# matrixorigin/matrixone

Measured on AMD Instinct MI355X. Metric: ANN queries/sec @ recall@10>=0.95, 10Mx768 f32, higher is better.
Workload: dtype f32; 1 GPU; ivfflat-l2-10000000x768-nlist4096-nprobe32-batch1024-k10; rows_per_gpu=10000000, dim=768, nlist=4096, nprobe=32, global_batch=1024, k=10, scan=two-stage-refine-R64, parallelism=single

## Files before the change

include/moann.h:

```cpp

#ifndef MOANN_H
#define MOANN_H

#include <stdint.h>
#include <stddef.h>
#include <stdbool.h>

#ifdef __cplusplus
extern "C" {
#endif


typedef enum {
    DistanceType_L2Expanded = 0,
    DistanceType_L2SqrtExpanded = 1,
    DistanceType_CosineExpanded = 2,
    DistanceType_L1 = 3,
    DistanceType_InnerProduct = 6,
    DistanceType_Unknown = 255
} distance_type_t;

typedef enum {
    Quantization_F32 = 0,
    Quantization_F16 = 1,
    Quantization_INT8 = 2,
    Quantization_UINT8 = 3,
    Quantization_BF16 = 4
} quantization_t;

typedef enum {
    DistributionMode_SINGLE_GPU = 0,
    DistributionMode_SHARDED = 1,
    DistributionMode_REPLICATED = 2
} distribution_mode_t;

typedef struct {
    uint32_t n_lists;
    bool add_data_on_build;
    double kmeans_trainset_fraction;
} ivf_flat_build_params_t;

typedef struct {
    uint32_t n_probes;
} ivf_flat_search_params_t;

typedef void* gpu_ivf_flat_c;
typedef void* gpu_ivf_flat_result_c;

typedef struct {
    gpu_ivf_flat_result_c result_ptr;
} gpu_ivf_flat_search_res_t;


gpu_ivf_flat_c gpu_ivf_flat_new(const void* dataset_data,
                                uint64_t count_vectors, uint32_t dimension,
                                distance_type_t metric,
                                ivf_flat_build_params_t build_params,
                                const int* devices, int device_count,
                                uint32_t nthread,
                                distribution_mode_t dist_mode,
                                quantization_t btype, quantization_t qtype,
                                const int64_t* ids, void* errmsg);

gpu_ivf_flat_c gpu_ivf_flat_load_file(const char* filename,
                                      uint32_t dimension,
                                      distance_type_t metric,
                                      ivf_flat_build_params_t build_params,
                                      const int* devices, int device_count,
                                      uint32_t nthread,
                                      distribution_mode_t dist_mode,
                                      quantization_t btype,
                                      quantization_t qtype, void* errmsg);

gpu_ivf_flat_c gpu_ivf_flat_new_empty(uint64_t total_count, uint32_t dimension,
                                      distance_type_t metric,
                                      ivf_flat_build_params_t build_params,
                                      const int* devices, int device_count,
                                      uint32_t nthread,
                                      distribution_mode_t dist_mode,
                                      quantization_t btype, quantization_t qtype,
                                      const int64_t* ids, void* errmsg);

void gpu_ivf_flat_add_chunk(gpu_ivf_flat_c index_c, const void* chunk_data,
                            uint64_t chunk_count, const int64_t* ids,
                            void* errmsg);

void gpu_ivf_flat_add_chunk_float(gpu_ivf_flat_c index_c,
                                  const float* chunk_data,
                                  uint64_t chunk_count, const int64_t* ids,
                                  void* errmsg);

void gpu_ivf_flat_add_chunk_quantize(gpu_ivf_flat_c index_c,
                                     const void* base_data,
                                     uint64_t chunk_count, const int64_t* ids,
                                     void* errmsg);

void gpu_ivf_flat_extend(gpu_ivf_flat_c index_c, const void* new_data,
                         uint64_t n_rows, const int64_t* new_ids,
                         void* errmsg);
void gpu_ivf_flat_extend_float(gpu_ivf_flat_c index_c, const float* new_data,
                               uint64_t n_rows, const int64_t* new_ids,
                               void* errmsg);

void gpu_ivf_flat_train_quantizer(gpu_ivf_flat_c index_c,
                                  const float* train_data,
                                  uint64_t n_samples, void* errmsg);

void gpu_ivf_flat_delete_id(gpu_ivf_flat_c index_c, int64_t id, void* errmsg);

void moann_ivf_flat_set_centroids(gpu_ivf_flat_c index_c,
                                  const float* centroids, uint32_t n_lists,
                                  void* errmsg);
void moann_ivf_flat_set_assignments(gpu_ivf_flat_c index_c,
                                    const int32_t* assignments, uint64_t count,
                                    void* errmsg);

void gpu_ivf_flat_build(gpu_ivf_flat_c index_c, void* errmsg);

void moann_ivf_flat_set_kmeans_params(gpu_ivf_flat_c index_c, uint32_t n_iters,
                                      uint64_t max_train_rows, void* errmsg);

void moann_ivf_flat_get_assignments(gpu_ivf_flat_c index_c, int32_t* out,
                                    void* errmsg);

void moann_ivf_flat_kmeans_stats(gpu_ivf_flat_c index_c, double* train_ms,
                                 double* assign_ms, uint32_t* iters,
                                 uint64_t* n_train, void* errmsg);

void gpu_ivf_flat_start(gpu_ivf_flat_c index_c, void* errmsg);

void gpu_ivf_flat_save_dir(gpu_ivf_flat_c index_c, const char* dir,
                           void* errmsg);
void gpu_ivf_flat_load_dir(gpu_ivf_flat_c index_c, const char* dir,
                           distribution_mode_t target_mode, void* errmsg);

void gpu_ivf_flat_save(gpu_ivf_flat_c index_c, const char* filename,
                       void* errmsg);

char* gpu_ivf_flat_info(gpu_ivf_flat_c index_c, void* errmsg);

void gpu_ivf_flat_destroy(gpu_ivf_flat_c index_c, void* errmsg);

void gpu_ivf_flat_set_quantizer(gpu_ivf_flat_c index_c, float min, float max,
                                void* errmsg);
void gpu_ivf_flat_get_quantizer(gpu_ivf_flat_c index_c, float* min, float* max,
                                void* errmsg);


gpu_ivf_flat_search_res_t gpu_ivf_flat_search(gpu_ivf_flat_c index_c,
                                              const void* queries_data,
                                              uint64_t num_queries,
                                              uint32_t query_dimension,
                                              uint32_t limit,
                                              ivf_flat_search_params_t search_params,
                                              void* errmsg);

gpu_ivf_flat_search_res_t gpu_ivf_flat_search_quantize(
    gpu_ivf_flat_c index_c, const void* queries_data, uint64_t num_queries,
    uint32_t query_dimension, uint32_t limit,
    ivf_flat_search_params_t search_params, void* errmsg);

uint64_t gpu_ivf_flat_search_quantize_async(
    gpu_ivf_flat_c index_c, const void* queries_data, uint64_t num_queries,
    uint32_t query_dimension, uint32_t limit,
    ivf_flat_search_params_t search_params, void* errmsg);

void moann_ivf_flat_enable_refine(gpu_ivf_flat_c index_c, uint32_t depth,
                                  void* errmsg);

gpu_ivf_flat_search_res_t moann_ivf_flat_search_submit(
    gpu_ivf_flat_c index_c, const void* queries, int queries_on_device,
    uint64_t num_queries, uint32_t query_dimension, uint32_t limit,
    ivf_flat_search_params_t search_params, void* errmsg);
int moann_ivf_flat_result_wait(gpu_ivf_flat_result_c result_c, void* errmsg);

gpu_ivf_flat_search_res_t moann_ivf_flat_search_device(gpu_ivf_flat_c index_c,
                                                       const void* queries_dev,
                                                       uint64_t num_queries,
                                                       uint32_t query_dimension,
                                                       uint32_t limit,
                                                       ivf_flat_search_params_t search_params,
                                                       void* errmsg);

uint64_t gpu_ivf_flat_search_async(gpu_ivf_flat_c index_c,
                                   const void* queries_data,
                                   uint64_t num_queries,
                                   uint32_t query_dimension, uint32_t limit,
                                   ivf_flat_search_params_t search_params,
                                   void* errmsg);
gpu_ivf_flat_search_res_t gpu_ivf_flat_search_wait(gpu_ivf_flat_c index_c,
                                                   uint64_t job_id,
                                                   void* errmsg);

void gpu_ivf_flat_get_neighbors(gpu_ivf_flat_result_c result_c,
                                uint64_t total_elements, int64_t* neighbors);
void gpu_ivf_flat_get_distances(gpu_ivf_flat_result_c result_c,
                                uint64_t total_elements, float* distances);
void gpu_ivf_flat_free_result(gpu_ivf_flat_result_c result_c);


uint64_t gpu_ivf_flat_cap(gpu_ivf_flat_c index_c);
uint64_t gpu_ivf_flat_len(gpu_ivf_flat_c index_c);
uint32_t gpu_ivf_flat_get_n_list(gpu_ivf_flat_c index_c);
void gpu_ivf_flat_get_centers(gpu_ivf_flat_c index_c, void* centers,
                              void* errmsg);


void moann_brute_force_search(const float* dataset, uint64_t count,
                              uint32_t dimension, distance_type_t metric,
                              const int64_t* ids,
                              const float* queries, uint64_t num_queries,
                              uint32_t limit, int device,
                              int64_t* out_neighbors, float* out_distances,
                              void* errmsg);

void moann_pairwise_distance(distance_type_t metric, const float* query,
                             const float* rows, uint64_t n, uint32_t dim,
                             int device, float* out_dists, void* errmsg);

gpu_ivf_flat_search_res_t moann_ivf_flat_search_filtered(
    gpu_ivf_flat_c index_c, const void* queries_data, uint64_t num_queries,
    uint32_t query_dimension, uint32_t limit,
    ivf_flat_search_params_t search_params, const uint32_t* slot_bitset,
    uint64_t nbits, void* errmsg);

void moann_ivf_flat_slots_of_ids(gpu_ivf_flat_c index_c, const int64_t* ids,
                                 uint64_t n, int64_t* out_slots,
                                 void* errmsg);

void gpu_ivf_flat_set_batch_window(gpu_ivf_flat_c index_c, int64_t window_us,
                                   void* errmsg);

void gpu_ivf_flat_set_dynb_conservative_dispatch(gpu_ivf_flat_c index_c,
                                                 bool enable, void* errmsg);

void gpu_ivf_flat_set_filter_columns(gpu_ivf_flat_c index_c,
                                     const char* col_meta_json,
                                     uint64_t total_count, void* errmsg);
void gpu_ivf_flat_add_filter_chunk(gpu_ivf_flat_c index_c, uint32_t col_idx,
                                   const void* data,
                                   const uint32_t* null_bitmap,
                                   uint64_t nrows, void* errmsg);

gpu_ivf_flat_search_res_t gpu_ivf_flat_search_with_filter(
    gpu_ivf_flat_c index_c, const void* queries_data, uint64_t num_queries,
    uint32_t query_dimension, uint32_t limit,
    ivf_flat_search_params_t search_params, const char* preds_json,
    void* errmsg);
gpu_ivf_flat_search_res_t gpu_ivf_flat_search_quantize_with_filter(
    gpu_ivf_flat_c index_c, const void* queries_data, uint64_t num_queries,
    uint32_t query_dimension, uint32_t limit,
    ivf_flat_search_params_t search_params, const char* preds_json,
    void* errmsg);
uint64_t gpu_ivf_flat_search_quantize_with_filter_async(
    gpu_ivf_flat_c index_c, const void* queries_data, uint64_t num_queries,
    uint32_t query_dimension, uint32_t limit,
    ivf_flat_search_params_t search_params, const char* preds_json,
    void* errmsg);

#define MOANN_FILTER_BLOOM 0
#define MOANN_FILTER_CROARING 2
#define MOANN_FILTER_CBITMAP 3
#define MOANN_FILTER_SORTED64 4

int moann_docfilter_eval(int kind, const void* payload, uint64_t payload_len,
                         const int64_t* keys, uint64_t nkeys,
                         uint32_t* out_words, void* errmsg);

int moann_preds_eval(const char* cols_json, const char* preds_json,
                     const void* const* col_data,
                     const uint32_t* const* col_nulls,
                     const int64_t* host_ids, uint64_t nrows,
                     uint32_t* out_words, void* errmsg);

int moann_ivf_flat_filter_from_preds(gpu_ivf_flat_c index_c,
                                     const char* cols_json,
                                     const char* preds_json,
                                     const void* const* col_data,
                                     const uint32_t* const* col_nulls,
                                     uint32_t* out_words, void* errmsg);

int moann_ivf_flat_filter_from_docfilter(gpu_ivf_flat_c index_c, int kind,
                                         const void* payload,
                                         uint64_t payload_len,
                                         uint32_t* out_words, void* errmsg);


typedef struct {
    uint64_t scan_launches;
    double scan_ms;
    uint64_t scan_bytes;
    uint64_t scan_rows;
    uint64_t rank_launches;
    double rank_ms;
    uint64_t rank_flops;
    double select_ms;
    double other_ms;
} moann_perf_t;

void moann_ivf_flat_perf(gpu_ivf_flat_c index_c, moann_perf_t* out);
void moann_ivf_flat_perf_reset(gpu_ivf_flat_c index_c);


typedef void* moann_bf_c;

moann_bf_c moann_bf_new(uint32_t dimension, distance_type_t metric,
                        uint64_t capacity_hint, const int* devices,
                        int device_count, void* errmsg);
moann_bf_c moann_bf_new_typed(uint32_t dimension, distance_type_t metric,
                              quantization_t storage, uint64_t capacity_hint,
                              const int* devices, int device_count,
                              void* errmsg);
void moann_bf_add(moann_bf_c h, const float* rows, uint64_t n,
                  const int64_t* ids, void* errmsg);
void moann_bf_add_half(moann_bf_c h, const uint16_t* rows, uint64_t n,
                       const int64_t* ids, void* errmsg);
void moann_bf_delete_id(moann_bf_c h, int64_t id, void* errmsg);
void moann_bf_set_params(moann_bf_c h, uint32_t mode, uint32_t slice_rows,
                         void* errmsg);
void moann_bf_search(moann_bf_c h, const float* queries, uint64_t nq,
                     uint32_t dim, uint32_t k, int64_t* out_ids,
// ... 111 lines not shown
```

matrixone_amd/csrc/moann_internal.h:

```cpp

#ifndef MOANN_INTERNAL_H
#define MOANN_INTERNAL_H

#include <hip/hip_runtime.h>
#include <cstdint>

#include "moann_scan_plan.h"

namespace moann {

struct ScanJobs {
    const int64_t* databaseg;
    const int32_t* gstart;
    const int32_t* gcount;
    const int32_t* rows;
    const int32_t* nq;
    const int32_t* qbase;
    const int32_t* qslot_query;
    const int64_t* qslot_outbase;
    const int64_t* slot_base;
    int njobs;
};

void launch_scan(int metric, ScanVariant variant, const float* packed,
                 const float* queries, const float* qnorms, int dpad,
                 const ScanJobs& jobs, float* dists_out, hipStream_t stream,
                 const uint32_t* filter_bitset = nullptr);

void launch_scan_asm768(const float* packed, const float* queries,
                        int dpad, const ScanJobs& jobs, float* dists_out,
                        hipStream_t stream,
                        const uint32_t* filter_bitset = nullptr);

void launch_topk(const float* dists, const int64_t* qoffs, int64_t uniform_n,
                 int nq, int k, int32_t* out_slots, float* out_dists,
                 hipStream_t stream);

void launch_gather(const int32_t* sel_slots, const float* sel_dists,
                   const int32_t* probe_lists, const int64_t* probe_offs,
                   const int64_t* list_slot_base, const int64_t* id_by_slot,
                   int nprobe, int nq, int k, int do_sqrt, double inv_mul2,
                   int64_t* out_ids, float* out_dists, hipStream_t stream);

void launch_gather_uniform(const int32_t* sel_slots, const float* sel_dists,
                           const int64_t* id_by_slot, int nq, int k,
                           int do_sqrt, double inv_mul2,
                           int64_t* out_ids, float* out_dists,
                           hipStream_t stream);

void launch_pack(const float* vecs, int dim, int dpad,
                 const int64_t* group_rowbase, const int32_t* group_valid,
                 const int64_t* slot_rows, int64_t ngroups, float* packed,
                 hipStream_t stream);

void launch_unpack(const float* packed, int dim, int dpad,
                   const int64_t* group_slotbase, const int32_t* group_valid,
                   int64_t ngroups, int64_t slot_lo, int64_t slot_hi,
                   float* out, hipStream_t stream);

bool launch_rank_gemm(int metric, const float* queries, const float* cents,
                      const float* qnorms, const float* cnorms, int nq,
                      int nlist, int dpad, float* out, hipStream_t stream);

struct KmRowMap {
    int64_t num, den;
};

void launch_km_assign(int metric, const float* rows, int64_t row_stride,
                      KmRowMap map, int64_t n, const float* cents,
                      const float* cnorms, int k, int dim, int dpad,
                      int32_t* assign, float* best, hipStream_t stream);
void launch_km_row_sumsq(bool inverse_norm, const float* rows,
                         int64_t row_stride, KmRowMap map, int64_t n, int dim,
                         float* out, hipStream_t stream);
void launch_km_update(const float* rows, int64_t row_stride, KmRowMap map,
                      const int64_t* offs, const int32_t* members,
                      const float* inv_norm, int k, int dim, int dpad,
                      float* cents, hipStream_t stream);
void launch_km_set_centroids(const float* rows, int64_t row_stride,
                             KmRowMap map, const int32_t* cidx,
                             const int64_t* trow, int count, int dim, int dpad,
                             float* cents, hipStream_t stream);
void launch_km_gather_pad(const float* rows, int64_t row_stride, KmRowMap map,
                          int64_t i0, int64_t count, int dim, int dpad,
                          float* out, hipStream_t stream);

struct BfPlan;

void launch_bf_fused_topk(int metric, const float* rows, const float* xnorms,
                          const uint32_t* mask, int64_t n,
                          const float* queries, const float* qnorms, int nq,
                          int dpad, int k, const BfPlan& plan, float* cand_d,
                          int32_t* cand_r, hipStream_t stream);
void launch_bf_fused_topk_h(int metric, const uint16_t* rows,
                            const float* xnorms, const uint32_t* mask,
                            int64_t n, const uint16_t* queries,
                            const float* qnorms, int nq, int dpad, int k,
                            const BfPlan& plan, float* cand_d, int32_t* cand_r,
                            hipStream_t stream);
void launch_bf_widen_half(const uint16_t* in, int64_t nrows, int dpad_h,
                          int dpad_w, float* out, hipStream_t stream);
void launch_bf_mask(float* dmat, int nq, int64_t len, int64_t row0,
                    const uint32_t* mask, hipStream_t stream);
void launch_bf_stash(const int32_t* sel_slots, const float* sel_dists, int nq,
                     int k, int64_t row0, int64_t slice, int64_t nslices,
                     float* cand_d, int32_t* cand_r, hipStream_t stream);
void launch_bf_gather(const int32_t* sel_slots, const float* sel_dists,
                      const int32_t* cand_r, int64_t cand_per_q,
                      const int64_t* ids, int nq, int k, int do_sqrt,
                      int64_t* out_ids, float* out_dists, hipStream_t stream);

void launch_scan_i8(int metric, ScanVariant variant, bool uns,
                    ByteImageLayout layout, const uint8_t* packed,
                    const uint8_t* queries_q, const int32_t* qnorms,
                    const int32_t* rownorms, int dpad, const ScanJobs& jb,
                    float* dists_out, hipStream_t stream,
                    const uint32_t* filter_bitset = nullptr);
void launch_bytes_pack_mfma(const uint8_t* rows_q, int dpad,
                            const int64_t* group_rowbase,
                            const int32_t* group_valid,
                            const int64_t* slot_rows, int64_t ngroups,
                            uint8_t* packed, hipStream_t stream);
void launch_bytes_pack16(const uint8_t* rows_q, int dpad,
                         const int64_t* group_rowbase,
                         const int32_t* group_valid,
                         const int64_t* slot_rows, int64_t ngroups,
                         uint8_t* packed, hipStream_t stream);
void launch_rownorms_i8(bool uns, ByteImageLayout layout,
                        const uint8_t* packed, int64_t ngroups, int dpad,
                        int32_t* out, hipStream_t stream);
void launch_unpack_bytes(const uint8_t* packed, int dim, int dpad,
                         const int64_t* group_slotbase,
                         const int32_t* group_valid, int64_t ngroups,
                         int64_t slot_lo, int64_t slot_hi, uint8_t* out,
                         hipStream_t stream);
void launch_refine(int metric, const float* rows_f32, const float* queries,
                   const float* qnorms, int dim, int dpad, int R, int nq,
                   const int32_t* rsel_slots, const float* rsel_dists,
                   const int32_t* probe_lists, const int64_t* probe_offs,
                   const int64_t* list_slot_base, int nprobe, float* refined,
                   hipStream_t stream);
void launch_compose_select(const int32_t* sel2, const int32_t* rsel_slots,
                           int R, int k, int nq, int32_t* out,
                           hipStream_t stream);
void launch_quantize_rows(bool uns, const float* in, int64_t nrows,
                          int in_stride, int dim, int dpad, float fmul,
                          float fadd, uint8_t* out, hipStream_t stream);
void launch_pq_pack(const uint8_t* codes_rowmajor, int nsub,
                    const int64_t* group_rowbase, const int32_t* group_valid,
                    const int64_t* slot_rows, int64_t ngroups, uint8_t* packed,
                    hipStream_t stream);
void launch_quantize_half_rows(bool bf, const float* in, int64_t nrows,
                               int in_stride, int dim, int dpad,
                               uint16_t* out, hipStream_t stream);
void launch_qnorms_h(bool bf, const uint16_t* q, int nq, int dpad,
                     float* out, hipStream_t stream);
void launch_scan_h(int metric, ScanVariant variant, bool bf,
                   const uint16_t* packed, const uint16_t* queries_h,
                   const float* qnorms, int dpad, const ScanJobs& jb,
                   float* dists_out, hipStream_t stream,
                   const uint32_t* filter_bitset = nullptr);
void launch_qnorms_i8(bool uns, const uint8_t* q, int nq, int dpad,
                      int32_t* out, hipStream_t stream);

void launch_pairwise(int metric, const float* rows, const float* query,
                     float qnorm, int64_t n, int dim, float* out,
                     hipStream_t stream);

void launch_qnorms(const float* queries, int nq, int dpad, float* qnorms,
                   hipStream_t stream);

}

#endif
```

matrixone_amd/csrc/moann_kernels.hip:

```cpp

#include <hip/hip_runtime.h>
#include <hip/hip_fp16.h>
#include <algorithm>
#include <cfloat>
#include <cstdint>
#include <cstdlib>
#include <cstring>
#include <stdexcept>
#include <string>
#include <type_traits>

#include "moann_internal.h"
#include "moann_scan_device.h"

namespace moann {

#define WAVE 64

template <typename F>
static void with_metric(int metric, F&& f) {
    switch (metric) {
    case KM_L2SQ: f(std::integral_constant<int, KM_L2SQ>{}); break;
    case KM_IP:   f(std::integral_constant<int, KM_IP>{}); break;
    case KM_COS:  f(std::integral_constant<int, KM_COS>{}); break;
    default:      f(std::integral_constant<int, KM_L1>{}); break;
    }
}

__device__ __forceinline__ uint32_t f2u(float f) {
    uint32_t u = __float_as_uint(f);
    return u ^ (((int32_t)u >> 31) | 0x80000000u);
}
__device__ __forceinline__ float u2f(uint32_t u) {
    u ^= (((int32_t)(u ^ 0x80000000u)) >> 31) | 0x80000000u;
    return __uint_as_float(u);
}

template <int METRIC, int QT>
__global__ __launch_bounds__(256) void scan_kernel(
    const float* __restrict__ packed, const float* __restrict__ queries,
    const float* __restrict__ qnorms, int dpad, const ScanJobs jobs,
    const uint32_t* __restrict__ filter_bitset,
    float* __restrict__ dists_out) {
    extern __shared__ float lds[];
    float* ldsq = lds;
    float* ldsn = lds + QT * dpad;

    const JobView jv = load_job(jobs);
    stage_query_tile<QT, METRIC == KM_COS>(jv, jobs.qslot_query, queries,
                                           qnorms, dpad, ldsq, ldsn);

    const int wave = threadIdx.x >> 6, lane = threadIdx.x & 63;
    const int gend = jv.gstart + jv.gcount;
    const int d4 = dpad >> 2;

    for (int g0 = jv.gstart + 2 * wave; g0 < gend; g0 += 8) {
        const bool has1 = (g0 + 1) < gend;
        const int g1 = has1 ? g0 + 1 : g0;
        const float4* __restrict__ d0 =
            (const float4*)(packed + (jv.baseg + g0) * (int64_t)64 * dpad) + lane;
        const float4* __restrict__ d1 =
            (const float4*)(packed + (jv.baseg + g1) * (int64_t)64 * dpad) + lane;

        float acc0[QT], acc1[QT];
#pragma unroll
        for (int t = 0; t < QT; ++t) acc0[t] = acc1[t] = 0.f;
        float rn0 = 0.f, rn1 = 0.f;

#pragma unroll 2
        for (int q4 = 0; q4 < d4; ++q4) {
            const float4 x0 = d0[q4 * 64];
            const float4 x1 = d1[q4 * 64];
            if (METRIC == KM_COS) {
                rn0 += x0.x * x0.x + x0.y * x0.y + x0.z * x0.z + x0.w * x0.w;
                rn1 += x1.x * x1.x + x1.y * x1.y + x1.z * x1.z + x1.w * x1.w;
            }
#pragma unroll
            for (int t = 0; t < QT; ++t) {
                const float4 qv = ((const float4*)(ldsq + t * dpad))[q4];
                if (METRIC == KM_L2SQ) {
                    float e;
                    e = x0.x - qv.x; acc0[t] = fmaf(e, e, acc0[t]);
                    e = x0.y - qv.y; acc0[t] = fmaf(e, e, acc0[t]);
                    e = x0.z - qv.z; acc0[t] = fmaf(e, e, acc0[t]);
                    e = x0.w - qv.w; acc0[t] = fmaf(e, e, acc0[t]);
                    e = x1.x - qv.x; acc1[t] = fmaf(e, e, acc1[t]);
                    e = x1.y - qv.y; acc1[t] = fmaf(e, e, acc1[t]);
                    e = x1.z - qv.z; acc1[t] = fmaf(e, e, acc1[t]);
                    e = x1.w - qv.w; acc1[t] = fmaf(e, e, acc1[t]);
                } else if (METRIC == KM_IP || METRIC == KM_COS) {
                    acc0[t] = fmaf(x0.x, qv.x, acc0[t]);
                    acc0[t] = fmaf(x0.y, qv.y, acc0[t]);
                    acc0[t] = fmaf(x0.z, qv.z, acc0[t]);
                    acc0[t] = fmaf(x0.w, qv.w, acc0[t]);
                    acc1[t] = fmaf(x1.x, qv.x, acc1[t]);
                    acc1[t] = fmaf(x1.y, qv.y, acc1[t]);
                    acc1[t] = fmaf(x1.z, qv.z, acc1[t]);
                    acc1[t] = fmaf(x1.w, qv.w, acc1[t]);
                } else {
                    acc0[t] += fabsf(x0.x - qv.x) + fabsf(x0.y - qv.y) +
                               fabsf(x0.z - qv.z) + fabsf(x0.w - qv.w);
                    acc1[t] += fabsf(x1.x - qv.x) + fabsf(x1.y - qv.y) +
                               fabsf(x1.z - qv.z) + fabsf(x1.w - qv.w);
                }
            }
        }

        store_group_pair<QT, METRIC == KM_COS>(
            jobs, jv, lane, g0, g1, has1, acc0, acc1, rn0, rn1, ldsn,
            filter_bitset, dists_out, [](float acc, float rn, float qn) {
                return finish_f32<METRIC>(acc, rn, qn);
            });
    }
}

[[noreturn]] static void bad_variant(const char* launcher, ScanVariant v) {
    throw std::logic_error(std::string(launcher) + ": no kernel for scan " +
                           scan_kind_name(v.kind) + " qt=" +
                           std::to_string(v.qt));
}

void launch_scan(int metric, ScanVariant v, const float* packed,
                 const float* queries, const float* qnorms, int dpad,
                 const ScanJobs& jb, float* dists_out, hipStream_t stream,
                 const uint32_t* filter_bitset) {
    const int qt = v.qt;
    const bool asm768 = v.kind == ScanKind::F32_ASM768 && qt == 16 &&
                        metric == KM_L2SQ && dpad == 768;
    const bool generic = v.kind == ScanKind::F32 &&
                         (qt == 8 || qt == 4 || qt == 2 || qt == 1);
    if (!asm768 && !generic) bad_variant("launch_scan", v);
    if (jb.njobs == 0) return;
    if (asm768) {
        launch_scan_asm768(packed, queries, dpad, jb, dists_out, stream,
                           filter_bitset);
        return;
    }
    with_metric(metric, [&](auto m) {
        constexpr int M = decltype(m)::value;
        const dim3 grid(jb.njobs), block(256);
        const size_t shmem = (size_t)(qt * dpad + qt) * sizeof(float);
        const auto launch = [&](auto kernel) {
            hipLaunchKernelGGL(kernel, grid, block, shmem, stream, packed,
                               queries, qnorms, dpad, jb, filter_bitset,
                               dists_out);
        };
        switch (qt) {
        case 8:  launch(scan_kernel<M, 8>); break;
        case 4:  launch(scan_kernel<M, 4>); break;
        case 2:  launch(scan_kernel<M, 2>); break;
        default: launch(scan_kernel<M, 1>); break;
        }
    });
}

__global__ __launch_bounds__(256) void topk_kernel(
    const float* __restrict__ dists, const int64_t* __restrict__ qoffs,
    int64_t uniform_n, int k, int sortP,
    int32_t* __restrict__ out_slots, float* __restrict__ out_dists) {
    extern __shared__ unsigned char smem[];
    uint32_t* hist = (uint32_t*)smem;
    uint32_t* ctr = hist + 256;
    uint32_t* st = ctr + 8;
    uint64_t* keys = (uint64_t*)(smem + 2048);

    const int q = blockIdx.x;
    const int64_t off = qoffs ? qoffs[q] : (int64_t)q * uniform_n;
    const int64_t count = (qoffs ? qoffs[q + 1] : (int64_t)(q + 1) * uniform_n) - off;
    const int tid = threadIdx.x;
    const int m = (int)(count < (int64_t)k ? count : k);
    int nkeys;

    if (count > (int64_t)k) {
        if (tid == 0) { st[0] = 0; st[1] = 0; st[3] = 0; st[4] = 0; st[5] = 0; }
        __syncthreads();
        for (int level = 0; level < 4 && !st[4]; ++level) {
            const int shift = 24 - 8 * level;
            for (int b = tid; b < 256; b += blockDim.x) hist[b] = 0;
            __syncthreads();
            const uint32_t pref = st[0];
            const int64_t step = blockDim.x;
            int64_t i = tid;
#define MOANN_HISTO(u)                                                                  if (level == 0 || ((u) >> (shift + 8)) == (pref >> (shift + 8)))                atomicAdd(&hist[((u) >> shift) & 255], 1u);
            for (; i + 3 * step < count; i += 4 * step) {
                const uint32_t u0 = f2u(dists[off + i]);
                const uint32_t u1 = f2u(dists[off + i + step]);
                const uint32_t u2 = f2u(dists[off + i + 2 * step]);
                const uint32_t u3 = f2u(dists[off + i + 3 * step]);
                MOANN_HISTO(u0) MOANN_HISTO(u1) MOANN_HISTO(u2) MOANN_HISTO(u3)
            }
            for (; i < count; i += step) {
                const uint32_t u = f2u(dists[off + i]);
                MOANN_HISTO(u)
            }
#undef MOANN_HISTO
            __syncthreads();
            if (tid == 0) {
                const uint32_t need = (uint32_t)k - st[1];
                uint32_t cum = 0; int b = 0;
                for (; b < 256; ++b) {
                    if (cum + hist[b] >= need) break;
                    cum += hist[b];
                }
                st[0] = pref | ((uint32_t)b << shift);
                st[1] += cum;
                if (cum + hist[b] == need) {
                    st[1] += hist[b];
                    st[0] |= (shift ? ((1u << shift) - 1u) : 0u);
                    st[3] = 0; st[4] = 1;
                } else if (st[1] + hist[b] <= (uint32_t)sortP) {
                    st[2] = st[0];
                    st[3] = hist[b];
                    st[5] = (uint32_t)shift;
                    st[4] = 1;
                } else if (level == 3) {
                    st[2] = st[0];
                    st[3] = need - cum;
                    st[5] = 0;
                }
            }
            __syncthreads();
        }
        const uint32_t c_sure = st[1];
        const uint32_t tieval = st[2];
        const uint32_t need_ties = st[3];
        const uint32_t tie_shift = st[5];
        const int exact = st[4] && !need_ties;
        const uint64_t below = (uint64_t)st[0] + (exact ? 1u : 0u);
        if (tid == 0) { ctr[0] = 0; ctr[1] = 0; }
        __syncthreads();
        {
            const int64_t step = blockDim.x;
            int64_t i = tid;
#define MOANN_COLLECT(u, idx)                                                           if ((uint64_t)(u) < below) {                                                    const uint32_t pos = atomicAdd(&ctr[0], 1u);                                keys[pos] = ((uint64_t)(u) << 32) | (uint32_t)(idx);                    } else if (need_ties &&                                                                ((u) >> tie_shift) == (tieval >> tie_shift)) {                       const uint32_t t = atomicAdd(&ctr[1], 1u);                                  if (t < need_ties)                                                              keys[c_sure + t] = ((uint64_t)(u) << 32) | (uint32_t)(idx);             }
            for (; i + 3 * step < count; i += 4 * step) {
                const uint32_t u0 = f2u(dists[off + i]);
                const uint32_t u1 = f2u(dists[off + i + step]);
                const uint32_t u2 = f2u(dists[off + i + 2 * step]);
                const uint32_t u3 = f2u(dists[off + i + 3 * step]);
                MOANN_COLLECT(u0, i) MOANN_COLLECT(u1, i + step)
                MOANN_COLLECT(u2, i + 2 * step) MOANN_COLLECT(u3, i + 3 * step)
            }
            for (; i < count; i += step) {
                const uint32_t u = f2u(dists[off + i]);
                MOANN_COLLECT(u, i)
            }
#undef MOANN_COLLECT
        }
        __syncthreads();
        nkeys = (int)(c_sure + need_ties);
    } else {
        for (int64_t i = tid; i < count; i += blockDim.x)
            keys[i] = ((uint64_t)f2u(dists[off + i]) << 32) | (uint32_t)i;
        __syncthreads();
        nkeys = m;
    }

    for (int i = nkeys + tid; i < sortP; i += blockDim.x) keys[i] = ~0ULL;
    __syncthreads();

    for (int ks = 2; ks <= sortP; ks <<= 1) {
        for (int jj = ks >> 1; jj > 0; jj >>= 1) {
            for (int i = tid; i < sortP; i += blockDim.x) {
                const int l = i ^ jj;
                if (l > i) {
                    const uint64_t a = keys[i], b = keys[l];
                    const bool up = (i & ks) == 0;
                    if ((a > b) == up) { keys[i] = b; keys[l] = a; }
                }
            }
            __syncthreads();
        }
    }

    for (int i = tid; i < k; i += blockDim.x) {
        if (i < m) {
            const uint64_t kv = keys[i];
            out_slots[(int64_t)q * k + i] = (int32_t)(kv & 0xFFFFFFFFu);
            out_dists[(int64_t)q * k + i] = u2f((uint32_t)(kv >> 32));
        } else {
            out_slots[(int64_t)q * k + i] = -1;
            out_dists[(int64_t)q * k + i] = FLT_MAX;
        }
    }
}

void launch_topk(const float* dists, const int64_t* qoffs, int64_t uniform_n,
                 int nq, int k, int32_t* out_slots, float* out_dists,
                 hipStream_t stream) {
    if (nq == 0) return;
    int sortP = 1;
    while (sortP < k) sortP <<= 1;
    if (sortP < 1024) sortP = 1024;
    const size_t shmem = 2048 + (size_t)sortP * 8;
    hipLaunchKernelGGL(topk_kernel, dim3(nq), dim3(256), shmem, stream,
                       dists, qoffs, uniform_n, k, sortP, out_slots, out_dists);
}


__device__ __forceinline__ float transform_score_dev(float raw, int do_sqrt,
                                                     double inv_mul2) {
    double r = (double)raw * inv_mul2;
    if (do_sqrt) r = sqrt(r);
    return (float)r;
}

__global__ void gather_kernel(
    const int32_t* __restrict__ sel_slots, const float* __restrict__ sel_dists,
    const int32_t* __restrict__ probe_lists, const int64_t* __restrict__ probe_offs,
    const int64_t* __restrict__ list_slot_base, const int64_t* __restrict__ id_by_slot,
    int nprobe, int nq, int k, int do_sqrt, double inv_mul2,
    int64_t* __restrict__ out_ids, float* __restrict__ out_dists) {
    const int64_t idx = (int64_t)blockIdx.x * blockDim.x + threadIdx.x;
    if (idx >= (int64_t)nq * k) return;
    const int q = (int)(idx / k);
    const int32_t slot = sel_slots[idx];
    if (slot < 0 || sel_dists[idx] == FLT_MAX) {
        out_ids[idx] = -1; out_dists[idx] = FLT_MAX; return;
    }
    const int64_t* offs = probe_offs + (int64_t)q * (nprobe + 1);
    int lo = 0, hi = nprobe - 1;
    while (lo < hi) {
        const int mid = (lo + hi + 1) >> 1;
        if (offs[mid] <= slot) lo = mid; else hi = mid - 1;
    }
    const int32_t list = probe_lists[(int64_t)q * nprobe + lo];
    const int64_t local = slot - offs[lo];
    out_ids[idx] = id_by_slot[list_slot_base[list] + local];
    out_dists[idx] = transform_score_dev(sel_dists[idx], do_sqrt, inv_mul2);
}

void launch_gather(const int32_t* sel_slots, const float* sel_dists,
                   const int32_t* probe_lists, const int64_t* probe_offs,
                   const int64_t* list_slot_base, const int64_t* id_by_slot,
                   int nprobe, int nq, int k, int do_sqrt, double inv_mul2,
                   int64_t* out_ids, float* out_dists, hipStream_t stream) {
    const int64_t total = (int64_t)nq * k;
    if (!total) return;
    const int block = 256;
    const int grid = (int)((total + block - 1) / block);
    hipLaunchKernelGGL(gather_kernel, dim3(grid), dim3(block), 0, stream,
                       sel_slots, sel_dists, probe_lists, probe_offs,
                       list_slot_base, id_by_slot, nprobe, nq, k, do_sqrt,
                       inv_mul2, out_ids, out_dists);
}

__global__ void gather_uniform_kernel(
    const int32_t* __restrict__ sel_slots, const float* __restrict__ sel_dists,
    const int64_t* __restrict__ id_by_slot, int nq, int k, int do_sqrt,
    double inv_mul2, int64_t* __restrict__ out_ids,
    float* __restrict__ out_dists) {
    const int64_t idx = (int64_t)blockIdx.x * blockDim.x + threadIdx.x;
    if (idx >= (int64_t)nq * k) return;
    const int32_t slot = sel_slots[idx];
    if (slot < 0) { out_ids[idx] = -1; out_dists[idx] = FLT_MAX; return; }
    out_ids[idx] = id_by_slot ? id_by_slot[slot] : (int64_t)slot;
    out_dists[idx] = transform_score_dev(sel_dists[idx], do_sqrt, inv_mul2);
}

void launch_gather_uniform(const int32_t* sel_slots, const float* sel_dists,
                           const int64_t* id_by_slot, int nq, int k,
                           int do_sqrt, double inv_mul2, int64_t* out_ids,
                           float* out_dists, hipStream_t stream) {
    const int64_t total = (int64_t)nq * k;
    if (!total) return;
    const int block = 256;
    const int grid = (int)((total + block - 1) / block);
    hipLaunchKernelGGL(gather_uniform_kernel, dim3(grid), dim3(block), 0,
                       stream, sel_slots, sel_dists, id_by_slot, nq, k,
                       do_sqrt, inv_mul2, out_ids, out_dists);
}

__global__ void pack_kernel(const float* __restrict__ vecs, int dim, int dpad,
                            const int64_t* __restrict__ group_rowbase,
                            const int32_t* __restrict__ group_valid,
                            const int64_t* __restrict__ slot_rows,
                            int64_t ngroups, float* __restrict__ packed) {
    const int64_t nquads = ngroups * (dpad >> 2) * 64;
    const int64_t stride = (int64_t)gridDim.x * blockDim.x;
    for (int64_t idx = (int64_t)blockIdx.x * blockDim.x + threadIdx.x;
         idx < nquads; idx += stride) {
        const int lane = (int)(idx & 63);
        const int64_t rest = idx >> 6;
        const int j4 = (int)(rest % (dpad >> 2));
        const int64_t g = rest / (dpad >> 2);
        float4 v = {0.f, 0.f, 0.f, 0.f};
        if (lane < group_valid[g]) {
            const int64_t row = slot_rows[group_rowbase[g] + lane];
            const float* src = vecs + row * (int64_t)dim;
            const int base = 4 * j4;
            v.x = base + 0 < dim ? src[base + 0] : 0.f;
            v.y = base + 1 < dim ? src[base + 1] : 0.f;
            v.z = base + 2 < dim ? src[base + 2] : 0.f;
            v.w = base + 3 < dim ? src[base + 3] : 0.f;
        }
        ((float4*)packed)[idx] = v;
    }
}

void launch_pack(const float* vecs, int dim, int dpad,
                 const int64_t* group_rowbase, const int32_t* group_valid,
                 const int64_t* slot_rows, int64_t ngroups, float* packed,
                 hipStream_t stream) {
    const int64_t nquads = ngroups * (int64_t)(dpad >> 2) * 64;
    if (!nquads) return;
    const int block = 256;
    const int64_t grid = std::min<int64_t>((nquads + block - 1) / block,
                                           1 << 22);
    hipLaunchKernelGGL(pack_kernel, dim3((uint32_t)grid), dim3(block), 0,
                       stream, vecs, dim, dpad, group_rowbase, group_valid,
                       slot_rows, ngroups, packed);
}

__global__ void unpack_kernel(const float* __restrict__ packed, int dim,
                              int dpad,
                              const int64_t* __restrict__ group_slotbase,
                              const int32_t* __restrict__ group_valid,
                              int64_t ngroups, int64_t slot_lo,
                              int64_t slot_hi, float* __restrict__ out) {
    const int64_t nquads = ngroups * (dpad >> 2) * 64;
    const int64_t stride = (int64_t)gridDim.x * blockDim.x;
    for (int64_t idx = (int64_t)blockIdx.x * blockDim.x + threadIdx.x;
         idx < nquads; idx += stride) {
        const int lane = (int)(idx & 63);
        const int64_t rest = idx >> 6;
        const int j4 = (int)(rest % (dpad >> 2));
        const int64_t g = rest / (dpad >> 2);
        if (lane >= group_valid[g]) continue;
        const int64_t slot = group_slotbase[g] + lane;
        if (slot < slot_lo || slot >= slot_hi) continue;
        const float4 v = ((const float4*)packed)[idx];
        float* dst = out + (slot - slot_lo) * (int64_t)dim;
        const int base = 4 * j4;
        if (base + 0 < dim) dst[base + 0] = v.x;
        if (base + 1 < dim) dst[base + 1] = v.y;
        if (base + 2 < dim) dst[base + 2] = v.z;
        if (base + 3 < dim) dst[base + 3] = v.w;
    }
}

void launch_unpack(const float* packed, int dim, int dpad,
                   const int64_t* group_slotbase, const int32_t* group_valid,
                   int64_t ngroups, int64_t slot_lo, int64_t slot_hi,
                   float* out, hipStream_t stream) {
    const int64_t nquads = ngroups * (int64_t)(dpad >> 2) * 64;
    if (!nquads) return;
    const int block = 256;
    const int64_t grid = std::min<int64_t>((nquads + block - 1) / block,
                                           1 << 22);
// ... 190 lines not shown
            }
#pragma unroll
            for (int t = 0; t < QT; ++t) {
                const uint4 qw =
                    *(const uint4*)(ldsq + t * dpad + j8 * 8);
                float qv[8];
                MOANN_H8(qw.x, qv[0], qv[1]) MOANN_H8(qw.y, qv[2], qv[3])
                MOANN_H8(qw.z, qv[4], qv[5]) MOANN_H8(qw.w, qv[6], qv[7])
#pragma unroll
                for (int u = 0; u < 8; ++u) {
                    if (METRIC == KM_L2SQ) {
                        const float e0 = x0[u] - qv[u];
                        acc0[t] = fmaf(e0, e0, acc0[t]);
                        const float e1 = x1[u] - qv[u];
                        acc1[t] = fmaf(e1, e1, acc1[t]);
                    } else if (METRIC == KM_IP || METRIC == KM_COS) {
                        acc0[t] = fmaf(x0[u], qv[u], acc0[t]);
                        acc1[t] = fmaf(x1[u], qv[u], acc1[t]);
                    } else {
                        acc0[t] += fabsf(x0[u] - qv[u]);
                        acc1[t] += fabsf(x1[u] - qv[u]);
                    }
                }
            }
        }
#undef MOANN_H8

        store_group_pair<QT, METRIC == KM_COS>(
            jobs, jv, lane, g0, g1, has1, acc0, acc1, rn0, rn1, ldsn,
            filter_bitset, dists_out, [](float acc, float rn, float qn) {
                return finish_f32<METRIC>(acc, rn, qn);
            });
    }
}

void launch_scan_h(int metric, ScanVariant v, bool bf,
                   const uint16_t* packed, const uint16_t* queries_h,
                   const float* qnorms, int dpad, const ScanJobs& jb,
                   float* dists_out, hipStream_t stream,
                   const uint32_t* filter_bitset) {
    if (v.kind != ScanKind::HALF || v.qt != 8) bad_variant("launch_scan_h", v);
    if (!jb.njobs) return;
    with_metric(metric, [&](auto m) {
        constexpr int M = decltype(m)::value;
        const dim3 grid(jb.njobs), block(256);
        const size_t shmem = 8 * dpad * 2 + 8 * 4 + 16;
        const auto launch = [&](auto kernel) {
            hipLaunchKernelGGL(kernel, grid, block, shmem, stream, packed,
                               queries_h, qnorms, dpad, jb, filter_bitset,
                               dists_out);
        };
        bf ? launch(scan_h_kernel<M, true>) : launch(scan_h_kernel<M, false>);
    });
}

template <int METRIC>
__global__ __launch_bounds__(256) void refine_kernel(
    const float* __restrict__ rows_f32,
    const float* __restrict__ queries,
    const float* __restrict__ qnorms,
    int dim, int dpad, int R,
    const int32_t* __restrict__ rsel_slots,
    const float* __restrict__ rsel_dists,
    const int32_t* __restrict__ probe_lists,
    const int64_t* __restrict__ probe_offs,
    const int64_t* __restrict__ list_slot_base, int nprobe,
    float* __restrict__ refined ) {
    extern __shared__ float ldsq[];
    const int q = blockIdx.x;
    const float* qv = queries + (int64_t)q * dpad;
    for (int e = threadIdx.x; e < dpad; e += blockDim.x) ldsq[e] = qv[e];
    __syncthreads();
    const int wave = threadIdx.x >> 6, lane = threadIdx.x & 63;
    const int64_t* offs = probe_offs + (int64_t)q * (nprobe + 1);

    for (int c = wave; c < R; c += 4) {
        const int64_t idx = (int64_t)q * R + c;
        const int32_t pos = rsel_slots[idx];
        if (pos < 0 || rsel_dists[idx] == FLT_MAX) {
            if (lane == 0) refined[idx] = FLT_MAX;
            continue;
        }
        int lo = 0, hi = nprobe - 1;
        while (lo < hi) {
            const int mid = (lo + hi + 1) >> 1;
            if (offs[mid] <= pos) lo = mid; else hi = mid - 1;
        }
        const int32_t list = probe_lists[(int64_t)q * nprobe + lo];
        const int64_t slot = list_slot_base[list] + (pos - offs[lo]);
        const float* row = rows_f32 + slot * (int64_t)dim;
        float acc = 0.f, rn = 0.f;
        for (int t = lane; t < dim; t += 64) {
            const float x = row[t], qq = ldsq[t];
            if (METRIC == KM_L2SQ) {
                const float e = x - qq;
                acc = fmaf(e, e, acc);
            } else if (METRIC == KM_IP || METRIC == KM_COS) {
                acc = fmaf(x, qq, acc);
                if (METRIC == KM_COS) rn = fmaf(x, x, rn);
            } else {
                acc += fabsf(x - qq);
            }
        }
        for (int off = 32; off; off >>= 1) {
            acc += __shfl_down(acc, off, 64);
            if (METRIC == KM_COS) rn += __shfl_down(rn, off, 64);
        }
        if (lane == 0) {
            float dist;
            if (METRIC == KM_IP) dist = -acc;
            else if (METRIC == KM_COS)
                dist = mo_cos_distance(acc, rn, qnorms[q]);
            else dist = acc;
            refined[idx] = dist;
        }
    }
}

void launch_refine(int metric, const float* rows_f32, const float* queries,
                   const float* qnorms, int dim, int dpad, int R, int nq,
                   const int32_t* rsel_slots, const float* rsel_dists,
                   const int32_t* probe_lists, const int64_t* probe_offs,
                   const int64_t* list_slot_base, int nprobe, float* refined,
                   hipStream_t stream) {
    if (!nq) return;
    const size_t shmem = (size_t)dpad * 4;
    with_metric(metric, [&](auto m) {
        hipLaunchKernelGGL(refine_kernel<decltype(m)::value>, dim3(nq),
                           dim3(256), shmem, stream, rows_f32, queries, qnorms,
                           dim, dpad, R, rsel_slots, rsel_dists, probe_lists,
                           probe_offs, list_slot_base, nprobe, refined);
    });
}

__global__ void compose_select_kernel(const int32_t* __restrict__ sel2,
                                      const int32_t* __restrict__ rsel_slots,
                                      int R, int k, int64_t total,
                                      int32_t* __restrict__ out) {
    const int64_t i = (int64_t)blockIdx.x * blockDim.x + threadIdx.x;
    if (i >= total) return;
    const int32_t s2 = sel2[i];
    const int64_t q = i / k;
    out[i] = s2 < 0 ? -1 : rsel_slots[q * R + s2];
}

void launch_compose_select(const int32_t* sel2, const int32_t* rsel_slots,
                           int R, int k, int nq, int32_t* out,
                           hipStream_t stream) {
    const int64_t total = (int64_t)nq * k;
    if (!total) return;
    hipLaunchKernelGGL(compose_select_kernel,
                       dim3((uint32_t)((total + 255) / 256)), dim3(256), 0,
                       stream, sel2, rsel_slots, R, k, total, out);
}

template <int METRIC, bool UNSIGNED>
__global__ __launch_bounds__(256) void scan_i8_kernel(
    const uint8_t* __restrict__ packed, const uint8_t* __restrict__ queries_q,
    const int32_t* __restrict__ qnorms_i ,
    int dpad, const ScanJobs jobs,
    const uint32_t* __restrict__ filter_bitset,
    float* __restrict__ dists_out) {
    constexpr int QT = 8;
    extern __shared__ float ldsf[];
    uint8_t* ldsq = (uint8_t*)ldsf;
    int32_t* ldsn = (int32_t*)(ldsq + QT * dpad);

    const JobView jv = load_job(jobs);
    stage_query_tile<QT, METRIC == KM_COS>(jv, jobs.qslot_query, queries_q,
                                           qnorms_i, dpad, ldsq, ldsn);

    const int wave = threadIdx.x >> 6, lane = threadIdx.x & 63;
    const int gend = jv.gstart + jv.gcount;
    const int d4 = dpad >> 2;

    const auto sx = [](uint8_t b) -> int {
        return UNSIGNED ? (int)b : (int)(int8_t)b;
    };

    for (int g0 = jv.gstart + 2 * wave; g0 < gend; g0 += 8) {
        const bool has1 = (g0 + 1) < gend;
        const int g1 = has1 ? g0 + 1 : g0;
        const uchar4* __restrict__ d0 =
            (const uchar4*)(packed + (jv.baseg + g0) * (int64_t)64 * dpad) + lane;
        const uchar4* __restrict__ d1 =
            (const uchar4*)(packed + (jv.baseg + g1) * (int64_t)64 * dpad) + lane;
        int32_t acc0[QT], acc1[QT];
#pragma unroll
        for (int t = 0; t < QT; ++t) acc0[t] = acc1[t] = 0;
        int32_t rn0 = 0, rn1 = 0;
#pragma unroll 2
        for (int q4 = 0; q4 < d4; ++q4) {
            const uchar4 x0 = d0[q4 * 64];
            const uchar4 x1 = d1[q4 * 64];
            if (METRIC == KM_COS) {
                rn0 += sx(x0.x) * sx(x0.x) + sx(x0.y) * sx(x0.y) +
                       sx(x0.z) * sx(x0.z) + sx(x0.w) * sx(x0.w);
                rn1 += sx(x1.x) * sx(x1.x) + sx(x1.y) * sx(x1.y) +
                       sx(x1.z) * sx(x1.z) + sx(x1.w) * sx(x1.w);
            }
#pragma unroll
            for (int t = 0; t < QT; ++t) {
                const uchar4 qv = ((const uchar4*)(ldsq + t * dpad))[q4];
                if (METRIC == KM_L2SQ) {
                    int e;
                    e = sx(x0.x) - sx(qv.x); acc0[t] += e * e;
                    e = sx(x0.y) - sx(qv.y); acc0[t] += e * e;
                    e = sx(x0.z) - sx(qv.z); acc0[t] += e * e;
                    e = sx(x0.w) - sx(qv.w); acc0[t] += e * e;
                    e = sx(x1.x) - sx(qv.x); acc1[t] += e * e;
                    e = sx(x1.y) - sx(qv.y); acc1[t] += e * e;
                    e = sx(x1.z) - sx(qv.z); acc1[t] += e * e;
                    e = sx(x1.w) - sx(qv.w); acc1[t] += e * e;
                } else if (METRIC == KM_IP || METRIC == KM_COS) {
                    acc0[t] += sx(x0.x) * sx(qv.x) + sx(x0.y) * sx(qv.y) +
                               sx(x0.z) * sx(qv.z) + sx(x0.w) * sx(qv.w);
                    acc1[t] += sx(x1.x) * sx(qv.x) + sx(x1.y) * sx(qv.y) +
                               sx(x1.z) * sx(qv.z) + sx(x1.w) * sx(qv.w);
                } else {
                    acc0[t] += abs(sx(x0.x) - sx(qv.x)) +
                               abs(sx(x0.y) - sx(qv.y)) +
                               abs(sx(x0.z) - sx(qv.z)) +
                               abs(sx(x0.w) - sx(qv.w));
                    acc1[t] += abs(sx(x1.x) - sx(qv.x)) +
                               abs(sx(x1.y) - sx(qv.y)) +
                               abs(sx(x1.z) - sx(qv.z)) +
                               abs(sx(x1.w) - sx(qv.w));
                }
            }
        }
        store_group_pair<QT, METRIC == KM_COS>(
            jobs, jv, lane, g0, g1, has1, acc0, acc1, rn0, rn1, ldsn,
            filter_bitset, dists_out, [](int32_t acc, int32_t rn, int32_t qn) {
                return finish_i32<METRIC, false>(acc, rn, qn);
            });
    }
}

template <int METRIC, bool UNSIGNED, int QT = 8>
__global__ __launch_bounds__(256) void scan_i8_dot_kernel(
    const uint8_t* __restrict__ packed, const uint8_t* __restrict__ queries_q,
    const int32_t* __restrict__ qnorms_i,
    const int32_t* __restrict__ rownorms,
    int dpad, const ScanJobs jobs,
    const uint32_t* __restrict__ filter_bitset,
    float* __restrict__ dists_out) {
    constexpr bool NEED_N = METRIC == KM_L2SQ || METRIC == KM_COS;
    extern __shared__ float ldsf[];
    uint8_t* ldsq = (uint8_t*)ldsf;
    int32_t* ldsn = (int32_t*)(ldsq + QT * dpad);

    const JobView jv = load_job(jobs);
    stage_query_tile<QT, NEED_N>(jv, jobs.qslot_query, queries_q, qnorms_i,
                                 dpad, ldsq, ldsn);

    const int wave = threadIdx.x >> 6, lane = threadIdx.x & 63;
    const int gend = jv.gstart + jv.gcount;
    const int d16 = dpad >> 4;

    for (int g0 = jv.gstart + 2 * wave; g0 < gend; g0 += 8) {
        const bool has1 = (g0 + 1) < gend;
        const int g1 = has1 ? g0 + 1 : g0;
        const uint4* __restrict__ d0 =
            (const uint4*)(packed + (jv.baseg + g0) * (int64_t)64 * dpad) + lane;
        const uint4* __restrict__ d1 =
            (const uint4*)(packed + (jv.baseg + g1) * (int64_t)64 * dpad) + lane;

        int32_t acc0[QT], acc1[QT];
#pragma unroll
        for (int t = 0; t < QT; ++t) acc0[t] = acc1[t] = 0;

#pragma unroll 2
        for (int j16 = 0; j16 < d16; ++j16) {
            uint4 x0 = d0[j16 * 64];
            uint4 x1 = d1[j16 * 64];
            if (METRIC == KM_L1 && !UNSIGNED) {
                x0.x ^= 0x80808080u; x0.y ^= 0x80808080u;
                x0.z ^= 0x80808080u; x0.w ^= 0x80808080u;
                x1.x ^= 0x80808080u; x1.y ^= 0x80808080u;
                x1.z ^= 0x80808080u; x1.w ^= 0x80808080u;
            }
#pragma unroll
            for (int t = 0; t < QT; ++t) {
                uint4 qv = *(const uint4*)(ldsq + t * dpad + j16 * 16);
                if (METRIC == KM_L1) {
                    if (!UNSIGNED) {
                        qv.x ^= 0x80808080u; qv.y ^= 0x80808080u;
                        qv.z ^= 0x80808080u; qv.w ^= 0x80808080u;
                    }
                    acc0[t] = (int32_t)__builtin_amdgcn_sad_u8(x0.x, qv.x, (uint32_t)acc0[t]);
                    acc0[t] = (int32_t)__builtin_amdgcn_sad_u8(x0.y, qv.y, (uint32_t)acc0[t]);
                    acc0[t] = (int32_t)__builtin_amdgcn_sad_u8(x0.z, qv.z, (uint32_t)acc0[t]);
                    acc0[t] = (int32_t)__builtin_amdgcn_sad_u8(x0.w, qv.w, (uint32_t)acc0[t]);
                    acc1[t] = (int32_t)__builtin_amdgcn_sad_u8(x1.x, qv.x, (uint32_t)acc1[t]);
                    acc1[t] = (int32_t)__builtin_amdgcn_sad_u8(x1.y, qv.y, (uint32_t)acc1[t]);
                    acc1[t] = (int32_t)__builtin_amdgcn_sad_u8(x1.z, qv.z, (uint32_t)acc1[t]);
                    acc1[t] = (int32_t)__builtin_amdgcn_sad_u8(x1.w, qv.w, (uint32_t)acc1[t]);
                } else if (UNSIGNED) {
                    acc0[t] = (int32_t)__builtin_amdgcn_udot4(x0.x, qv.x, (uint32_t)acc0[t], false);
                    acc0[t] = (int32_t)__builtin_amdgcn_udot4(x0.y, qv.y, (uint32_t)acc0[t], false);
                    acc0[t] = (int32_t)__builtin_amdgcn_udot4(x0.z, qv.z, (uint32_t)acc0[t], false);
                    acc0[t] = (int32_t)__builtin_amdgcn_udot4(x0.w, qv.w, (uint32_t)acc0[t], false);
                    acc1[t] = (int32_t)__builtin_amdgcn_udot4(x1.x, qv.x, (uint32_t)acc1[t], false);
                    acc1[t] = (int32_t)__builtin_amdgcn_udot4(x1.y, qv.y, (uint32_t)acc1[t], false);
                    acc1[t] = (int32_t)__builtin_amdgcn_udot4(x1.z, qv.z, (uint32_t)acc1[t], false);
                    acc1[t] = (int32_t)__builtin_amdgcn_udot4(x1.w, qv.w, (uint32_t)acc1[t], false);
// ... 513 lines not shown
```

matrixone_amd/csrc/moann_lib.cpp:

```cpp

#include <hip/hip_runtime.h>

#include <algorithm>
#include <cfloat>
#include <cmath>
#include <cstdio>
#include <cstdlib>
#include <cstring>
#include <map>
#include <unordered_map>
#include <memory>
#include <atomic>
#include <condition_variable>
#include <mutex>
#include <thread>
#include <chrono>
#include <numeric>
#include <stdexcept>
#include <string>
#include <vector>

#include "../../include/moann.h"
#include "moann_host_common.h"
#include "moann_kmeans_plan.h"

namespace {

using namespace moann;

#define HIP_CHECK MOANN_HIP_CHECK
#define KCHECK MOANN_KCHECK
using DevBuf = MoannDevBuf;
constexpr auto set_errmsg = moann_set_errmsg;

using Result = MoannResult;

struct PerfState {
    moann_perf_t c {};
    hipEvent_t ev[8] {};
    bool made = false;
    void ensure() {
        if (made) return;
        for (auto& e : ev) HIP_CHECK(hipEventCreate(&e));
        made = true;
    }
    ~PerfState() {
        if (made)
            for (auto& e : ev) (void)hipEventDestroy(e);
    }
};

struct SearchCtx {
    hipStream_t stream = nullptr;
    hipEvent_t ev[6] {};
    bool made = false;
    DevBuf w_queries, w_qnorms, w_cdists, w_csel_slots, w_csel_dists;
    DevBuf w_jobs, w_qslots, w_cand, w_sel_slots, w_sel_dists;
    DevBuf w_probe_lists, w_probe_offs, w_qoffs, w_out_ids, w_out_dists;
    DevBuf w_filter, w_queries_q, w_qnorms_i;
    DevBuf w_rsel_slots, w_rsel_dists, w_refined, w_sel2;
    void* h_out = nullptr;
    size_t h_out_bytes = 0;
    std::vector<uint32_t> h_filter;
    std::vector<int32_t> h_probe;
    HostScanJobs rank_jobs;
    ProbeOffsets offs;
    ListScanPlan lists;
    struct Call {
        uint64_t nq = 0;
        uint32_t limit = 0, probe = 0;
        ScanChoice scan {};
        bool refine = false;
        const float* d_q = nullptr;
        const float* d_qn = nullptr;
    } call;
    MoannResult* pending = nullptr;
    void* parent = nullptr;
    void ensure(void* ix) {
        parent = ix;
        if (made) return;
        HIP_CHECK(hipStreamCreate(&stream));
        for (auto& e : ev) HIP_CHECK(hipEventCreate(&e));
        made = true;
    }
    void ensure_hout(size_t need) {
        if (need <= h_out_bytes) return;
        if (h_out) (void)hipHostFree(h_out);
        h_out = nullptr;
        h_out_bytes = 0;
        HIP_CHECK(hipHostMalloc(&h_out, need));
        h_out_bytes = need;
    }
    ~SearchCtx() {
        if (made) {
            (void)hipStreamDestroy(stream);
            for (auto& e : ev) (void)hipEventDestroy(e);
        }
        if (h_out) (void)hipHostFree(h_out);
    }
};

struct IvfIndex {
    int device = 0;
    uint32_t dim = 0, dpad = 0, nlist = 0;
    distance_type_t metric = DistanceType_L2Expanded;
    int kmetric = KM_L2SQ;
    uint64_t cap = 0, count = 0;
    quantization_t btype = Quantization_F32;
    quantization_t qtype = Quantization_F32;
    double quant_mul = 1.0, quant_add = 0.0;
    double quant_min = 0.0, quant_max = 0.0;
    uint8_t* d_packed_q = nullptr;
    int32_t* d_rownorm_q = nullptr;
    int refine_depth = 0;
    float* d_rows_f32 = nullptr;
    uint8_t* d_packed_rq = nullptr;
    ByteImageLayout rq_layout = ByteImageLayout::ROWS16;
    int32_t* d_rownorm_rq = nullptr;
    double rq_mul = 1.0, rq_add = 0.0;
    bool built = false, started = false;

    hipStream_t stream = nullptr;

    std::vector<int64_t> h_ids;
    std::vector<int32_t> h_assign;
    std::vector<float> h_centroids;
    float* d_staging = nullptr;
    double km_fraction = KMEANS_DEFAULT_FRACTION;
    uint32_t km_iters = 0;
    uint64_t km_max_train = 0;
    double km_train_ms = 0.0, km_assign_ms = 0.0;
    uint32_t km_iters_run = 0;
    uint64_t km_n_train = 0;

    float* d_packed = nullptr;
    float* d_cent_packed = nullptr;
    float* d_cent_rows = nullptr;
    float* d_cnorms = nullptr;
    bool rank_mfma = false;
    int64_t* d_id_by_slot = nullptr;
    int64_t* d_list_slot_base = nullptr;
    std::vector<int64_t> list_gbase;
    std::vector<int64_t> group_slotbase;
    std::vector<int32_t> group_valid;
    std::vector<int32_t> list_rows;
    std::vector<int64_t> list_slot_base;
    int64_t total_groups = 0;
    int64_t cent_groups = 0;

    SearchCtx sctx[2];
    uint64_t sparity = 0;
    std::vector<int64_t> h_id_by_slot;
    std::vector<int64_t> h_slot_rows;
    std::unordered_map<int64_t, int64_t> id_to_slot;

    std::mutex mu;
    PerfState perf;

    std::map<uint64_t, std::unique_ptr<Result>> jobs;
    uint64_t next_job = 1;

    std::atomic<int64_t> batch_window_us {0};
    struct PendingReq {
        std::vector<float> queries;
        uint64_t nq;
        uint32_t limit, nprobe;
        uint64_t job_id;
    };
    std::mutex bmu;
    std::condition_variable bcv;
    std::condition_variable bdone_cv;
    std::vector<PendingReq> pending;
    std::map<uint64_t, std::unique_ptr<Result>> done_jobs;
    std::thread batcher;
    bool batcher_stop = false;
    bool batcher_started = false;
    bool dynb_conservative = false;

    std::shared_ptr<IvfIndex> tail;
    std::vector<float> tail_staging;
    std::vector<int64_t> tail_ids;
    std::vector<int32_t> tail_assign;
    std::vector<int64_t> tail_deleted;

    std::vector<uint32_t> alive;
    uint64_t deleted_count = 0;

    std::string filter_cols_json;
    std::vector<int> filter_col_types;
    std::vector<std::vector<uint8_t>> filter_col_data;
    std::vector<std::vector<uint32_t>> filter_col_nulls;
    std::vector<uint64_t> filter_col_rows;
    std::vector<bool> filter_col_has_nulls;

    ~IvfIndex() {
        if (batcher_started) {
            {
                std::lock_guard<std::mutex> lk(bmu);
                batcher_stop = true;
            }
            bcv.notify_all();
            batcher.join();
        }
        (void)hipSetDevice(device);
        for (auto p : {(void*)d_staging, (void*)d_packed, (void*)d_cent_packed,
                       (void*)d_cent_rows, (void*)d_cnorms, (void*)d_packed_q,
                       (void*)d_rownorm_q, (void*)d_rows_f32,
                       (void*)d_packed_rq, (void*)d_rownorm_rq,
                       (void*)d_id_by_slot, (void*)d_list_slot_base})
            if (p) (void)hipFree(p);
        if (stream) (void)hipStreamDestroy(stream);
    }
};

void pack_lists(IvfIndex* ix, const float* d_rows, int64_t nrows,
                const std::vector<int64_t>& slot_rows,
                const std::vector<int64_t>& loffsets,
                float** d_packed_out, std::vector<int64_t>* gbase_out,
                int64_t* ngroups_out) {
    (void)nrows;
    const int64_t nlists = (int64_t)loffsets.size() - 1;
    std::vector<int64_t> gbase(nlists + 1, 0);
    for (int64_t l = 0; l < nlists; ++l) {
        const int64_t rows = loffsets[l + 1] - loffsets[l];
        gbase[l + 1] = gbase[l] + (rows + 63) / 64;
    }
    const int64_t ngroups = gbase[nlists];
    std::vector<int64_t> group_rowbase(ngroups);
    std::vector<int32_t> group_valid(ngroups);
    for (int64_t l = 0; l < nlists; ++l) {
        const int64_t rows = loffsets[l + 1] - loffsets[l];
        for (int64_t g = gbase[l]; g < gbase[l + 1]; ++g) {
            const int64_t gi = g - gbase[l];
            group_rowbase[g] = loffsets[l] + gi * 64;
            const int64_t rem = rows - gi * 64;
            group_valid[g] = (int32_t)std::min<int64_t>(64, rem);
        }
    }
    float* d_packed = nullptr;
    HIP_CHECK(hipMalloc(&d_packed,
                        (size_t)ngroups * 64 * ix->dpad * sizeof(float)));
    DevBuf tmp_rb, tmp_gv, tmp_sr;
    tmp_rb.ensure(ngroups * sizeof(int64_t));
    tmp_gv.ensure(ngroups * sizeof(int32_t));
    tmp_sr.ensure(std::max<size_t>(1, slot_rows.size() * sizeof(int64_t)));
    HIP_CHECK(hipMemcpyAsync(tmp_rb.ptr, group_rowbase.data(),
                             ngroups * sizeof(int64_t), hipMemcpyHostToDevice,
                             ix->stream));
    HIP_CHECK(hipMemcpyAsync(tmp_gv.ptr, group_valid.data(),
                             ngroups * sizeof(int32_t), hipMemcpyHostToDevice,
                             ix->stream));
    if (!slot_rows.empty())
        HIP_CHECK(hipMemcpyAsync(tmp_sr.ptr, slot_rows.data(),
                                 slot_rows.size() * sizeof(int64_t),
                                 hipMemcpyHostToDevice, ix->stream));
    launch_pack(d_rows, (int)ix->dim, (int)ix->dpad, tmp_rb.as<int64_t>(),
                tmp_gv.as<int32_t>(), tmp_sr.as<int64_t>(), ngroups, d_packed,
                ix->stream);
    KCHECK("pack");
    HIP_CHECK(hipStreamSynchronize(ix->stream));
    HIP_CHECK(hipGetLastError());
    *d_packed_out = d_packed;
    if (gbase_out) *gbase_out = std::move(gbase);
    *ngroups_out = ngroups;
}


float half_to_f32(uint16_t b) {
    const uint32_t s = (uint32_t)(b >> 15) << 31;
    uint32_t e = (b >> 10) & 0x1f, m = b & 0x3ff;
    uint32_t out;
    if (e == 0) {
        if (m == 0) out = s;
        else {
            e = 127 - 14;
            while (!(m & 0x400)) { m <<= 1; --e; }
            m &= 0x3ff;
            out = s | (e << 23) | (m << 13);
        }
    } else if (e == 31) {
        out = s | 0x7f800000u | (m << 13);
    } else {
        out = s | ((e + 112) << 23) | (m << 13);
    }
    float f;
    memcpy(&f, &out, 4);
    return f;
}

float bf16_to_f32(uint16_t b) {
    const uint32_t out = (uint32_t)b << 16;
    float f;
    memcpy(&f, &out, 4);
    return f;
}

void storage_to_f32(quantization_t st, const void* src, size_t n,
                    double mul, double add, float* dst) {
    switch (st) {
    case Quantization_F32:
        memcpy(dst, src, n * 4);
        break;
    case Quantization_INT8: {
        const int8_t* p = (const int8_t*)src;
        const double m = mul == 0.0 ? 1.0 : mul;
        for (size_t i = 0; i < n; ++i)
            dst[i] = (float)(((double)p[i] - add) / m);
        break;
    }
    case Quantization_UINT8: {
        const uint8_t* p = (const uint8_t*)src;
        const double m = mul == 0.0 ? 1.0 : mul;
        for (size_t i = 0; i < n; ++i)
            dst[i] = (float)(((double)p[i] - add) / m);
        break;
    }
    case Quantization_F16: {
        const uint16_t* p = (const uint16_t*)src;
        for (size_t i = 0; i < n; ++i) dst[i] = half_to_f32(p[i]);
        break;
    }
    case Quantization_BF16: {
        const uint16_t* p = (const uint16_t*)src;
        for (size_t i = 0; i < n; ++i) dst[i] = bf16_to_f32(p[i]);
        break;
    }
    default:
        throw std::runtime_error("unsupported storage type");
    }
}

size_t storage_elem_bytes(quantization_t st) {
    return st == Quantization_F32 ? 4
           : (st == Quantization_F16 || st == Quantization_BF16) ? 2 : 1;
}

std::vector<float> base_to_f32(quantization_t btype, const void* src,
                               size_t n) {
    std::vector<float> out(n);
    if (btype == Quantization_F32) memcpy(out.data(), src, n * 4);
    else if (btype == Quantization_F16) {
        const uint16_t* p = (const uint16_t*)src;
        for (size_t i = 0; i < n; ++i) out[i] = half_to_f32(p[i]);
    } else throw std::runtime_error("base type must be F32 or F16");
    return out;
}


double collect_result(MoannResult* res);

const ScanOverrides& scan_overrides() {
    static const ScanOverrides ov = [] {
        const char *sc = getenv("MOANN_SCAN"), *bq = getenv("MOANN_BYTE_QT"),
                   *cg = getenv("MOANN_CHUNKG"),
                   *bm = getenv("MOANN_BYTE_MFMA");
        ScanOverrides o;
        o.generic_f32 = sc && strcmp(sc, "generic") == 0;
        o.byte_qt8 = bq && atoi(bq) == 8;
        o.chunk_g = cg ? atoi(cg) : 0;
        o.byte_mfma_off = bm && strcmp(bm, "0") == 0;
        return o;
    }();
    return ov;
}

void stage_queries(IvfIndex* ix, SearchCtx* cx, const float* queries,
                   bool queries_on_device) {
    SearchCtx::Call& c = cx->call;
    const int dpad = (int)ix->dpad;
    const hipStream_t s = cx->stream;
    c.d_q = stage_padded_queries(cx->w_queries, queries, queries_on_device,
                                 c.nq, ix->dim, ix->dpad, s);
    c.d_qn = nullptr;
    const bool use_mfma_rank = ix->rank_mfma && ix->kmetric != KM_L1;
    if (ix->kmetric == KM_COS || use_mfma_rank) {
        cx->w_qnorms.ensure(c.nq * 4);
        launch_qnorms(c.d_q, (int)c.nq, dpad, cx->w_qnorms.as<float>(), s);
        KCHECK("qnorms");
        c.d_qn = cx->w_qnorms.as<float>();
    }
}

void rank_centroids(IvfIndex* ix, SearchCtx* cx) {
    const SearchCtx::Call& c = cx->call;
    const int dpad = (int)ix->dpad, nq = (int)c.nq;
    const hipStream_t s = cx->stream;
    cx->w_cdists.ensure((size_t)c.nq * ix->nlist * 4);
    if (ix->rank_mfma && ix->kmetric != KM_L1) {
        HIP_CHECK(hipEventRecord(cx->ev[0], s));
        launch_rank_gemm(ix->kmetric, c.d_q, ix->d_cent_rows, c.d_qn,
                         ix->d_cnorms, nq, (int)ix->nlist, dpad,
                         cx->w_cdists.as<float>(), s);
        KCHECK("rank-gemm");
    } else {
        plan_rank_scan(c.nq, c.scan.rank.qt, ix->nlist, ix->cent_groups,
                       cx->rank_jobs);
        const ScanJobs jb = upload_scan_jobs(cx->rank_jobs, cx->w_jobs, s);
        HIP_CHECK(hipEventRecord(cx->ev[0], s));
        launch_scan(ix->kmetric, c.scan.rank, ix->d_cent_packed, c.d_q,
                    c.d_qn, dpad, jb, cx->w_cdists.as<float>(), s);
        KCHECK("rank-scan");
    }
    HIP_CHECK(hipEventRecord(cx->ev[1], s));
    cx->w_csel_slots.ensure((size_t)c.nq * c.probe * 4);
    cx->w_csel_dists.ensure((size_t)c.nq * c.probe * 4);
    launch_topk(cx->w_cdists.as<float>(), nullptr, ix->nlist, nq,
                (int)c.probe, cx->w_csel_slots.as<int32_t>(),
                cx->w_csel_dists.as<float>(), s);
    KCHECK("rank-topk");
}

void fetch_probe_and_plan(IvfIndex* ix, SearchCtx* cx) {
    const SearchCtx::Call& c = cx->call;
    const hipStream_t s = cx->stream;
    cx->h_probe.resize((size_t)c.nq * c.probe);
    HIP_CHECK(hipMemcpyAsync(cx->h_probe.data(), cx->w_csel_slots.ptr,
                             cx->h_probe.size() * 4, hipMemcpyDeviceToHost, s));
    HIP_CHECK(hipStreamSynchronize(s));
    HIP_CHECK(hipGetLastError());
    plan_probe_offsets(cx->h_probe.data(), c.nq, c.probe, ix->list_rows,
                       cx->offs);
    plan_list_scan(cx->h_probe.data(), c.nq, c.probe, c.scan.list.qt,
                   list_chunk_groups(ix->qtype, scan_overrides()),
                   ix->list_rows, ix->list_gbase, ix->list_slot_base,
                   cx->offs, cx->lists);
}

void scan_lists(IvfIndex* ix, SearchCtx* cx, const uint32_t* filter_words) {
    const SearchCtx::Call& c = cx->call;
    const int dpad = (int)ix->dpad, nq = (int)c.nq;
    const hipStream_t s = cx->stream;
    const ScanVariant v = c.scan.list;
    const uint32_t* d_filter = nullptr;
    if (filter_words) {
        const size_t fw = (size_t)((ix->count + 31) / 32);
        cx->h_filter.assign(filter_words, filter_words + fw);
        cx->w_filter.ensure(fw * 4);
        HIP_CHECK(hipMemcpyAsync(cx->w_filter.ptr, cx->h_filter.data(),
                                 fw * 4, hipMemcpyHostToDevice, s));
        d_filter = cx->w_filter.as<uint32_t>();
    }
    cx->w_cand.ensure(std::max<int64_t>(1, cx->offs.total_cand) * 4);
    float* d_cand = cx->w_cand.as<float>();
    const ScanJobs jb = upload_scan_jobs(cx->lists.jobs, cx->w_qslots, s);
    HIP_CHECK(hipEventRecord(cx->ev[2], s));
    switch (v.kind) {
    case ScanKind::BYTE_DOT:
    case ScanKind::BYTE_U4: {
        const bool uns = !c.refine && ix->qtype == Quantization_UINT8;
        const uint8_t* image = c.refine ? ix->d_packed_rq : ix->d_packed_q;
        const ByteImageLayout layout =
            c.refine ? ix->rq_layout : ByteImageLayout::ROWS16;
        const int32_t* rownorms =
            c.refine ? ix->d_rownorm_rq : ix->d_rownorm_q;
        const double mul = c.refine ? ix->rq_mul : ix->quant_mul;
        const double add = c.refine ? ix->rq_add : ix->quant_add;
        cx->w_queries_q.ensure((size_t)c.nq * dpad);
        uint8_t* d_qq = cx->w_queries_q.as<uint8_t>();
        launch_quantize_rows(uns, c.d_q, (int64_t)c.nq, dpad, (int)ix->dim,
                             dpad, (float)mul, (float)add, d_qq, s);
        KCHECK("query-quantize");
        const int32_t* d_qni = nullptr;
        if (ix->kmetric == KM_COS || ix->kmetric == KM_L2SQ) {
            cx->w_qnorms_i.ensure(c.nq * 4);
            launch_qnorms_i8(uns, d_qq, nq, dpad,
                             cx->w_qnorms_i.as<int32_t>(), s);
            d_qni = cx->w_qnorms_i.as<int32_t>();
        }
        launch_scan_i8(ix->kmetric, v, uns, layout, image, d_qq, d_qni,
                       rownorms, dpad, jb, d_cand, s, d_filter);
        break;
    }
    case ScanKind::HALF: {
        const bool bf = ix->qtype == Quantization_BF16;
        cx->w_queries_q.ensure((size_t)c.nq * dpad * 2);
        uint16_t* d_qh = cx->w_queries_q.as<uint16_t>();
        launch_quantize_half_rows(bf, c.d_q, (int64_t)c.nq, dpad,
                                  (int)ix->dim, dpad, d_qh, s);
        KCHECK("query-half-cast");
        const float* d_qnh = nullptr;
        if (ix->kmetric == KM_COS) {
            cx->w_qnorms_i.ensure(c.nq * 4);
            launch_qnorms_h(bf, d_qh, nq, dpad, cx->w_qnorms_i.as<float>(),
                            s);
            d_qnh = cx->w_qnorms_i.as<float>();
        }
        launch_scan_h(ix->kmetric, v, bf, (const uint16_t*)ix->d_packed_q,
                      d_qh, d_qnh, dpad, jb, d_cand, s, d_filter);
        break;
    }
    case ScanKind::F32:
    case ScanKind::F32_ASM768:
        launch_scan(ix->kmetric, v, ix->d_packed, c.d_q, c.d_qn, dpad, jb,
                    d_cand, s, d_filter);
        break;
    }
    KCHECK("list-scan");
    HIP_CHECK(hipEventRecord(cx->ev[3], s));
}

void select_candidates(IvfIndex* ix, SearchCtx* cx) {
    const SearchCtx::Call& c = cx->call;
    const int dpad = (int)ix->dpad, nq = (int)c.nq, limit = (int)c.limit;
    const hipStream_t s = cx->stream;
    upload_vector(cx->w_qoffs, cx->offs.qoffs, s);
    upload_vector(cx->w_probe_lists, cx->h_probe, s);
    upload_vector(cx->w_probe_offs, cx->offs.probe_offs, s);
    cx->w_sel_slots.ensure((size_t)c.nq * limit * 4);
    cx->w_sel_dists.ensure((size_t)c.nq * limit * 4);
    HIP_CHECK(hipEventRecord(cx->ev[4], s));
    if (c.refine) {
        const int R = std::max<int>(limit, ix->refine_depth);
        cx->w_rsel_slots.ensure((size_t)c.nq * R * 4);
        cx->w_rsel_dists.ensure((size_t)c.nq * R * 4);
        launch_topk(cx->w_cand.as<float>(), cx->w_qoffs.as<int64_t>(), 0, nq,
                    R, cx->w_rsel_slots.as<int32_t>(),
                    cx->w_rsel_dists.as<float>(), s);
        KCHECK("refine-topR");
        cx->w_refined.ensure((size_t)c.nq * R * 4);
        launch_refine(ix->kmetric, ix->d_rows_f32, c.d_q, c.d_qn,
                      (int)ix->dim, dpad, R, nq,
                      cx->w_rsel_slots.as<int32_t>(),
                      cx->w_rsel_dists.as<float>(),
                      cx->w_probe_lists.as<int32_t>(),
                      cx->w_probe_offs.as<int64_t>(), ix->d_list_slot_base,
                      (int)c.probe, cx->w_refined.as<float>(), s);
        KCHECK("refine");
        cx->w_sel2.ensure((size_t)c.nq * limit * 4);
        launch_topk(cx->w_refined.as<float>(), nullptr, R, nq, limit,
                    cx->w_sel2.as<int32_t>(), cx->w_sel_dists.as<float>(), s);
        KCHECK("refine-topk");
        launch_compose_select(cx->w_sel2.as<int32_t>(),
                              cx->w_rsel_slots.as<int32_t>(), R, limit, nq,
                              cx->w_sel_slots.as<int32_t>(), s);
        KCHECK("refine-compose");
    } else {
        launch_topk(cx->w_cand.as<float>(), cx->w_qoffs.as<int64_t>(), 0, nq,
                    limit, cx->w_sel_slots.as<int32_t>(),
                    cx->w_sel_dists.as<float>(), s);
        KCHECK("cand-topk");
    }
    HIP_CHECK(hipEventRecord(cx->ev[5], s));
}

void gather_results(IvfIndex* ix, SearchCtx* cx) {
    const SearchCtx::Call& c = cx->call;
    const size_t n = (size_t)c.nq * c.limit;
    const hipStream_t s = cx->stream;
    const int do_sqrt = ix->metric == DistanceType_L2SqrtExpanded;
    const double inv_mul2 =
        (ix->quant_mul != 0.0 && ix->quant_mul != 1.0)
            ? 1.0 / (ix->quant_mul * ix->quant_mul) : 1.0;
    cx->w_out_ids.ensure(n * 8);
    cx->w_out_dists.ensure(n * 4);
    launch_gather(cx->w_sel_slots.as<int32_t>(), cx->w_sel_dists.as<float>(),
                  cx->w_probe_lists.as<int32_t>(),
                  cx->w_probe_offs.as<int64_t>(), ix->d_list_slot_base,
                  ix->d_id_by_slot, (int)c.probe, (int)c.nq, (int)c.limit,
                  do_sqrt, inv_mul2, cx->w_out_ids.as<int64_t>(),
                  cx->w_out_dists.as<float>(), s);
    KCHECK("gather");
    cx->ensure_hout(n * 12);
    int64_t* ho_ids = (int64_t*)cx->h_out;
    float* ho_dists = (float*)(ho_ids + n);
    HIP_CHECK(hipMemcpyAsync(ho_ids, cx->w_out_ids.ptr, n * 8,
                             hipMemcpyDeviceToHost, s));
    HIP_CHECK(hipMemcpyAsync(ho_dists, cx->w_out_dists.ptr, n * 4,
                             hipMemcpyDeviceToHost, s));
}

std::unique_ptr<Result> run_search(IvfIndex* ix, const float* queries,
                                   bool queries_on_device, uint64_t nq,
                                   uint32_t limit, uint32_t n_probes,
                                   const uint32_t* filter_words = nullptr,
                                   bool sync_end = true) {
    std::lock_guard<std::mutex> lk(ix->mu);
    HIP_CHECK(hipSetDevice(ix->device));
    SearchCtx* cx = &ix->sctx[ix->sparity++ & 1];
    cx->ensure(ix);
    if (cx->pending) collect_result(cx->pending);
    auto res = std::make_unique<Result>();
    res->neighbors.assign((size_t)nq * limit, -1);
    res->distances.assign((size_t)nq * limit, FLT_MAX);
    if (nq == 0) return res;
    if (!ix->built) throw std::runtime_error("index not built");
    if (ix->count == 0) return res;
    if (limit > 4096) throw std::runtime_error("limit > 4096 unsupported");
    const uint32_t probe =
        std::min<uint32_t>(n_probes ? n_probes : 1, ix->nlist);
    if (probe > 4096) throw std::runtime_error("n_probes > 4096 unsupported");
    ix->perf.ensure();

    SearchCtx::Call& c = cx->call;
    c.nq = nq;
    c.limit = limit;
    c.probe = probe;
    c.refine = ix->qtype == Quantization_F32 && ix->refine_depth > 0 &&
               ix->d_packed_rq != nullptr;
    c.scan = pick_scan(ix->kmetric, (int)ix->dpad, ix->qtype, c.refine,
                       (c.refine ? ix->d_rownorm_rq : ix->d_rownorm_q) !=
                           nullptr,
                       scan_overrides());

    const auto t_all0 = std::chrono::steady_clock::now();
    stage_queries(ix, cx, queries, queries_on_device);
    rank_centroids(ix, cx);
    fetch_probe_and_plan(ix, cx);
    scan_lists(ix, cx, filter_words);
    select_candidates(ix, cx);
    gather_results(ix, cx);

    ix->perf.c.rank_launches++;
    ix->perf.c.rank_flops += 2ull * nq * ix->nlist * ix->dim;
    uint64_t unique_rows = 0;
    for (uint32_t l = 0; l < ix->nlist; ++l)
        if (cx->lists.lcount[l]) unique_rows += (uint64_t)ix->list_rows[l];
    ix->perf.c.scan_launches++;
    ix->perf.c.scan_bytes += unique_rows * ix->dim * 4;
    ix->perf.c.scan_rows += (uint64_t)cx->offs.total_cand;

    res->owner = cx;
    res->collected = false;
    HIP_CHECK(hipEventCreate(&res->done_ev));
    HIP_CHECK(hipEventRecord(res->done_ev, cx->stream));
    cx->pending = res.get();
    const double kms = sync_end ? collect_result(res.get()) : 0.0;
    const double wall = std::chrono::duration<double, std::milli>(
        std::chrono::steady_clock::now() - t_all0).count();
    ix->perf.c.other_ms += wall - kms;
    return res;
}

void merge_tail_into(MoannResult* res) {
    if (!res->tail_res || res->tail_merged) return;
    MoannResult* t = res->tail_res.get();
    const size_t total = res->neighbors.size();
    if (t->neighbors.size() != total || total == 0) { res->tail_merged = true; return; }
    const uint32_t limit = res->merge_limit;
    const size_t nq = limit ? total / limit : 0;
    const bool ip = res->merge_kmetric == KM_IP;
    auto closer = [&](float a, float b) { return ip ? a > b : a < b; };
    std::vector<int64_t> mi(limit);
    std::vector<float> md(limit);
    for (size_t q = 0; q < nq; ++q) {
        const int64_t* an = res->neighbors.data() + q * limit;
        const float* ad = res->distances.data() + q * limit;
        const int64_t* bn = t->neighbors.data() + q * limit;
        const float* bd = t->distances.data() + q * limit;
        uint32_t i = 0, j = 0, o = 0;
        while (o < limit) {
            const bool av = i < limit && an[i] != -1;
            const bool bv = j < limit && bn[j] != -1;
            if (!av && !bv) break;
            if (av && (!bv || closer(ad[i], bd[j]) ||
                       (ad[i] == bd[j] && true ))) {
                mi[o] = an[i]; md[o] = ad[i]; ++i;
            } else {
                mi[o] = bn[j]; md[o] = bd[j]; ++j;
            }
            ++o;
        }
        for (; o < limit; ++o) { mi[o] = -1; md[o] = FLT_MAX; }
        memcpy(res->neighbors.data() + q * limit, mi.data(), limit * 8);
        memcpy(res->distances.data() + q * limit, md.data(), limit * 4);
    }
    res->tail_merged = true;
    res->tail_res.reset();
}

double collect_result(MoannResult* res) {
    if (res->collected) return 0.0;
    auto cx = (SearchCtx*)res->owner;
    auto ix = (IvfIndex*)cx->parent;
    HIP_CHECK(hipEventSynchronize(res->done_ev));
    HIP_CHECK(hipGetLastError());
    const size_t n = res->neighbors.size();
    const int64_t* ho_ids = (const int64_t*)cx->h_out;
    const float* ho_dists = (const float*)(ho_ids + n);
    memcpy(res->neighbors.data(), ho_ids, n * 8);
    memcpy(res->distances.data(), ho_dists, n * 4);
    if (ix->kmetric == KM_IP) {
        float* d = res->distances.data();
        for (size_t i = 0; i < n; ++i)
            if (d[i] != FLT_MAX && d[i] != -FLT_MAX) d[i] = -d[i];
    }
    float r_ms = 0, sc_ms = 0, sel_ms = 0;
    (void)hipEventElapsedTime(&r_ms, cx->ev[0], cx->ev[1]);
    (void)hipEventElapsedTime(&sc_ms, cx->ev[2], cx->ev[3]);
    (void)hipEventElapsedTime(&sel_ms, cx->ev[4], cx->ev[5]);
    ix->perf.c.rank_ms += r_ms;
    ix->perf.c.scan_ms += sc_ms;
    ix->perf.c.select_ms += sel_ms;
    res->collected = true;
    if (cx->pending == res) cx->pending = nullptr;
    merge_tail_into(res);
    return (double)r_ms + sc_ms + sel_ms;
}

uint64_t total_len(IvfIndex* ix) {
    return ix->count + (ix->tail ? ix->tail->count : 0);
}

std::vector<uint32_t> combined_filter(IvfIndex* ix, uint64_t slot0,
                                      const uint32_t* user, uint64_t nbits) {
    const uint64_t n = ix->count;
    std::vector<uint32_t> out((size_t)((n + 31) / 32), ~0u);
    if (user) {
        if (slot0 % 32 == 0 && slot0 + n <= nbits) {
            memcpy(out.data(), user + slot0 / 32, out.size() * 4);
            if (n % 32)
                out.back() |= ~((1u << (n % 32)) - 1u);
        } else {
            for (uint64_t i = 0; i < n; ++i) {
                const uint64_t g = slot0 + i;
// ... 879 lines not shown
        ix->done_jobs.erase(it);
        if (res->neighbors.empty() && res->distances.empty())
            throw std::runtime_error("batched search failed");
        out.result_ptr = res.release();
    } catch (const std::exception& e) {
        set_errmsg(errmsg, "gpu_ivf_flat_search_wait", e.what());
    }
    return out;
}

void gpu_ivf_flat_get_neighbors(gpu_ivf_flat_result_c r, uint64_t n,
                                int64_t* neighbors) {
    auto res = (Result*)r;
    if (!res->collected) collect_result(res);
    const uint64_t m = std::min<uint64_t>(n, res->neighbors.size());
    memcpy(neighbors, res->neighbors.data(), m * 8);
}

void gpu_ivf_flat_get_distances(gpu_ivf_flat_result_c r, uint64_t n,
                                float* distances) {
    auto res = (Result*)r;
    if (!res->collected) collect_result(res);
    const uint64_t m = std::min<uint64_t>(n, res->distances.size());
    memcpy(distances, res->distances.data(), m * 4);
}

void gpu_ivf_flat_free_result(gpu_ivf_flat_result_c r) {
    auto res = (Result*)r;
    if (res && res->done_ev) {
        if (!res->collected) {
            (void)hipEventSynchronize(res->done_ev);
            auto cx = (SearchCtx*)res->owner;
            if (cx && cx->pending == res) cx->pending = nullptr;
        }
        (void)hipEventDestroy(res->done_ev);
    }
    delete res;
}

int moann_ivf_flat_filter_from_preds(gpu_ivf_flat_c h, const char* cols_json,
                                     const char* preds_json,
                                     const void* const* col_data,
                                     const uint32_t* const* col_nulls,
                                     uint32_t* out_words, void* errmsg) {
    try {
        auto ix = IX(h);
        if (!ix->built) throw std::runtime_error("index not built");
        const uint64_t n = ix->count;
        std::vector<uint32_t> row_bits((n + 31) / 32, 0);
        std::vector<int64_t> ids_by_row(n);
        for (uint64_t s2 = 0; s2 < n; ++s2)
            ids_by_row[ix->h_slot_rows[s2]] = ix->h_id_by_slot[s2];
        const int rc = moann_preds_eval(cols_json, preds_json, col_data,
                                        col_nulls, ids_by_row.data(), n,
                                        row_bits.data(), errmsg);
        if (rc != 0) return rc;
        std::memset(out_words, 0, ((n + 31) / 32) * 4);
        for (uint64_t s2 = 0; s2 < n; ++s2) {
            const uint64_t row = (uint64_t)ix->h_slot_rows[s2];
            if ((row_bits[row >> 5] >> (row & 31)) & 1u)
                out_words[s2 >> 5] |= 1u << (s2 & 31);
        }
        return 0;
    } catch (const std::exception& e) {
        set_errmsg(errmsg, "moann_ivf_flat_filter_from_preds", e.what());
        return -1;
    }
}

int moann_ivf_flat_filter_from_docfilter(gpu_ivf_flat_c h, int kind,
                                         const void* payload,
                                         uint64_t payload_len,
                                         uint32_t* out_words, void* errmsg) {
    try {
        auto ix = IX(h);
        if (!ix->built) throw std::runtime_error("index not built");
        return moann_docfilter_eval(kind, payload, payload_len,
                                    ix->h_id_by_slot.data(), ix->count,
                                    out_words, errmsg);
    } catch (const std::exception& e) {
        set_errmsg(errmsg, "moann_ivf_flat_filter_from_docfilter", e.what());
        return -1;
    }
}

uint64_t gpu_ivf_flat_cap(gpu_ivf_flat_c h) { return IX(h)->cap; }
uint64_t gpu_ivf_flat_len(gpu_ivf_flat_c h) { return total_len(IX(h)); }
uint32_t gpu_ivf_flat_get_n_list(gpu_ivf_flat_c h) { return IX(h)->nlist; }

void gpu_ivf_flat_get_centers(gpu_ivf_flat_c h, void* centers, void* errmsg) {
    try {
        auto ix = IX(h);
        if (ix->h_centroids.empty())
            throw std::runtime_error("no centroids set");
        memcpy(centers, ix->h_centroids.data(),
               ix->h_centroids.size() * sizeof(float));
    } catch (const std::exception& e) {
        set_errmsg(errmsg, "gpu_ivf_flat_get_centers", e.what());
    }
}

void moann_ivf_flat_set_kmeans_params(gpu_ivf_flat_c h, uint32_t n_iters,
                                      uint64_t max_train_rows, void* errmsg) {
    try {
        auto ix = IX(h);
        std::lock_guard<std::mutex> lk(ix->mu);
        if (ix->built)
            throw std::runtime_error("index already built");
        ix->km_iters = n_iters;
        ix->km_max_train = max_train_rows;
    } catch (const std::exception& e) {
        set_errmsg(errmsg, "moann_ivf_flat_set_kmeans_params", e.what());
    }
}

void moann_ivf_flat_get_assignments(gpu_ivf_flat_c h, int32_t* out,
                                    void* errmsg) {
    try {
        auto ix = IX(h);
        std::lock_guard<std::mutex> lk(ix->mu);
        if (!ix->built) throw std::runtime_error("index not built");
        if (ix->h_slot_rows.size() != ix->count)
            throw std::runtime_error(
                "add-order rows are not kept for a loaded index");
        for (uint32_t l = 0; l < ix->nlist; ++l) {
            const int64_t b = ix->list_slot_base[l];
            for (int64_t sl = b; sl < b + ix->list_rows[l]; ++sl)
                out[ix->h_slot_rows[sl]] = (int32_t)l;
        }
        for (size_t i = 0; i < ix->tail_assign.size(); ++i)
            out[ix->count + i] = ix->tail_assign[i];
    } catch (const std::exception& e) {
        set_errmsg(errmsg, "moann_ivf_flat_get_assignments", e.what());
    }
}

void moann_ivf_flat_kmeans_stats(gpu_ivf_flat_c h, double* train_ms,
                                 double* assign_ms, uint32_t* iters,
                                 uint64_t* n_train, void* errmsg) {
    try {
        auto ix = IX(h);
        if (!ix) throw std::runtime_error("null index");
        std::lock_guard<std::mutex> lk(ix->mu);
        if (!ix->built) throw std::runtime_error("index not built");
        if (train_ms) *train_ms = ix->km_train_ms;
        if (assign_ms) *assign_ms = ix->km_assign_ms;
        if (iters) *iters = ix->km_iters_run;
        if (n_train) *n_train = ix->km_n_train;
    } catch (const std::exception& e) {
        set_errmsg(errmsg, "moann_ivf_flat_kmeans_stats", e.what());
    }
}

void moann_brute_force_search(const float* dataset, uint64_t count,
                              uint32_t dimension, distance_type_t metric,
                              const int64_t* ids, const float* queries,
                              uint64_t num_queries, uint32_t limit, int device,
                              int64_t* out_neighbors, float* out_distances,
                              void* errmsg) {
    char* inner = nullptr;
    try {
        ivf_flat_build_params_t bp {1, true, 0.5};
        gpu_ivf_flat_c h = gpu_ivf_flat_new_empty(
            count, dimension, metric, bp, &device, 1, 0,
            DistributionMode_SINGLE_GPU, Quantization_F32, Quantization_F32,
            nullptr, &inner);
        if (!h) throw std::runtime_error(inner ? inner : "new failed");
        gpu_ivf_flat_add_chunk(h, dataset, count, ids, &inner);
        std::vector<float> cent(dimension, 0.f);
        moann_ivf_flat_set_centroids(h, cent.data(), 1, &inner);
        std::vector<int32_t> assign(count, 0);
        moann_ivf_flat_set_assignments(h, assign.data(), count, &inner);
        gpu_ivf_flat_build(h, &inner);
        if (inner) throw std::runtime_error(inner);
        ivf_flat_search_params_t sp {1};
        auto r = gpu_ivf_flat_search(h, queries, num_queries, dimension, limit,
                                     sp, &inner);
        if (!r.result_ptr) throw std::runtime_error(inner ? inner : "search failed");
        gpu_ivf_flat_get_neighbors(r.result_ptr, num_queries * limit,
                                   out_neighbors);
        gpu_ivf_flat_get_distances(r.result_ptr, num_queries * limit,
                                   out_distances);
        if (metric == DistanceType_InnerProduct)
            for (uint64_t i = 0; i < num_queries * (uint64_t)limit; ++i)
                if (out_distances[i] != FLT_MAX && out_distances[i] != -FLT_MAX)
                    out_distances[i] = -out_distances[i];
        gpu_ivf_flat_free_result(r.result_ptr);
        gpu_ivf_flat_destroy(h, nullptr);
    } catch (const std::exception& e) {
        set_errmsg(errmsg, "moann_brute_force_search", e.what());
    }
    if (inner) free(inner);
}

gpu_ivf_flat_search_res_t moann_ivf_flat_search_filtered(
    gpu_ivf_flat_c h, const void* queries_data, uint64_t num_queries,
    uint32_t query_dimension, uint32_t limit, ivf_flat_search_params_t sp,
    const uint32_t* slot_bitset, uint64_t nbits, void* errmsg) {
    gpu_ivf_flat_search_res_t out {nullptr};
    try {
        auto ix = IX(h);
        if (query_dimension != ix->dim)
            throw std::runtime_error("query dimension mismatch");
        if (nbits < total_len(ix))
            throw std::runtime_error("filter bitset smaller than index");
        out.result_ptr = run_search_full(ix, (const float*)queries_data,
                                         false, num_queries, limit,
                                         sp.n_probes, slot_bitset, nbits)
                             .release();
    } catch (const std::exception& e) {
        set_errmsg(errmsg, "moann_ivf_flat_search_filtered", e.what());
    }
    return out;
}

void moann_ivf_flat_slots_of_ids(gpu_ivf_flat_c h, const int64_t* ids,
                                 uint64_t n, int64_t* out_slots,
                                 void* errmsg) {
    try {
        auto ix = IX(h);
        std::lock_guard<std::mutex> lk(ix->mu);
        if (!ix->built) throw std::runtime_error("index not built");
        if (ix->id_to_slot.empty() && ix->count) {
            ix->id_to_slot.reserve(ix->count * 2);
            for (uint64_t sidx = 0; sidx < ix->count; ++sidx)
                ix->id_to_slot.emplace(ix->h_id_by_slot[sidx], (int64_t)sidx);
        }
        IvfIndex* t = ix->tail.get();
        if (t && t->count && t->id_to_slot.empty()) {
            t->id_to_slot.reserve(t->count * 2);
            for (uint64_t sidx = 0; sidx < t->count; ++sidx)
                t->id_to_slot.emplace(t->h_id_by_slot[sidx], (int64_t)sidx);
        }
        for (uint64_t i = 0; i < n; ++i) {
            auto it = ix->id_to_slot.find(ids[i]);
            if (it != ix->id_to_slot.end()) {
                out_slots[i] = it->second;
                continue;
            }
            out_slots[i] = -1;
            if (t && t->count) {
                auto jt = t->id_to_slot.find(ids[i]);
                if (jt != t->id_to_slot.end())
                    out_slots[i] = (int64_t)ix->count + jt->second;
            }
        }
    } catch (const std::exception& e) {
        set_errmsg(errmsg, "moann_ivf_flat_slots_of_ids", e.what());
    }
}


gpu_ivf_flat_c gpu_ivf_flat_new(const void* dataset_data,
                                uint64_t count_vectors, uint32_t dimension,
                                distance_type_t metric,
                                ivf_flat_build_params_t build_params,
                                const int* devices, int device_count,
                                uint32_t nthread,
                                distribution_mode_t dist_mode,
                                quantization_t btype, quantization_t qtype,
                                const int64_t* ids, void* errmsg) {
    char* inner = nullptr;
    gpu_ivf_flat_c h = gpu_ivf_flat_new_empty(
        count_vectors, dimension, metric, build_params, devices,
        device_count, nthread, dist_mode, btype, qtype, ids, &inner);
    if (!h) {
        set_errmsg(errmsg, "gpu_ivf_flat_new", inner ? inner : "new failed");
        if (inner) free(inner);
        return nullptr;
    }
    if (count_vectors)
        gpu_ivf_flat_add_chunk(h, dataset_data, count_vectors, ids, &inner);
    if (inner) {
        set_errmsg(errmsg, "gpu_ivf_flat_new", inner);
        free(inner);
        gpu_ivf_flat_destroy(h, nullptr);
        return nullptr;
    }
    return h;
}


static void rebuild_tail(IvfIndex* ix) {
    char* inner = nullptr;
    auto chk = [&](const char* what) {
        if (inner) {
            std::string m = std::string(what) + ": " + inner;
            free(inner);
            inner = nullptr;
            throw std::runtime_error(m);
        }
    };
    const uint64_t n = ix->tail_ids.size();
    ivf_flat_build_params_t bp {ix->nlist, true, 1.0};
    int dev = ix->device;
    gpu_ivf_flat_c th = gpu_ivf_flat_new_empty(
        n, ix->dim, ix->metric, bp, &dev, 1, 0,
        DistributionMode_SINGLE_GPU, ix->btype, ix->qtype, nullptr, &inner);
    chk("tail new_empty");
    if (!th) throw std::runtime_error("tail new_empty failed");
    std::unique_ptr<IvfIndex> tix((IvfIndex*)th);
    if (ix->qtype == Quantization_INT8 || ix->qtype == Quantization_UINT8) {
        gpu_ivf_flat_set_quantizer(th, (float)ix->quant_min,
                                   (float)ix->quant_max, &inner);
        chk("tail set_quantizer");
    }
    gpu_ivf_flat_add_chunk_float(th, ix->tail_staging.data(), n,
                                 ix->tail_ids.data(), &inner);
    chk("tail add_chunk");
    moann_ivf_flat_set_centroids(th, ix->h_centroids.data(), ix->nlist,
                                 &inner);
    chk("tail set_centroids");
    moann_ivf_flat_set_assignments(th, ix->tail_assign.data(), n, &inner);
    chk("tail set_assignments");
    gpu_ivf_flat_build(th, &inner);
    chk("tail build");
    ix->tail = std::move(tix);
    for (int64_t id : ix->tail_deleted) {
        IvfIndex* t = ix->tail.get();
        if (t->id_to_slot.empty() && t->count) {
            t->id_to_slot.reserve(t->count * 2);
            for (uint64_t s2 = 0; s2 < t->count; ++s2)
                t->id_to_slot.emplace(t->h_id_by_slot[s2], (int64_t)s2);
        }
        auto it = t->id_to_slot.find(id);
        if (it == t->id_to_slot.end()) continue;
        const uint64_t pos = (uint64_t)it->second;
        const uint64_t nw = (t->count + 31) / 32;
        if (t->alive.size() < nw) t->alive.resize(nw, ~0u);
        if ((t->alive[pos / 32] >> (pos % 32)) & 1u) {
            t->alive[pos / 32] &= ~(1u << (pos % 32));
            ++t->deleted_count;
        }
    }
}

void gpu_ivf_flat_extend_float(gpu_ivf_flat_c h, const float* new_data,
                               uint64_t n_rows, const int64_t* new_ids,
                               void* errmsg) {
    try {
        auto ix = IX(h);
        std::lock_guard<std::mutex> lk(ix->mu);
        if (!ix->built)
            throw std::runtime_error("extend: index not built");
        if (n_rows == 0) return;
        std::vector<int64_t> nearest(n_rows);
        std::vector<float> ndist(n_rows);
        char* inner = nullptr;
        moann_brute_force_search(ix->h_centroids.data(), ix->nlist, ix->dim,
                                 ix->metric, nullptr, new_data, n_rows, 1,
                                 ix->device, nearest.data(), ndist.data(),
                                 &inner);
        if (inner) {
            std::string m = std::string("extend assign: ") + inner;
            free(inner);
            throw std::runtime_error(m);
        }
        const uint64_t base = total_len(ix);
        ix->tail_staging.insert(ix->tail_staging.end(), new_data,
                                new_data + n_rows * ix->dim);
        for (uint64_t i = 0; i < n_rows; ++i) {
            ix->tail_ids.push_back(new_ids ? new_ids[i]
                                           : (int64_t)(base + i));
            ix->tail_assign.push_back((int32_t)nearest[i]);
        }
        rebuild_tail(ix);
    } catch (const std::exception& e) {
        set_errmsg(errmsg, "gpu_ivf_flat_extend_float", e.what());
    }
}

void gpu_ivf_flat_extend(gpu_ivf_flat_c h, const void* new_data,
                         uint64_t n_rows, const int64_t* new_ids,
                         void* errmsg) {
    try {
        auto ix = IX(h);
        if (ix->qtype == Quantization_F32) {
            gpu_ivf_flat_extend_float(h, (const float*)new_data, n_rows,
                                      new_ids, errmsg);
            return;
        }
        std::vector<float> conv((size_t)n_rows * ix->dim);
        storage_to_f32(ix->qtype, new_data, conv.size(), ix->quant_mul,
                       ix->quant_add, conv.data());
        gpu_ivf_flat_extend_float(h, conv.data(), n_rows, new_ids, errmsg);
    } catch (const std::exception& e) {
        set_errmsg(errmsg, "gpu_ivf_flat_extend", e.what());
    }
}


void gpu_ivf_flat_delete_id(gpu_ivf_flat_c h, int64_t id, void* errmsg) {
    try {
        auto ix = IX(h);
        std::lock_guard<std::mutex> lk(ix->mu);
        if (!ix->built) throw std::runtime_error("delete_id: index not built");
        if (ix->id_to_slot.empty() && ix->count) {
            ix->id_to_slot.reserve(ix->count * 2);
            for (uint64_t sidx = 0; sidx < ix->count; ++sidx)
                ix->id_to_slot.emplace(ix->h_id_by_slot[sidx],
                                       (int64_t)sidx);
        }
        auto it = ix->id_to_slot.find(id);
        if (it != ix->id_to_slot.end()) {
            const uint64_t pos = (uint64_t)it->second;
            const uint64_t nw = (ix->count + 31) / 32;
            if (ix->alive.size() < nw) ix->alive.resize(nw, ~0u);
            if ((ix->alive[pos / 32] >> (pos % 32)) & 1u) {
                ix->alive[pos / 32] &= ~(1u << (pos % 32));
                ++ix->deleted_count;
            }
            return;
        }
        IvfIndex* t = ix->tail.get();
        if (t && t->count) {
            if (t->id_to_slot.empty()) {
                t->id_to_slot.reserve(t->count * 2);
                for (uint64_t s2 = 0; s2 < t->count; ++s2)
                    t->id_to_slot.emplace(t->h_id_by_slot[s2], (int64_t)s2);
            }
            auto jt = t->id_to_slot.find(id);
            if (jt != t->id_to_slot.end()) {
                const uint64_t pos = (uint64_t)jt->second;
                const uint64_t nw = (t->count + 31) / 32;
                if (t->alive.size() < nw) t->alive.resize(nw, ~0u);
                if ((t->alive[pos / 32] >> (pos % 32)) & 1u) {
                    t->alive[pos / 32] &= ~(1u << (pos % 32));
                    ++t->deleted_count;
                    ix->tail_deleted.push_back(id);
                }
                return;
            }
        }
    } catch (const std::exception& e) {
        set_errmsg(errmsg, "gpu_ivf_flat_delete_id", e.what());
    }
}


void gpu_ivf_flat_train_quantizer(gpu_ivf_flat_c h, const float* train_data,
                                  uint64_t n_samples, void* errmsg) {
    try {
        auto ix = IX(h);
        if (ix->qtype != Quantization_INT8 &&
            ix->qtype != Quantization_UINT8)
            throw std::runtime_error(
                "storage has no affine quantizer (int8/uint8 only)");
        if (n_samples == 0) throw std::runtime_error("empty training set");
        size_t n = (size_t)n_samples * ix->dim;
        size_t stride = 1;
        const size_t cap = 1u << 26;
        if (n > cap) stride = (n + cap - 1) / cap;
        if (stride > 1) {
            stride |= 1;
            if (stride % 3 == 0) stride += 2;
        }
        std::vector<float> samp;
        samp.reserve(n / stride + 1);
        for (size_t i = 0; i < n; i += stride) samp.push_back(train_data[i]);
        const size_t k = samp.size() / 200;
        std::nth_element(samp.begin(), samp.begin() + k, samp.end());
        const float lo = samp[k];
        std::nth_element(samp.begin(), samp.end() - 1 - k, samp.end());
        const float hi = samp[samp.size() - 1 - k];
        gpu_ivf_flat_set_quantizer(h, lo, hi, errmsg);
    } catch (const std::exception& e) {
        set_errmsg(errmsg, "gpu_ivf_flat_train_quantizer", e.what());
    }
}
// ... 913 lines not shown
```

matrixone_amd/csrc/moann_scan_plan.h:

```cpp

#ifndef MOANN_SCAN_PLAN_H
#define MOANN_SCAN_PLAN_H

#include <algorithm>
#include <cstddef>
#include <cstdint>
#include <stdexcept>
#include <vector>

#include "../../include/moann.h"

namespace moann {

enum MetricKind : int {
    KM_L2SQ = 0,
    KM_IP = 1,
    KM_COS = 2,
    KM_L1 = 3,
};

inline int metric_kind(distance_type_t m) {
    switch (m) {
    case DistanceType_L2Expanded:
    case DistanceType_L2SqrtExpanded: return KM_L2SQ;
    case DistanceType_CosineExpanded: return KM_COS;
    case DistanceType_InnerProduct: return KM_IP;
    case DistanceType_L1: return KM_L1;
    default: throw std::runtime_error("unsupported metric");
    }
}


enum class ScanKind {
    F32,
    F32_ASM768,
    HALF,
    BYTE_DOT,
    BYTE_U4,
};

struct ScanVariant {
    ScanKind kind;
    int qt;
};

inline const char* scan_kind_name(ScanKind k) {
    static const char* const names[] = {"F32", "F32_ASM768", "HALF",
                                        "BYTE_DOT", "BYTE_U4"};
    return names[(int)k];
}

struct ScanOverrides {
    bool generic_f32 = false;
    bool byte_qt8 = false;
    int chunk_g = 0;
    bool byte_mfma_off = false;
};

struct ScanChoice {
    ScanVariant list, rank;
};

inline ScanVariant pick_f32_variant(int kmetric, int dpad, bool allow_asm) {
    if (allow_asm && kmetric == KM_L2SQ && dpad == 768)
        return {ScanKind::F32_ASM768, 16};
    for (int qt : {8, 4, 2})
        if ((size_t)qt * dpad * 4 + qt * 4 <= 52 * 1024)
            return {ScanKind::F32, qt};
    return {ScanKind::F32, 1};
}

inline ScanChoice pick_scan(int kmetric, int dpad, quantization_t storage,
                            bool refine, bool rownorms,
                            const ScanOverrides& ov) {
    const bool f32_st = storage == Quantization_F32;
    const bool half_st = storage == Quantization_F16 ||
                         storage == Quantization_BF16;
    const bool byte_scan = f32_st ? refine : !half_st;
    ScanChoice c;
    c.rank = pick_f32_variant(kmetric, dpad,
                              f32_st && !refine && !ov.generic_f32);
    if (byte_scan) {
        if (dpad % 16 == 0 && rownorms) {
            const bool wide = (size_t)16 * dpad + 80 <= 48 * 1024 &&
                              !ov.byte_qt8;
            c.list = {ScanKind::BYTE_DOT, wide ? 16 : 8};
        } else {
            c.list = {ScanKind::BYTE_U4, 8};
        }
    } else if (half_st) {
        c.list = {ScanKind::HALF, 8};
    } else {
        c.list = c.rank;
    }
    return c;
}

enum class ByteImageLayout {
    ROWS16,
    MFMA64,
};

inline bool byte_mfma_applies(int kmetric, ScanVariant list, int dpad) {
    return list.kind == ScanKind::BYTE_DOT && list.qt == 16 &&
           kmetric != KM_L1 && dpad % 64 == 0;
}

inline ByteImageLayout pick_refine_layout(int kmetric, ScanVariant list,
                                          int dpad, const ScanOverrides& ov) {
    return byte_mfma_applies(kmetric, list, dpad) && !ov.byte_mfma_off
               ? ByteImageLayout::MFMA64
               : ByteImageLayout::ROWS16;
}


struct HostScanJobs {
    std::vector<int64_t> databaseg, qslot_outbase, slot_base;
    std::vector<int32_t> gstart, gcount, rows, nq, qbase, qslot_query;
    int njobs = 0, nqslots = 0;
    void clear() {
        for (auto* v : {&databaseg, &qslot_outbase, &slot_base}) v->clear();
        for (auto* v : {&gstart, &gcount, &rows, &nq, &qbase, &qslot_query})
            v->clear();
        njobs = nqslots = 0;
    }
};

inline void plan_rank_scan(uint64_t nq, int qt, uint32_t nlist,
                           int64_t cent_groups, HostScanJobs& out) {
    out.clear();
    const int ntiles = (int)((nq + qt - 1) / qt);
    const int64_t want_chunks = std::min<int64_t>(
        cent_groups, std::max<int64_t>(1, (1024 + ntiles - 1) / ntiles));
    const int chunk = (int)((cent_groups + want_chunks - 1) / want_chunks);
    const int nchunk = (int)((cent_groups + chunk - 1) / chunk);
    out.njobs = ntiles * nchunk;
    out.nqslots = ntiles * qt;
    for (int t = 0; t < ntiles; ++t) {
        const int q0 = t * qt;
        const int tn = (int)std::min<int64_t>(qt, (int64_t)nq - q0);
        for (int u = 0; u < qt; ++u) {
            const int qi = std::min<int>(q0 + u, (int)nq - 1);
            out.qslot_query.push_back(qi);
            out.qslot_outbase.push_back((int64_t)qi * nlist);
        }
        for (int c = 0; c < nchunk; ++c) {
            out.databaseg.push_back(0);
            out.gstart.push_back((int32_t)(c * chunk));
            out.gcount.push_back(
                (int32_t)std::min<int64_t>(chunk, cent_groups - c * chunk));
            out.rows.push_back((int32_t)nlist);
            out.nq.push_back(tn);
            out.qbase.push_back(q0);
        }
    }
}

struct ProbeOffsets {
    std::vector<int64_t> probe_offs;
    std::vector<int64_t> qoffs;
    int64_t total_cand = 0;
};

inline void plan_probe_offsets(const int32_t* h_probe, uint64_t nq,
                               uint32_t probe,
                               const std::vector<int32_t>& list_rows,
                               ProbeOffsets& out) {
    out.probe_offs.resize((size_t)nq * (probe + 1));
    out.qoffs.assign(nq + 1, 0);
    for (uint64_t q = 0; q < nq; ++q) {
        int64_t acc = 0;
        out.probe_offs[q * (probe + 1)] = 0;
        for (uint32_t r = 0; r < probe; ++r) {
            const int32_t l = h_probe[q * probe + r];
            if (l >= 0) acc += list_rows[l];
            out.probe_offs[q * (probe + 1) + r + 1] = acc;
        }
        out.qoffs[q + 1] = out.qoffs[q] + acc;
    }
    out.total_cand = out.qoffs[nq];
}

struct ListScanPlan {
    HostScanJobs jobs;
    std::vector<int32_t> lcount, pair_q;
    std::vector<int64_t> lbase, cursor, pair_ob;
};

inline void plan_list_scan(const int32_t* h_probe, uint64_t nq,
                           uint32_t probe, int qt, int64_t chunk_g,
                           const std::vector<int32_t>& list_rows,
                           const std::vector<int64_t>& list_gbase,
                           const std::vector<int64_t>& list_slot_base,
                           const ProbeOffsets& offs, ListScanPlan& out) {
    const uint32_t nlist = (uint32_t)list_rows.size();
    out.lcount.assign(nlist, 0);
    for (uint64_t q = 0; q < nq; ++q)
        for (uint32_t r = 0; r < probe; ++r) {
            const int32_t l = h_probe[q * probe + r];
            if (l >= 0 && list_rows[l] > 0) out.lcount[l]++;
        }
    out.lbase.assign(nlist + 1, 0);
    for (uint32_t l = 0; l < nlist; ++l)
        out.lbase[l + 1] = out.lbase[l] + out.lcount[l];
    const int64_t npairs = out.lbase[nlist];
    out.pair_q.resize(npairs);
    out.pair_ob.resize(npairs);
    out.cursor.assign(out.lbase.begin(), out.lbase.end() - 1);
    for (uint64_t q = 0; q < nq; ++q)
// ... 50 lines not shown
```

matrixone_amd/engine.py:

```python

from __future__ import annotations

import ctypes as ct
import os

import numpy as np

_PKG = os.path.dirname(os.path.abspath(__file__))
_LIB_PATH = os.path.join(_PKG, "libmoann_hip.so")

METRICS = {
    "l2sq": 0,
    "l2": 1,
    "cos": 2,
    "l1": 3,
    "ip": 6,
}


class BuildParams(ct.Structure):
    _fields_ = [("n_lists", ct.c_uint32), ("add_data_on_build", ct.c_bool),
                ("kmeans_trainset_fraction", ct.c_double)]


class SearchParams(ct.Structure):
    _fields_ = [("n_probes", ct.c_uint32)]


class SearchRes(ct.Structure):
    _fields_ = [("result_ptr", ct.c_void_p)]


class PerfT(ct.Structure):
    _fields_ = [
        ("scan_launches", ct.c_uint64), ("scan_ms", ct.c_double),
        ("scan_bytes", ct.c_uint64), ("scan_rows", ct.c_uint64),
        ("rank_launches", ct.c_uint64), ("rank_ms", ct.c_double),
        ("rank_flops", ct.c_uint64),
        ("select_ms", ct.c_double), ("other_ms", ct.c_double),
    ]


_lib = None


def lib() -> ct.CDLL:
    global _lib
    if _lib is not None:
        return _lib
    if not os.path.exists(_LIB_PATH):
        raise RuntimeError(
            f"moann HIP extension missing at {_LIB_PATH} — build it with "
            "`make -C matrixone_amd/csrc` or __graft_entry__.build(). "
            "There is no CPU fallback.")
    L = ct.CDLL(_LIB_PATH)
    L.gpu_ivf_flat_new_empty.restype = ct.c_void_p
    L.gpu_ivf_flat_new_empty.argtypes = [
        ct.c_uint64, ct.c_uint32, ct.c_int, BuildParams,
        ct.POINTER(ct.c_int), ct.c_int, ct.c_uint32, ct.c_int, ct.c_int,
        ct.c_int, ct.c_void_p, ct.c_void_p]
    L.gpu_ivf_flat_new.restype = ct.c_void_p
    L.gpu_ivf_flat_new.argtypes = [
        ct.c_void_p, ct.c_uint64, ct.c_uint32, ct.c_int, BuildParams,
        ct.POINTER(ct.c_int), ct.c_int, ct.c_uint32, ct.c_int, ct.c_int,
        ct.c_int, ct.c_void_p, ct.c_void_p]
    L.gpu_ivf_flat_load_file.restype = ct.c_void_p
    L.gpu_ivf_flat_load_file.argtypes = [
        ct.c_char_p, ct.c_uint32, ct.c_int, BuildParams,
        ct.POINTER(ct.c_int), ct.c_int, ct.c_uint32, ct.c_int, ct.c_int,
        ct.c_int, ct.c_void_p]
    for f in (L.gpu_ivf_flat_add_chunk, L.gpu_ivf_flat_add_chunk_float,
              L.gpu_ivf_flat_add_chunk_quantize, L.gpu_ivf_flat_extend,
              L.gpu_ivf_flat_extend_float):
        f.argtypes = [
            ct.c_void_p, ct.c_void_p, ct.c_uint64, ct.c_void_p, ct.c_void_p]
    L.gpu_ivf_flat_delete_id.argtypes = [ct.c_void_p, ct.c_int64, ct.c_void_p]
    L.gpu_ivf_flat_train_quantizer.argtypes = [
        ct.c_void_p, ct.c_void_p, ct.c_uint64, ct.c_void_p]
    L.gpu_ivf_flat_info.restype = ct.c_void_p
    L.gpu_ivf_flat_info.argtypes = [ct.c_void_p, ct.c_void_p]
    L.gpu_ivf_flat_save.argtypes = [ct.c_void_p, ct.c_char_p, ct.c_void_p]
    L.gpu_ivf_flat_set_dynb_conservative_dispatch.argtypes = [
        ct.c_void_p, ct.c_bool, ct.c_void_p]
    L.gpu_ivf_flat_set_filter_columns.argtypes = [
        ct.c_void_p, ct.c_char_p, ct.c_uint64, ct.c_void_p]
    L.gpu_ivf_flat_add_filter_chunk.argtypes = [
        ct.c_void_p, ct.c_uint32, ct.c_void_p, ct.c_void_p, ct.c_uint64,
        ct.c_void_p]
    for f in (L.gpu_ivf_flat_search_with_filter,
              L.gpu_ivf_flat_search_quantize_with_filter):
        f.restype = SearchRes
        f.argtypes = [ct.c_void_p, ct.c_void_p, ct.c_uint64, ct.c_uint32,
                      ct.c_uint32, SearchParams, ct.c_char_p, ct.c_void_p]
    L.gpu_ivf_flat_search_quantize_with_filter_async.restype = ct.c_uint64
    L.gpu_ivf_flat_search_quantize_with_filter_async.argtypes = [
        ct.c_void_p, ct.c_void_p, ct.c_uint64, ct.c_uint32, ct.c_uint32,
        SearchParams, ct.c_char_p, ct.c_void_p]
    L.moann_docfilter_parse.restype = ct.c_void_p
    L.moann_docfilter_parse.argtypes = [ct.c_int, ct.c_void_p, ct.c_uint64,
                                        ct.c_void_p]
    L.moann_docfilter_test.restype = ct.c_int
    L.moann_docfilter_test.argtypes = [ct.c_void_p, ct.c_void_p,
                                       ct.c_uint64, ct.c_void_p, ct.c_void_p]
    L.moann_docfilter_free.argtypes = [ct.c_void_p]
    L.moann_hnsw_set_ef.argtypes = [ct.c_void_p, ct.c_uint32, ct.c_void_p]
    L.usearchex_filtered_search_with_membership.restype = ct.c_size_t
    L.usearchex_filtered_search_with_membership.argtypes = [
        ct.c_void_p, ct.c_void_p, ct.c_int, ct.c_size_t, ct.c_void_p,
        ct.c_int, ct.c_void_p, ct.c_void_p, ct.POINTER(ct.c_char_p)]
    L.moann_ivf_flat_set_centroids.argtypes = [
        ct.c_void_p, ct.c_void_p, ct.c_uint32, ct.c_void_p]
    L.moann_ivf_flat_set_assignments.argtypes = [
        ct.c_void_p, ct.c_void_p, ct.c_uint64, ct.c_void_p]
    L.moann_ivf_flat_set_kmeans_params.argtypes = [
        ct.c_void_p, ct.c_uint32, ct.c_uint64, ct.c_void_p]
    L.moann_ivf_flat_get_assignments.argtypes = [
        ct.c_void_p, ct.c_void_p, ct.c_void_p]
    L.gpu_ivf_flat_get_centers.argtypes = [
        ct.c_void_p, ct.c_void_p, ct.c_void_p]
    L.moann_ivf_flat_kmeans_stats.argtypes = [
        ct.c_void_p, ct.POINTER(ct.c_double), ct.POINTER(ct.c_double),
        ct.POINTER(ct.c_uint32), ct.POINTER(ct.c_uint64), ct.c_void_p]
    for f in (L.gpu_ivf_flat_build, L.gpu_ivf_flat_start):
        f.argtypes = [ct.c_void_p, ct.c_void_p]
    L.gpu_ivf_flat_destroy.argtypes = [ct.c_void_p, ct.c_void_p]
    for f in (L.gpu_ivf_flat_search, L.gpu_ivf_flat_search_quantize,
              L.moann_ivf_flat_search_device):
        f.restype = SearchRes
        f.argtypes = [ct.c_void_p, ct.c_void_p, ct.c_uint64, ct.c_uint32,
                      ct.c_uint32, SearchParams, ct.c_void_p]
    for f in (L.gpu_ivf_flat_search_async,
              L.gpu_ivf_flat_search_quantize_async):
        f.restype = ct.c_uint64
        f.argtypes = [
            ct.c_void_p, ct.c_void_p, ct.c_uint64, ct.c_uint32, ct.c_uint32,
            SearchParams, ct.c_void_p]
    L.gpu_ivf_flat_search_wait.restype = SearchRes
    L.gpu_ivf_flat_search_wait.argtypes = [ct.c_void_p, ct.c_uint64, ct.c_void_p]
    L.gpu_ivf_flat_get_neighbors.argtypes = [ct.c_void_p, ct.c_uint64, ct.c_void_p]
    L.gpu_ivf_flat_get_distances.argtypes = [ct.c_void_p, ct.c_uint64, ct.c_void_p]
    L.gpu_ivf_flat_free_result.argtypes = [ct.c_void_p]
    for f in (L.gpu_ivf_flat_cap, L.gpu_ivf_flat_len):
        f.restype = ct.c_uint64
        f.argtypes = [ct.c_void_p]
    L.gpu_ivf_flat_get_n_list.restype = ct.c_uint32
    L.gpu_ivf_flat_get_n_list.argtypes = [ct.c_void_p]
    L.gpu_ivf_flat_set_batch_window.argtypes = [ct.c_void_p, ct.c_int64,
                                                ct.c_void_p]
    L.gpu_ivf_flat_set_quantizer.argtypes = [ct.c_void_p, ct.c_float,
                                             ct.c_float, ct.c_void_p]
    L.gpu_ivf_flat_get_quantizer.argtypes = [ct.c_void_p, ct.c_void_p,
                                             ct.c_void_p, ct.c_void_p]
    L.gpu_ivf_flat_save_dir.argtypes = [ct.c_void_p, ct.c_char_p, ct.c_void_p]
    L.gpu_ivf_flat_load_dir.argtypes = [ct.c_void_p, ct.c_char_p, ct.c_int,
                                        ct.c_void_p]
    L.moann_ivf_flat_search_filtered.restype = SearchRes
    L.moann_ivf_flat_search_filtered.argtypes = [
        ct.c_void_p, ct.c_void_p, ct.c_uint64, ct.c_uint32, ct.c_uint32,
        SearchParams, ct.c_void_p, ct.c_uint64, ct.c_void_p]
    L.moann_ivf_flat_search_submit.restype = SearchRes
    L.moann_ivf_flat_search_submit.argtypes = [
        ct.c_void_p, ct.c_void_p, ct.c_int, ct.c_uint64, ct.c_uint32,
        ct.c_uint32, SearchParams, ct.c_void_p]
    L.moann_ivf_flat_result_wait.restype = ct.c_int
    L.moann_ivf_flat_result_wait.argtypes = [ct.c_void_p, ct.c_void_p]
    L.moann_ivf_flat_enable_refine.argtypes = [ct.c_void_p, ct.c_uint32,
                                               ct.c_void_p]
    L.moann_docfilter_eval.restype = ct.c_int
    L.moann_docfilter_eval.argtypes = [
        ct.c_int, ct.c_void_p, ct.c_uint64, ct.c_void_p, ct.c_uint64,
        ct.c_void_p, ct.c_void_p]
    L.moann_ivf_flat_filter_from_docfilter.restype = ct.c_int
    L.moann_ivf_flat_filter_from_docfilter.argtypes = [
        ct.c_void_p, ct.c_int, ct.c_void_p, ct.c_uint64, ct.c_void_p,
        ct.c_void_p]
    L.moann_preds_eval.restype = ct.c_int
    L.moann_preds_eval.argtypes = [
        ct.c_char_p, ct.c_char_p, ct.POINTER(ct.c_void_p),
        ct.POINTER(ct.c_void_p), ct.c_void_p, ct.c_uint64, ct.c_void_p,
        ct.c_void_p]
    L.moann_ivf_flat_filter_from_preds.restype = ct.c_int
    L.moann_ivf_flat_filter_from_preds.argtypes = [
        ct.c_void_p, ct.c_char_p, ct.c_char_p, ct.POINTER(ct.c_void_p),
        ct.POINTER(ct.c_void_p), ct.c_void_p, ct.c_void_p]
    L.moann_ivf_flat_slots_of_ids.argtypes = [
        ct.c_void_p, ct.c_void_p, ct.c_uint64, ct.c_void_p, ct.c_void_p]
    L.moann_brute_force_search.argtypes = [
        ct.c_void_p, ct.c_uint64, ct.c_uint32, ct.c_int, ct.c_void_p,
        ct.c_void_p, ct.c_uint64, ct.c_uint32, ct.c_int, ct.c_void_p,
        ct.c_void_p, ct.c_void_p]
    L.moann_ivf_pq_new.restype = ct.c_void_p
    L.moann_ivf_pq_new.argtypes = [ct.c_uint32, ct.c_uint32, ct.c_uint32,
                                   ct.c_uint64, ct.POINTER(ct.c_int),
                                   ct.c_int, ct.c_void_p]
    L.moann_ivf_pq_set_centroids.argtypes = [ct.c_void_p, ct.c_void_p,
                                             ct.c_uint32, ct.c_void_p]
    L.moann_ivf_pq_set_codebooks.argtypes = [ct.c_void_p, ct.c_void_p,
                                             ct.c_void_p]
    L.moann_ivf_pq_add_codes.argtypes = [ct.c_void_p, ct.c_void_p,
                                         ct.c_uint64, ct.c_void_p, ct.c_void_p]
    L.moann_ivf_pq_set_assignments.argtypes = [ct.c_void_p, ct.c_void_p,
                                               ct.c_uint64, ct.c_void_p]
    L.moann_ivf_pq_build.argtypes = [ct.c_void_p, ct.c_void_p]
    L.moann_ivf_pq_search.restype = SearchRes
    L.moann_ivf_pq_save_dir.argtypes = [ct.c_void_p, ct.c_char_p,
                                        ct.c_void_p]
    L.moann_ivf_pq_load_dir.argtypes = [ct.c_void_p, ct.c_char_p,
                                        ct.c_void_p]
    L.moann_ivf_pq_search_filtered.restype = SearchRes
    L.moann_ivf_pq_search_filtered.argtypes = [
        ct.c_void_p, ct.c_void_p, ct.c_uint64, ct.c_uint32, ct.c_uint32,
        SearchParams, ct.c_void_p, ct.c_uint64, ct.c_void_p]
    L.moann_ivf_pq_search.argtypes = [ct.c_void_p, ct.c_void_p, ct.c_uint64,
                                      ct.c_uint32, ct.c_uint32, SearchParams,
                                      ct.c_void_p]
    L.moann_ivf_pq_perf.argtypes = [ct.c_void_p, ct.POINTER(PerfT)]
    L.moann_ivf_pq_destroy.argtypes = [ct.c_void_p, ct.c_void_p]
    L.moann_ivf_flat_perf.argtypes = [ct.c_void_p, ct.POINTER(PerfT)]
    L.moann_ivf_flat_perf_reset.argtypes = [ct.c_void_p]
    L.moann_pairwise_distance.argtypes = [
        ct.c_int, ct.c_void_p, ct.c_void_p, ct.c_uint64, ct.c_uint32,
        ct.c_int, ct.c_void_p, ct.c_void_p]
    L.moann_bf_new.restype = ct.c_void_p
    L.moann_bf_new.argtypes = [ct.c_uint32, ct.c_int, ct.c_uint64,
                               ct.c_void_p, ct.c_int, ct.c_void_p]
    L.moann_bf_new_typed.restype = ct.c_void_p
    L.moann_bf_new_typed.argtypes = [ct.c_uint32, ct.c_int, ct.c_int,
                                     ct.c_uint64, ct.c_void_p, ct.c_int,
                                     ct.c_void_p]
    L.moann_bf_add_half.argtypes = [ct.c_void_p, ct.c_void_p, ct.c_uint64,
                                    ct.c_void_p, ct.c_void_p]
    L.moann_bf_storage.restype = ct.c_uint32
    L.moann_bf_storage.argtypes = [ct.c_void_p]
    L.moann_bf_add.argtypes = [ct.c_void_p, ct.c_void_p, ct.c_uint64,
                               ct.c_void_p, ct.c_void_p]
    L.moann_bf_delete_id.argtypes = [ct.c_void_p, ct.c_int64, ct.c_void_p]
    L.moann_bf_set_params.argtypes = [ct.c_void_p, ct.c_uint32, ct.c_uint32,
                                      ct.c_void_p]
    for f in (L.moann_bf_search, L.moann_bf_search_device):
        f.argtypes = [ct.c_void_p, ct.c_void_p, ct.c_uint64, ct.c_uint32,
                      ct.c_uint32, ct.c_void_p, ct.c_void_p, ct.c_void_p]
    L.moann_bf_search_filtered.argtypes = [
        ct.c_void_p, ct.c_void_p, ct.c_uint64, ct.c_uint32, ct.c_uint32,
        ct.c_void_p, ct.c_uint64, ct.c_void_p, ct.c_void_p, ct.c_void_p]
    L.moann_bf_len.restype = ct.c_uint64
    L.moann_bf_len.argtypes = [ct.c_void_p]
    L.moann_bf_fused_kmax.restype = ct.c_uint32
    L.moann_bf_perf.argtypes = [ct.c_void_p, ct.POINTER(PerfT)]
    L.moann_bf_destroy.argtypes = [ct.c_void_p, ct.c_void_p]
    L.moann_device_count.restype = ct.c_int
    L.moann_version.restype = ct.c_char_p
    _lib = L
    return L


class MoannError(RuntimeError):
    pass


class _Err:

    def __init__(self):
        self.p = ct.c_char_p(None)

    @property
    def ref(self):
        return ct.byref(self.p)

    def check(self, where: str):
        if self.p.value:
            msg = self.p.value.decode()
            raise MoannError(f"{where}: {msg}")


def device_count() -> int:
    return lib().moann_device_count()


def _as_f32(a) -> np.ndarray:
    arr = np.ascontiguousarray(a, dtype=np.float32)
    return arr


COL_I32, COL_I64, COL_F32, COL_F64, COL_U64 = 0, 1, 2, 3, 4
_COL_DTYPES = {0: np.int32, 1: np.int64, 2: np.float32, 3: np.float64,
               4: np.uint64}


def _col_arrays(cols_meta, columns, nulls):
    import json as _json
    cols_json = _json.dumps([{"name": n, "type": t}
                             for n, t in cols_meta]).encode()
    keep = []
    data_arr = (ct.c_void_p * max(1, len(columns)))()
    null_arr = (ct.c_void_p * max(1, len(columns)))()
    for i, ((name, t), col) in enumerate(zip(cols_meta, columns)):
        a = np.ascontiguousarray(col, dtype=_COL_DTYPES[t])
        keep.append(a)
        data_arr[i] = a.ctypes.data
        nl = None if nulls is None else nulls[i]
        if nl is not None:
            w = np.ascontiguousarray(nl, dtype=np.uint32)
            keep.append(w)
            null_arr[i] = w.ctypes.data
        else:
            null_arr[i] = None
    return cols_json, data_arr, null_arr, keep


def preds_eval(cols_meta, columns, preds_json: str, nrows: int, nulls=None,
               host_ids=None) -> np.ndarray:
    cols_json, data_arr, null_arr, keep = _col_arrays(cols_meta, columns,
                                                      nulls)
    out = np.zeros((nrows + 31) // 32, dtype=np.uint32)
    hid = None
    if host_ids is not None:
        hid = np.ascontiguousarray(host_ids, dtype=np.int64)
        keep.append(hid)
    err = _Err()
    rc = lib().moann_preds_eval(
# ... 144 lines not shown
        err = _Err()
        lib().moann_ivf_flat_set_assignments(self._h, assignments.ctypes.data,
                                             assignments.shape[0], err.ref)
        err.check("set_assignments")

    def set_kmeans_params(self, n_iters: int = 0, max_train_rows: int = 0):
        err = _Err()
        lib().moann_ivf_flat_set_kmeans_params(self._h, n_iters,
                                               max_train_rows, err.ref)
        err.check("set_kmeans_params")

    def centers(self) -> np.ndarray:
        out = np.empty((self.nlist, self.dim), dtype=np.float32)
        err = _Err()
        lib().gpu_ivf_flat_get_centers(self._h, out.ctypes.data, err.ref)
        err.check("get_centers")
        return out

    def assignments(self) -> np.ndarray:
        out = np.empty(len(self), dtype=np.int32)
        err = _Err()
        lib().moann_ivf_flat_get_assignments(self._h, out.ctypes.data,
                                             err.ref)
        err.check("get_assignments")
        return out

    def kmeans_stats(self) -> dict:
        t, a = ct.c_double(0), ct.c_double(0)
        it, nt = ct.c_uint32(0), ct.c_uint64(0)
        err = _Err()
        lib().moann_ivf_flat_kmeans_stats(self._h, ct.byref(t), ct.byref(a),
                                          ct.byref(it), ct.byref(nt), err.ref)
        err.check("kmeans_stats")
        return {"train_ms": t.value, "assign_ms": a.value,
                "iters": it.value, "n_train": nt.value}

    def build(self):
        err = _Err()
        lib().gpu_ivf_flat_build(self._h, err.ref)
        err.check("build")
        lib().gpu_ivf_flat_start(self._h, err.ref)
        err.check("start")

    def __len__(self):
        return lib().gpu_ivf_flat_len(self._h)

    def _read_result(self, res, nq, k, where):
        if not res.result_ptr:
            raise MoannError(f"{where} returned NULL result")
        ids = np.empty((nq, k), dtype=np.int64)
        dists = np.empty((nq, k), dtype=np.float32)
        L = lib()
        L.gpu_ivf_flat_get_neighbors(res.result_ptr, nq * k, ids.ctypes.data)
        L.gpu_ivf_flat_get_distances(res.result_ptr, nq * k, dists.ctypes.data)
        L.gpu_ivf_flat_free_result(res.result_ptr)
        if self.metric == "ip":
            sent = np.float32(np.finfo(np.float32).max)
            m = (dists != sent) & (dists != -sent)
            dists[m] = -dists[m]
        return ids, dists

    def search(self, queries, k: int, nprobe: int):
        queries = _as_f32(queries)
        nq = queries.shape[0]
        err = _Err()
        res = lib().gpu_ivf_flat_search_quantize(
            self._h, queries.ctypes.data, nq, queries.shape[1], k,
            SearchParams(nprobe), err.ref)
        err.check("search_quantize")
        return self._read_result(res, nq, k, "search")

    def set_quantizer(self, vmin: float, vmax: float):
        err = _Err()
        lib().gpu_ivf_flat_set_quantizer(self._h, vmin, vmax, err.ref)
        err.check("set_quantizer")

    def save_dir(self, path: str):
        err = _Err()
        lib().gpu_ivf_flat_save_dir(self._h, path.encode(), err.ref)
        err.check("save_dir")

    def load_dir(self, path: str):
        err = _Err()
        lib().gpu_ivf_flat_load_dir(self._h, path.encode(), 0, err.ref)
        err.check("load_dir")

    def slots_of_ids(self, ids):
        ids = np.ascontiguousarray(ids, dtype=np.int64)
        out = np.empty(ids.size, dtype=np.int64)
        err = _Err()
        lib().moann_ivf_flat_slots_of_ids(self._h, ids.ctypes.data, ids.size,
                                          out.ctypes.data, err.ref)
        err.check("slots_of_ids")
        return out

    def filter_bitset(self, allowed_ids):
        n = len(self)
        words = np.zeros((n + 31) // 32, dtype=np.uint32)
        slots = self.slots_of_ids(allowed_ids)
        slots = slots[slots >= 0]
        np.bitwise_or.at(words, slots // 32,
                         (np.uint32(1) << (slots % 32).astype(np.uint32)))
        return words

    def search_filtered(self, queries, k: int, nprobe: int, bitset_words):
        queries = _as_f32(queries)
        bitset_words = np.ascontiguousarray(bitset_words, dtype=np.uint32)
        nq = queries.shape[0]
        err = _Err()
        res = lib().moann_ivf_flat_search_filtered(
            self._h, queries.ctypes.data, nq, queries.shape[1], k,
            SearchParams(nprobe), bitset_words.ctypes.data,
            bitset_words.size * 32, err.ref)
        err.check("search_filtered")
        return self._read_result(res, nq, k, "search_filtered")

    def search_device(self, queries_tensor, k: int, nprobe: int):
        nq, qdim = queries_tensor.shape
        err = _Err()
        res = lib().moann_ivf_flat_search_device(
            self._h, ct.c_void_p(queries_tensor.data_ptr()), nq, qdim, k,
            SearchParams(nprobe), err.ref)
        err.check("search_device")
        return self._read_result(res, nq, k, "search_device")

    def search_submit(self, queries_tensor, k: int, nprobe: int):
        nq, qdim = queries_tensor.shape
        err = _Err()
        res = lib().moann_ivf_flat_search_submit(
            self._h, ct.c_void_p(queries_tensor.data_ptr()), 1, nq, qdim, k,
            SearchParams(nprobe), err.ref)
        err.check("search_submit")
        if not res.result_ptr:
            raise MoannError("search_submit returned NULL result")
        return (res.result_ptr, nq, k)

    def search_collect(self, ticket):
        ptr, nq, k = ticket
        err = _Err()
        rc = lib().moann_ivf_flat_result_wait(ptr, err.ref)
        err.check("result_wait")
        if rc != 0:
            raise MoannError("result_wait failed")

        class _R:
            result_ptr = ptr
        return self._read_result(_R, nq, k, "search_collect")

    def enable_refine(self, depth: int):
        err = _Err()
        lib().moann_ivf_flat_enable_refine(self._h, depth, err.ref)
        err.check("enable_refine")

    def preds_bitset(self, cols_meta, columns, preds_json: str,
                     nulls=None) -> np.ndarray:
        cols_json, data_arr, null_arr, keep = _col_arrays(cols_meta, columns,
                                                          nulls)
        n = len(self)
        out = np.zeros(max(1, (n + 31) // 32), dtype=np.uint32)
        err = _Err()
        rc = lib().moann_ivf_flat_filter_from_preds(
            self._h, cols_json, preds_json.encode(), data_arr, null_arr,
            out.ctypes.data, err.ref)
        err.check("preds_bitset")
        if rc != 0:
            raise MoannError("preds_bitset failed")
        return out

    def search_pred_filtered(self, queries, k: int, nprobe: int, cols_meta,
                             columns, preds_json: str, nulls=None):
        return self.search_filtered(
            queries, k, nprobe,
            self.preds_bitset(cols_meta, columns, preds_json, nulls))

    def docfilter_bitset(self, kind: int, payload: bytes) -> np.ndarray:
        n = len(self)
        nw = (n + 31) // 32
        out = np.zeros(max(1, nw), dtype=np.uint32)
        buf = ct.create_string_buffer(bytes(payload), len(payload))
        err = _Err()
        rc = lib().moann_ivf_flat_filter_from_docfilter(
            self._h, kind, ct.cast(buf, ct.c_void_p), len(payload),
            out.ctypes.data, err.ref)
        err.check("docfilter_bitset")
        if rc != 0:
            raise MoannError("docfilter_bitset failed")
        return out

    def search_docfiltered(self, queries, k: int, nprobe: int, kind: int,
                           payload: bytes):
        return self.search_filtered(queries, k, nprobe,
                                    self.docfilter_bitset(kind, payload))

    def set_batch_window(self, window_us: int):
        err = _Err()
        lib().gpu_ivf_flat_set_batch_window(self._h, window_us, err.ref)
        err.check("set_batch_window")

    def search_async(self, queries, k: int, nprobe: int):
        queries = _as_f32(queries)
        self._async_shape = (queries.shape[0], k)
        err = _Err()
        job = lib().gpu_ivf_flat_search_quantize_async(
            self._h, queries.ctypes.data, queries.shape[0], queries.shape[1],
            k, SearchParams(nprobe), err.ref)
        err.check("search_quantize_async")
        return job

    def search_wait(self, job: int):
        err = _Err()
        res = lib().gpu_ivf_flat_search_wait(self._h, job, err.ref)
        err.check("search_wait")
        nq, k = self._async_shape
        return self._read_result(res, nq, k, "search_wait")

    def perf(self) -> dict:
        p = PerfT()
        lib().moann_ivf_flat_perf(self._h, ct.byref(p))
        return {f[0]: getattr(p, f[0]) for f in PerfT._fields_}

    def perf_reset(self):
        lib().moann_ivf_flat_perf_reset(self._h)

    def close(self):
        if getattr(self, "_h", None):
            err = _Err()
            lib().gpu_ivf_flat_destroy(self._h, err.ref)
            self._h = None

    def __del__(self):
        try:
            self.close()
        except Exception:
            pass


def pairwise_distance(metric: str, query, rows, device: int = 0):
    query = _as_f32(query).reshape(-1)
    rows = _as_f32(rows)
    out = np.empty(rows.shape[0], dtype=np.float32)
    err = _Err()
    lib().moann_pairwise_distance(METRICS[metric], query.ctypes.data,
                                  rows.ctypes.data, rows.shape[0],
                                  rows.shape[1], device, out.ctypes.data,
                                  err.ref)
    err.check("pairwise_distance")
    return out


def search_with_tail(index, queries, k: int, nprobe: int,
                     tail_vecs, tail_ids, metric: str = None,
                     tail_index=None):
    metric = metric or getattr(index, "metric", "l2sq")
    main_ids, main_d = index.search(queries, k, nprobe)
    if tail_index is not None:
        if len(tail_index) == 0:
            return main_ids, main_d
        t_ids, t_d = tail_index.search(queries, min(k, len(tail_index)))
    elif tail_vecs is None or len(tail_vecs) == 0:
        return main_ids, main_d
    else:
        t_ids, t_d = brute_force_search(tail_vecs, queries,
                                        min(k, len(tail_vecs)),
                                        metric=metric, ids=tail_ids)
    nq = main_ids.shape[0]
    kk = t_ids.shape[1]
    if kk < k:
        pad_i = np.full((nq, k - kk), -1, dtype=np.int64)
        pad_d = np.full((nq, k - kk), np.finfo(np.float32).max,
                        dtype=np.float32)
        t_ids = np.concatenate([t_ids, pad_i], 1)
        t_d = np.concatenate([t_d, pad_d], 1)
    both_i = np.stack([main_ids, t_ids])
    both_d = np.stack([main_d.astype(np.float32), t_d.astype(np.float32)])
    dd = both_d.copy()
    dd[both_i < 0] = np.finfo(np.float32).max
    flat_i = both_i.transpose(1, 0, 2).reshape(nq, -1)
    flat_d = dd.transpose(1, 0, 2).reshape(nq, -1)
    order = np.argsort(flat_d, axis=1, kind="stable")[:, :k]
    out_d = np.take_along_axis(flat_d, order, 1)
    out_i = np.take_along_axis(flat_i, order, 1)
    out_i[out_d >= np.finfo(np.float32).max] = -1
    return out_i, out_d


def brute_force_search(dataset, queries, k: int, metric: str = "l2sq",
                       ids=None, device: int = 0):
    dataset = _as_f32(dataset)
    queries = _as_f32(queries)
    nq = queries.shape[0]
    out_ids = np.empty((nq, k), dtype=np.int64)
    out_dists = np.empty((nq, k), dtype=np.float32)
    idp = None
    if ids is not None:
        ids = np.ascontiguousarray(ids, dtype=np.int64)
        idp = ids.ctypes.data
    err = _Err()
    lib().moann_brute_force_search(
        dataset.ctypes.data, dataset.shape[0], dataset.shape[1],
        METRICS[metric], idp, queries.ctypes.data, nq, k, device,
        out_ids.ctypes.data, out_dists.ctypes.data, err.ref)
    err.check("brute_force_search")
    return out_ids, out_dists


BF_MODES = {"auto": 0, "fused": 1, "gemm": 2}
BF_STORAGES = {"f32": 0, "f16": 1}


def bf_fused_kmax() -> int:
    return int(lib().moann_bf_fused_kmax())


class BruteForceIndex:

    def __init__(self, dim: int, metric: str = "l2sq", capacity: int = 0,
                 storage: str = "f32", device: int = 0):
        self.dim, self.metric = int(dim), metric
        err = _Err()
        devs = (ct.c_int * 1)(device)
        if storage == "f32":
            self._h = lib().moann_bf_new(self.dim, METRICS[metric], capacity,
                                         devs, 1, err.ref)
        else:
            q = BF_STORAGES.get(storage, IvfFlatIndex.QTYPES.get(storage))
            if q is None:
                raise MoannError(f"BruteForceIndex: storage {storage!r} must "
                                 "be 'f32' or 'f16'")
            self._h = lib().moann_bf_new_typed(self.dim, METRICS[metric], q,
                                               capacity, devs, 1, err.ref)
        err.check("BruteForceIndex")
        if not self._h:
            raise MoannError("BruteForceIndex: moann_bf_new returned NULL")

    @property
    def storage(self) -> str:
        q = int(lib().moann_bf_storage(self._h))
        return next(name for name, v in BF_STORAGES.items() if v == q)

    def add(self, rows, ids=None):
        as_half = (self.storage == "f16" and
                   getattr(rows, "dtype", None) == np.float16)
        rows = np.ascontiguousarray(rows) if as_half else _as_f32(rows)
        if rows.ndim != 2 or rows.shape[1] != self.dim:
            raise MoannError(f"add: rows must be [n][{self.dim}]")
        idp = None
        if ids is not None:
            ids = np.ascontiguousarray(ids, dtype=np.int64)
            if ids.shape != (rows.shape[0],):
                raise MoannError("add: one id per row")
            idp = ids.ctypes.data
        err = _Err()
        entry = lib().moann_bf_add_half if as_half else lib().moann_bf_add
        entry(self._h, rows.ctypes.data, rows.shape[0], idp, err.ref)
        err.check("add")

    def add_half(self, rows, ids=None):
        rows = np.ascontiguousarray(rows, dtype=np.float16)
        if rows.ndim != 2 or rows.shape[1] != self.dim:
            raise MoannError(f"add_half: rows must be [n][{self.dim}]")
        idp = None
        if ids is not None:
            ids = np.ascontiguousarray(ids, dtype=np.int64)
            if ids.shape != (rows.shape[0],):
                raise MoannError("add_half: one id per row")
            idp = ids.ctypes.data
        err = _Err()
        lib().moann_bf_add_half(self._h, rows.ctypes.data, rows.shape[0], idp,
                                err.ref)
        err.check("add_half")

    def delete(self, id_: int):
        err = _Err()
        lib().moann_bf_delete_id(self._h, int(id_), err.ref)
        err.check("delete")

    def set_params(self, mode="auto", slice_rows: int = 0):
        err = _Err()
        lib().moann_bf_set_params(self._h, BF_MODES.get(mode, mode),
                                  slice_rows, err.ref)
        err.check("set_params")

    def search(self, queries, k: int, row_bitset=None):
        queries = _as_f32(queries)
        nq = queries.shape[0]
        out_ids = np.empty((nq, max(k, 0)), dtype=np.int64)
        out_dists = np.empty((nq, max(k, 0)), dtype=np.float32)
        err = _Err()
        if row_bitset is None:
            lib().moann_bf_search(self._h, queries.ctypes.data, nq,
                                  queries.shape[1], k, out_ids.ctypes.data,
                                  out_dists.ctypes.data, err.ref)
        else:
            row_bitset = np.ascontiguousarray(row_bitset, dtype=np.uint32)
            lib().moann_bf_search_filtered(
                self._h, queries.ctypes.data, nq, queries.shape[1], k,
                row_bitset.ctypes.data, row_bitset.size * 32,
                out_ids.ctypes.data, out_dists.ctypes.data, err.ref)
        err.check("search")
        return out_ids, out_dists

    def search_device(self, queries_tensor, k: int):
        nq, qdim = queries_tensor.shape
        out_ids = np.empty((nq, k), dtype=np.int64)
        out_dists = np.empty((nq, k), dtype=np.float32)
        err = _Err()
        lib().moann_bf_search_device(
            self._h, ct.c_void_p(queries_tensor.data_ptr()), nq, qdim, k,
            out_ids.ctypes.data, out_dists.ctypes.data, err.ref)
        err.check("search_device")
        return out_ids, out_dists

    def __len__(self):
        return int(lib().moann_bf_len(self._h))

    def perf(self) -> dict:
        p = PerfT()
        lib().moann_bf_perf(self._h, ct.byref(p))
        return {f[0]: getattr(p, f[0]) for f in PerfT._fields_}

    def close(self):
        if getattr(self, "_h", None):
            err = _Err()
            lib().moann_bf_destroy(self._h, err.ref)
            self._h = None

    def __del__(self):
        try:
            self.close()
        except Exception:
            pass


class IvfPqIndex:

    def __init__(self, dim: int, nsub: int, nlist: int, capacity: int = 0,
                 device: int = 0):
        err = _Err()
        dev = (ct.c_int * 1)(device)
        self.dim, self.nsub, self.nlist = dim, nsub, nlist
        self._h = lib().moann_ivf_pq_new(dim, nsub, nlist, capacity, dev, 1,
                                         err.ref)
        err.check("pq_new")
        if not self._h:
            raise MoannError("moann_ivf_pq_new returned NULL")

    def set_centroids(self, centroids):
        centroids = _as_f32(centroids)
        err = _Err()
        lib().moann_ivf_pq_set_centroids(self._h, centroids.ctypes.data,
                                         centroids.shape[0], err.ref)
        err.check("pq_set_centroids")

    def set_codebooks(self, cb):
        cb = _as_f32(cb)
        err = _Err()
        lib().moann_ivf_pq_set_codebooks(self._h, cb.ctypes.data, err.ref)
        err.check("pq_set_codebooks")
# ... 89 lines not shown
```

Measured before the change: 370,000 queries/s.

## Add sample-threshold filtered top-k select and fused refine-finish kernel

Adds a select kernel that samples 4096 distances per query, finds a rank threshold by bitwise binary search, and keeps only candidates under that threshold in LDS. It then bitonic-sorts the survivors, and falls back to the full radix top-k when the survivor count is out of range. It also adds a fused refine-finish kernel that recomputes exact distances for the R refine candidates, sorts them and writes final ids in one launch, replacing the separate refine, select, compose and gather steps. The aim is to cut full radix passes over each query's roughly 78k candidate distances and several small launches, at the cost of an extra sampling pass and atomics. Legacy paths remain selectable, and stats counters are added.

```diff
diff --git a/include/moann.h b/include/moann.h
--- a/include/moann.h
+++ b/include/moann.h
@@ -167,6 +167,22 @@
 
 void moann_ivf_flat_enable_refine(gpu_ivf_flat_c index_c, uint32_t depth,
                                   void* errmsg);
+
+void moann_ivf_flat_set_refine_tail(gpu_ivf_flat_c index_c, int legacy,
+                                    void* errmsg);
+
+void moann_ivf_flat_select_stats(gpu_ivf_flat_c index_c, uint64_t* filtered,
+                                 uint64_t* fallback, void* errmsg);
+
+void moann_select_topk(const float* dists, const int64_t* qoffs, int64_t nq,
+                       int32_t k, int32_t mode, int32_t* out_slots,
+                       float* out_dists, uint64_t* fallbacks,
+                       double* kernel_ms, void* errmsg);
+
+void moann_select_plan(int64_t count, int32_t k, int32_t* filter,
+                       int32_t* sample, int32_t* rank, int32_t* capacity,
+                       int64_t* min_count, int32_t* kmax);
+void moann_select_sample_positions(int64_t count, int32_t k, int64_t* out);
 
 gpu_ivf_flat_search_res_t moann_ivf_flat_search_submit(
     gpu_ivf_flat_c index_c, const void* queries, int queries_on_device,
diff --git a/matrixone_amd/csrc/moann_internal.h b/matrixone_amd/csrc/moann_internal.h
--- a/matrixone_amd/csrc/moann_internal.h
+++ b/matrixone_amd/csrc/moann_internal.h
@@ -35,6 +35,10 @@
 void launch_topk(const float* dists, const int64_t* qoffs, int64_t uniform_n,
                  int nq, int k, int32_t* out_slots, float* out_dists,
                  hipStream_t stream);
+
+void launch_select(const float* dists, const int64_t* qoffs, int nq, int k,
+                   int32_t* out_slots, float* out_dists,
+                   unsigned long long* stats, hipStream_t stream);
 
 void launch_gather(const int32_t* sel_slots, const float* sel_dists,
                    const int32_t* probe_lists, const int64_t* probe_offs,
@@ -143,6 +147,16 @@
 void launch_compose_select(const int32_t* sel2, const int32_t* rsel_slots,
                            int R, int k, int nq, int32_t* out,
                            hipStream_t stream);
+bool refine_finish_applies(int R, int dpad);
+void launch_refine_finish(int metric, const float* rows_f32,
+                          const float* queries, const float* qnorms, int dim,
+                          int dpad, int R, int nq, const int32_t* rsel_slots,
+                          const float* rsel_dists, const int32_t* probe_lists,
+                          const int64_t* probe_offs,
+                          const int64_t* list_slot_base,
+                          const int64_t* id_by_slot, int nprobe, int k,
+                          int do_sqrt, double inv_mul2, int64_t* out_ids,
+                          float* out_dists, hipStream_t stream);
 void launch_quantize_rows(bool uns, const float* in, int64_t nrows,
                           int in_stride, int dim, int dpad, float fmul,
                           float fadd, uint8_t* out, hipStream_t stream);
diff --git a/matrixone_amd/csrc/moann_kernels.hip b/matrixone_amd/csrc/moann_kernels.hip
--- a/matrixone_amd/csrc/moann_kernels.hip
+++ b/matrixone_amd/csrc/moann_kernels.hip
@@ -12,6 +12,7 @@
 
 #include "moann_internal.h"
 #include "moann_scan_device.h"
+#include "moann_select_plan.h"
 
 namespace moann {
 
@@ -154,19 +155,52 @@
     });
 }
 
-__global__ __launch_bounds__(256) void topk_kernel(
-    const float* __restrict__ dists, const int64_t* __restrict__ qoffs,
-    int64_t uniform_n, int k, int sortP,
+__host__ __device__ constexpr size_t topk_radix_lds(int sortP) {
+    return 2048 + (size_t)sortP * 8;
+}
+
+__device__ __forceinline__ void topk_sort_write(
+    uint64_t* keys, int nkeys, int P, int m, int q, int k,
     int32_t* __restrict__ out_slots, float* __restrict__ out_dists) {
-    extern __shared__ unsigned char smem[];
+    const int tid = threadIdx.x;
+    for (int i = nkeys + tid; i < P; i += blockDim.x) keys[i] = ~0ULL;
+    __syncthreads();
+
+    for (int ks = 2; ks <= P; ks <<= 1) {
+        for (int jj = ks >> 1; jj > 0; jj >>= 1) {
+            for (int i = tid; i < P; i += blockDim.x) {
+                const int l = i ^ jj;
+                if (l > i) {
+                    const uint64_t a = keys[i], b = keys[l];
+                    const bool up = (i & ks) == 0;
+                    if ((a > b) == up) { keys[i] = b; keys[l] = a; }
+                }
+            }
+            __syncthreads();
+        }
+    }
+
+    for (int i = tid; i < k; i += blockDim.x) {
+        if (i < m) {
+            const uint64_t kv = keys[i];
+            out_slots[(int64_t)q * k + i] = (int32_t)(kv & 0xFFFFFFFFu);
+            out_dists[(int64_t)q * k + i] = u2f((uint32_t)(kv >> 32));
+        } else {
+            out_slots[(int64_t)q * k + i] = -1;
+            out_dists[(int64_t)q * k + i] = FLT_MAX;
+        }
+    }
+}
+
+__device__ __forceinline__ void topk_radix_block(
+    const float* __restrict__ dists, int64_t off, int64_t count, int q, int k,
+    int sortP, unsigned char* smem, int32_t* __restrict__ out_slots,
+    float* __restrict__ out_dists) {
     uint32_t* hist = (uint32_t*)smem;
     uint32_t* ctr = hist + 256;
     uint32_t* st = ctr + 8;
     uint64_t* keys = (uint64_t*)(smem + 2048);
 
-    const int q = blockIdx.x;
-    const int64_t off = qoffs ? qoffs[q] : (int64_t)q * uniform_n;
-    const int64_t count = (qoffs ? qoffs[q + 1] : (int64_t)(q + 1) * uniform_n) - off;
     const int tid = threadIdx.x;
     const int m = (int)(count < (int64_t)k ? count : k);
     int nkeys;
@@ -256,45 +290,144 @@
         nkeys = m;
     }
 
-    for (int i = nkeys + tid; i < sortP; i += blockDim.x) keys[i] = ~0ULL;
-    __syncthreads();
-
-    for (int ks = 2; ks <= sortP; ks <<= 1) {
-        for (int jj = ks >> 1; jj > 0; jj >>= 1) {
-            for (int i = tid; i < sortP; i += blockDim.x) {
-                const int l = i ^ jj;
-                if (l > i) {
-                    const uint64_t a = keys[i], b = keys[l];
-                    const bool up = (i & ks) == 0;
-                    if ((a > b) == up) { keys[i] = b; keys[l] = a; }
-                }
-            }
+    topk_sort_write(keys, nkeys, sortP, m, q, k, out_slots, out_dists);
+}
+
+__global__ __launch_bounds__(256) void topk_kernel(
+    const float* __restrict__ dists, const int64_t* __restrict__ qoffs,
+    int64_t uniform_n, int k, int sortP,
+    int32_t* __restrict__ out_slots, float* __restrict__ out_dists) {
+    extern __shared__ unsigned char smem[];
+    const int q = blockIdx.x;
+    const int64_t off = qoffs ? qoffs[q] : (int64_t)q * uniform_n;
+    const int64_t count = (qoffs ? qoffs[q + 1] : (int64_t)(q + 1) * uniform_n) - off;
+    topk_radix_block(dists, off, count, q, k, sortP, smem, out_slots,
+                     out_dists);
+}
+
+__device__ __forceinline__ void select_hit(uint32_t u, uint32_t thr,
+                                           int64_t idx, uint32_t* cnt,
+                                           uint64_t* keys) {
+    if (u <= thr) {
+        const uint32_t pos = atomicAdd(cnt, 1u);
+        if (pos < (uint32_t)SELECT_CAPACITY)
+            keys[pos] = ((uint64_t)u << 32) | (uint32_t)idx;
+    }
+}
+
+__global__ __launch_bounds__(SELECT_THREADS) void select_filter_kernel(
+    const float* __restrict__ dists, const int64_t* __restrict__ qoffs,
+    int k, int sortP, int32_t* __restrict__ out_slots,
+    float* __restrict__ out_dists, unsigned long long* __restrict__ stats) {
+    extern __shared__ unsigned char smem[];
+    uint32_t* cnt = (uint32_t*)smem;
+    constexpr int NWAVES = SELECT_THREADS / WAVE;
+    static_assert(SELECT_THREADS % WAVE == 0 && 4 + 2 * NWAVES <= 512,
+                  "per-wave counts live in the 2 KiB state area");
+    uint32_t* wsum = cnt + 4;
+    uint64_t* keys = (uint64_t*)(smem + 2048);
+
+    const int q = blockIdx.x;
+    const int64_t off = qoffs[q];
+    const int64_t count = qoffs[q + 1] - off;
+    const int tid = threadIdx.x, wave = tid >> 6, lane = tid & 63;
+    const SelectPlan plan = select_plan(count, k);
+    const float* row = dists + off;
+    bool radix = !plan.filter;
+    if (plan.filter) {
+        constexpr int SPT = SELECT_SAMPLE / SELECT_THREADS;
+        static_assert(SPT == SELECT_CLUSTER, "one sampled run per thread");
+        uint32_t s[SPT];
+#pragma unroll
+        for (int j = 0; j < SPT; ++j)
+            s[j] = f2u(row[select_sample_pos(count, SELECT_SAMPLE,
+                                             tid * SPT + j)]);
+        if (tid == 0) *cnt = 0;
+        uint32_t thr = 0;
+        for (int bit = 31; bit >= 0; --bit) {
+            const uint32_t cand = thr | (1u << bit);
+            int c = 0;
+#pragma unroll
+            for (int j = 0; j < SPT; ++j) c += s[j] < cand;
+            for (int o = 32; o; o >>= 1) c += __shfl_down(c, o, 64);
+            uint32_t* slot = wsum + NWAVES * (bit & 1);
+            if (lane == 0) slot[wave] = (uint32_t)c;
             __syncthreads();
-        }
-    }
-
-    for (int i = tid; i < k; i += blockDim.x) {
-        if (i < m) {
-            const uint64_t kv = keys[i];
-            out_slots[(int64_t)q * k + i] = (int32_t)(kv & 0xFFFFFFFFu);
-            out_dists[(int64_t)q * k + i] = u2f((uint32_t)(kv >> 32));
-        } else {
-            out_slots[(int64_t)q * k + i] = -1;
-            out_dists[(int64_t)q * k + i] = FLT_MAX;
-        }
-    }
+            uint32_t below = 0;
+#pragma unroll
+            for (int w = 0; w < NWAVES; ++w) below += slot[w];
+            if (below < (uint32_t)plan.t) thr = cand;
+        }
+
+        int64_t head = (4 - (off & 3)) & 3;
+        if (head > count) head = count;
+        const int64_t nvec = (count - head) >> 2;
+        const int64_t tail0 = head + 4 * nvec;
+        if (tid < head) select_hit(f2u(row[tid]), thr, tid, cnt, keys);
+        if (tail0 + tid < count)
+            select_hit(f2u(row[tail0 + tid]), thr, tail0 + tid, cnt, keys);
+        const float4* body = (const float4*)(row + head);
+#define MOANN_SEL4(v, vi)                                                   \
+    select_hit(f2u((v).x), thr, head + 4 * (vi), cnt, keys);                \
+    select_hit(f2u((v).y), thr, head + 4 * (vi) + 1, cnt, keys);            \
+    select_hit(f2u((v).z), thr, head + 4 * (vi) + 2, cnt, keys);            \
+    select_hit(f2u((v).w), thr, head + 4 * (vi) + 3, cnt, keys);
+        int64_t i = tid;
+        const int64_t step = SELECT_THREADS;
+        for (; i + 3 * step < nvec; i += 4 * step) {
+            const float4 v0 = body[i], v1 = body[i + step];
+            const float4 v2 = body[i + 2 * step], v3 = body[i + 3 * step];
+            MOANN_SEL4(v0, i) MOANN_SEL4(v1, i + step)
+            MOANN_SEL4(v2, i + 2 * step) MOANN_SEL4(v3, i + 3 * step)
+        }
+        for (; i < nvec; i += step) {
+            const float4 v = body[i];
+            MOANN_SEL4(v, i)
+        }
+#undef MOANN_SEL4
+        __syncthreads();
+
+        const uint32_t got = *cnt;
+        radix = got < (uint32_t)k || got > (uint32_t)SELECT_CAPACITY;
+        if (tid == 0) atomicAdd(&stats[radix ? 1 : 0], 1ull);
+        if (!radix) {
+            int P = 1;
+            while (P < (int)got) P <<= 1;
+            topk_sort_write(keys, (int)got, P, k, q, k, out_slots, out_dists);
+        }
+        __syncthreads();
+    }
+    if (radix)
+        topk_radix_block(dists, off, count, q, k, sortP, smem, out_slots,
+                         out_dists);
+}
+
+static int topk_sort_size(int k) {
+    int sortP = 1;
+    while (sortP < k) sortP <<= 1;
+    return sortP < 1024 ? 1024 : sortP;
 }
 
 void launch_topk(const float* dists, const int64_t* qoffs, int64_t uniform_n,
                  int nq, int k, int32_t* out_slots, float* out_dists,
                  hipStream_t stream) {
     if (nq == 0) return;
-    int sortP = 1;
-    while (sortP < k) sortP <<= 1;
-    if (sortP < 1024) sortP = 1024;
-    const size_t shmem = 2048 + (size_t)sortP * 8;
-    hipLaunchKernelGGL(topk_kernel, dim3(nq), dim3(256), shmem, stream,
-                       dists, qoffs, uniform_n, k, sortP, out_slots, out_dists);
+    const int sortP = topk_sort_size(k);
+    hipLaunchKernelGGL(topk_kernel, dim3(nq), dim3(256),
+                       topk_radix_lds(sortP), stream, dists, qoffs, uniform_n,
+                       k, sortP, out_slots, out_dists);
+}
+
+void launch_select(const float* dists, const int64_t* qoffs, int nq, int k,
+                   int32_t* out_slots, float* out_dists,
+                   unsigned long long* stats, hipStream_t stream) {
+    if (nq == 0) return;
+    const int sortP = topk_sort_size(k);
+    const size_t shmem = std::max(topk_radix_lds(sortP),
+                                  topk_radix_lds(SELECT_CAPACITY));
+    hipLaunchKernelGGL(select_filter_kernel, dim3(nq), dim3(SELECT_THREADS),
+                       shmem, stream, dists, qoffs, k, sortP, out_slots,
+                       out_dists, stats);
 }
 
 
@@ -791,6 +924,175 @@
     hipLaunchKernelGGL(compose_select_kernel,
                        dim3((uint32_t)((total + 255) / 256)), dim3(256), 0,
                        stream, sel2, rsel_slots, R, k, total, out);
+}
+
+constexpr int REFINE_FINISH_RMAX = 1024;
+
+template <int METRIC>
+__global__ __launch_bounds__(256) void refine_finish_kernel(
+    const float* __restrict__ rows_f32, const float* __restrict__ queries,
+    const float* __restrict__ qnorms, int dim, int dpad, int R, int P,
+    const int32_t* __restrict__ rsel_slots,
+    const float* __restrict__ rsel_dists,
+    const int32_t* __restrict__ probe_lists,
+    const int64_t* __restrict__ probe_offs,
+    const int64_t* __restrict__ list_slot_base,
+    const int64_t* __restrict__ id_by_slot, int nprobe, int k, int do_sqrt,
+    double inv_mul2, int64_t* __restrict__ out_ids,
+    float* __restrict__ out_dists) {
+    extern __shared__ unsigned char rf_smem[];
+    uint64_t* keys = (uint64_t*)rf_smem;
+    int64_t* slots = (int64_t*)(keys + P);
+    float* ldsq = (float*)(slots + R);
+    const int q = blockIdx.x, tid = threadIdx.x;
+    const int wave = tid >> 6, lane = tid & 63;
+    const float* qv = queries + (int64_t)q * dpad;
+    for (int e = tid; e < dpad; e += blockDim.x) ldsq[e] = qv[e];
+
+    const int64_t* offs = probe_offs + (int64_t)q * (nprobe + 1);
+    for (int c = tid; c < R; c += blockDim.x) {
+        const int64_t idx = (int64_t)q * R + c;
+        const int32_t pos = rsel_slots[idx];
+        int64_t slot = -1;
+        if (pos >= 0 && rsel_dists[idx] != FLT_MAX) {
+            int lo = 0, hi = nprobe - 1;
+            while (lo < hi) {
+                const int mid = (lo + hi + 1) >> 1;
+                if (offs[mid] <= pos) lo = mid; else hi = mid - 1;
+            }
+            const int32_t list = probe_lists[(int64_t)q * nprobe + lo];
+            slot = list_slot_base[list] + (pos - offs[lo]);
+        }
+        slots[c] = slot;
+    }
+    for (int c = R + tid; c < P; c += blockDim.x) keys[c] = ~0ULL;
+    __syncthreads();
+
+    for (int c0 = wave * 4; c0 < R; c0 += 16) {
+        const float* row[4];
+#pragma unroll
+        for (int j = 0; j < 4; ++j) {
+            const int64_t slot = c0 + j < R ? slots[c0 + j] : -1;
+            row[j] = slot < 0 ? nullptr : rows_f32 + slot * (int64_t)dim;
+        }
+        float acc[4] = {0.f, 0.f, 0.f, 0.f}, rn[4] = {0.f, 0.f, 0.f, 0.f};
+        for (int t0 = lane; t0 < dim; t0 += 256) {
+            float x[4][4];
+#pragma unroll
+            for (int s = 0; s < 4; ++s)
+#pragma unroll
+                for (int j = 0; j < 4; ++j)
+                    x[s][j] = (t0 + 64 * s < dim && row[j])
+                                  ? row[j][t0 + 64 * s] : 0.f;
+#pragma unroll
+            for (int s = 0; s < 4; ++s) {
+                const int t = t0 + 64 * s;
+                if (t < dim) {
+                    const float qq = ldsq[t];
+#pragma unroll
+                    for (int j = 0; j < 4; ++j) {
+                        const float xv = x[s][j];
+                        if (METRIC == KM_L2SQ) {
+                            const float e = xv - qq;
+                            acc[j] = fmaf(e, e, acc[j]);
+                        } else if (METRIC == KM_IP || METRIC == KM_COS) {
+                            acc[j] = fmaf(xv, qq, acc[j]);
+                            if (METRIC == KM_COS)
+                                rn[j] = fmaf(xv, xv, rn[j]);
+                        } else {
+                            acc[j] += fabsf(xv - qq);
+                        }
+                    }
+                }
+            }
+        }
+#pragma unroll
+        for (int j = 0; j < 4; ++j) {
+            float a = acc[j], r = rn[j];
+            for (int off = 32; off; off >>= 1) {
+                a += __shfl_down(a, off, 64);
+                if (METRIC == KM_COS) r += __shfl_down(r, off, 64);
+            }
+            if (lane == 0 && c0 + j < R) {
+                float dist = FLT_MAX;
+                if (row[j]) {
+                    if (METRIC == KM_IP) dist = -a;
+                    else if (METRIC == KM_COS)
+                        dist = mo_cos_distance(a, r, qnorms[q]);
+                    else dist = a;
+                }
+                keys[c0 + j] = ((uint64_t)f2u(dist) << 32) | (uint32_t)(c0 + j);
+            }
+        }
+    }
+    __syncthreads();
+
+    for (int ks = 2; ks <= P; ks <<= 1) {
+        for (int jj = ks >> 1; jj > 0; jj >>= 1) {
+            for (int i = tid; i < P; i += blockDim.x) {
+                const int l = i ^ jj;
+                if (l > i) {
+                    const uint64_t a = keys[i], b = keys[l];
+                    const bool up = (i & ks) == 0;
+                    if ((a > b) == up) { keys[i] = b; keys[l] = a; }
+                }
+            }
+            __syncthreads();
+        }
+    }
+    for (int i = tid; i < k; i += blockDim.x) {
+        const int64_t o = (int64_t)q * k + i;
+        int64_t slot = -1;
+        float dist = FLT_MAX;
+        if (i < R) {
+            const uint64_t kv = keys[i];
+            slot = slots[(uint32_t)kv];
+            dist = u2f((uint32_t)(kv >> 32));
+        }
+        if (slot < 0 || dist == FLT_MAX) {
+            out_ids[o] = -1; out_dists[o] = FLT_MAX;
+        } else {
+            out_ids[o] = id_by_slot[slot];
+            out_dists[o] = transform_score_dev(dist, do_sqrt, inv_mul2);
+        }
+    }
+}
+
+static size_t refine_finish_lds(int R, int dpad) {
+    int P = 1;
+    while (P < R) P <<= 1;
+    return (size_t)P * 8 + (size_t)R * 8 + (size_t)dpad * 4;
+}
+
+bool refine_finish_applies(int R, int dpad) {
+    return R <= REFINE_FINISH_RMAX && refine_finish_lds(R, dpad) <= 64 * 1024;
+}
+
+void launch_refine_finish(int metric, const float* rows_f32,
+                          const float* queries, const float* qnorms, int dim,
+                          int dpad, int R, int nq, const int32_t* rsel_slots,
+                          const float* rsel_dists, const int32_t* probe_lists,
+                          const int64_t* probe_offs,
+                          const int64_t* list_slot_base,
+                          const int64_t* id_by_slot, int nprobe, int k,
+                          int do_sqrt, double inv_mul2, int64_t* out_ids,
+                          float* out_dists, hipStream_t stream) {
+    if (!nq) return;
+    if (!refine_finish_applies(R, dpad) || k > R)
+        throw std::logic_error("launch_refine_finish: R " + std::to_string(R) +
+                               " k " + std::to_string(k) + " dpad " +
+                               std::to_string(dpad));
+    int P = 1;
+    while (P < R) P <<= 1;
+    const size_t shmem = refine_finish_lds(R, dpad);
+    with_metric(metric, [&](auto m) {
+        hipLaunchKernelGGL(refine_finish_kernel<decltype(m)::value>, dim3(nq),
+                           dim3(256), shmem, stream, rows_f32, queries, qnorms,
+                           dim, dpad, R, P, rsel_slots, rsel_dists,
+                           probe_lists, probe_offs, list_slot_base,
+                           id_by_slot, nprobe, k, do_sqrt, inv_mul2, out_ids,
+                           out_dists);
+    });
 }
 
 template <int METRIC, bool UNSIGNED>
diff --git a/matrixone_amd/csrc/moann_lib.cpp b/matrixone_amd/csrc/moann_lib.cpp
--- a/matrixone_amd/csrc/moann_lib.cpp
+++ b/matrixone_amd/csrc/moann_lib.cpp
@@ -23,6 +23,7 @@
 #include "../../include/moann.h"
 #include "moann_host_common.h"
 #include "moann_kmeans_plan.h"
+#include "moann_select_plan.h"
 
 namespace {
 
@@ -71,6 +72,7 @@
         uint32_t limit = 0, probe = 0;
         ScanChoice scan {};
         bool refine = false;
+        bool outputs_written = false;
         const float* d_q = nullptr;
         const float* d_qn = nullptr;
     } call;
@@ -99,6 +101,8 @@
         if (h_out) (void)hipHostFree(h_out);
     }
 };
+
+const ScanOverrides& scan_overrides();
 
 struct IvfIndex {
     int device = 0;
@@ -118,6 +122,8 @@
     ByteImageLayout rq_layout = ByteImageLayout::ROWS16;
     int32_t* d_rownorm_rq = nullptr;
     double rq_mul = 1.0, rq_add = 0.0;
+    bool refine_tail_legacy = scan_overrides().refine_tail_legacy;
+    unsigned long long* d_select_stats = nullptr;
     bool built = false, started = false;
 
     hipStream_t stream = nullptr;
@@ -207,7 +213,8 @@
                        (void*)d_cent_rows, (void*)d_cnorms, (void*)d_packed_q,
                        (void*)d_rownorm_q, (void*)d_rows_f32,
                        (void*)d_packed_rq, (void*)d_rownorm_rq,
-                       (void*)d_id_by_slot, (void*)d_list_slot_base})
+                       (void*)d_id_by_slot, (void*)d_list_slot_base,
+                       (void*)d_select_stats})
             if (p) (void)hipFree(p);
         if (stream) (void)hipStreamDestroy(stream);
     }
@@ -353,8 +360,10 @@
     static const ScanOverrides ov = [] {
         const char *sc = getenv("MOANN_SCAN"), *bq = getenv("MOANN_BYTE_QT"),
                    *cg = getenv("MOANN_CHUNKG"),
-                   *bm = getenv("MOANN_BYTE_MFMA");
+                   *bm = getenv("MOANN_BYTE_MFMA"),
+                   *rt = getenv("MOANN_REFINE_TAIL");
         ScanOverrides o;
+        o.refine_tail_legacy = rt && strcmp(rt, "legacy") == 0;
         o.generic_f32 = sc && strcmp(sc, "generic") == 0;
         o.byte_qt8 = bq && atoi(bq) == 8;
         o.chunk_g = cg ? atoi(cg) : 0;
@@ -499,8 +508,16 @@
     HIP_CHECK(hipEventRecord(cx->ev[3], s));
 }
 
+int score_sqrt(const IvfIndex* ix) {
+    return ix->metric == DistanceType_L2SqrtExpanded;
+}
+double score_inv_mul2(const IvfIndex* ix) {
+    return (ix->quant_mul != 0.0 && ix->quant_mul != 1.0)
+               ? 1.0 / (ix->quant_mul * ix->quant_mul) : 1.0;
+}
+
 void select_candidates(IvfIndex* ix, SearchCtx* cx) {
-    const SearchCtx::Call& c = cx->call;
+    SearchCtx::Call& c = cx->call;
     const int dpad = (int)ix->dpad, nq = (int)c.nq, limit = (int)c.limit;
     const hipStream_t s = cx->stream;
     upload_vector(cx->w_qoffs, cx->offs.qoffs, s);
@@ -508,15 +525,46 @@
     upload_vector(cx->w_probe_offs, cx->offs.probe_offs, s);
     cx->w_sel_slots.ensure((size_t)c.nq * limit * 4);
     cx->w_sel_dists.ensure((size_t)c.nq * limit * 4);
+    const bool legacy = ix->refine_tail_legacy;
+    if (!legacy && !ix->d_select_stats) {
+        HIP_CHECK(hipMalloc(&ix->d_select_stats, 16));
+        HIP_CHECK(hipMemset(ix->d_select_stats, 0, 16));
+    }
+    const auto select_ragged = [&](int k, int32_t* slots, float* dists) {
+        if (legacy)
+            launch_topk(cx->w_cand.as<float>(), cx->w_qoffs.as<int64_t>(), 0,
+                        nq, k, slots, dists, s);
+        else
+            launch_select(cx->w_cand.as<float>(), cx->w_qoffs.as<int64_t>(),
+                          nq, k, slots, dists, ix->d_select_stats, s);
+    };
+    c.outputs_written = false;
     HIP_CHECK(hipEventRecord(cx->ev[4], s));
     if (c.refine) {
         const int R = std::max<int>(limit, ix->refine_depth);
         cx->w_rsel_slots.ensure((size_t)c.nq * R * 4);
         cx->w_rsel_dists.ensure((size_t)c.nq * R * 4);
-        launch_topk(cx->w_cand.as<float>(), cx->w_qoffs.as<int64_t>(), 0, nq,
-                    R, cx->w_rsel_slots.as<int32_t>(),
-                    cx->w_rsel_dists.as<float>(), s);
+        select_ragged(R, cx->w_rsel_slots.as<int32_t>(),
+                      cx->w_rsel_dists.as<float>());
         KCHECK("refine-topR");
+        if (!legacy && refine_finish_applies(R, dpad)) {
+            const size_t n = (size_t)c.nq * limit;
+            cx->w_out_ids.ensure(n * 8);
+            cx->w_out_dists.ensure(n * 4);
+            launch_refine_finish(
+                ix->kmetric, ix->d_rows_f32, c.d_q, c.d_qn, (int)ix->dim,
+                dpad, R, nq, cx->w_rsel_slots.as<int32_t>(),
+                cx->w_rsel_dists.as<float>(),
+                cx->w_probe_lists.as<int32_t>(),
+                cx->w_probe_offs.as<int64_t>(), ix->d_list_slot_base,
+                ix->d_id_by_slot, (int)c.probe, limit, score_sqrt(ix),
+                score_inv_mul2(ix), cx->w_out_ids.as<int64_t>(),
+                cx->w_out_dists.as<float>(), s);
+            KCHECK("refine-finish");
+            c.outputs_written = true;
+            HIP_CHECK(hipEventRecord(cx->ev[5], s));
+            return;
+        }
         cx->w_refined.ensure((size_t)c.nq * R * 4);
         launch_refine(ix->kmetric, ix->d_rows_f32, c.d_q, c.d_qn,
                       (int)ix->dim, dpad, R, nq,
@@ -535,9 +583,8 @@
                               cx->w_sel_slots.as<int32_t>(), s);
         KCHECK("refine-compose");
     } else {
-        launch_topk(cx->w_cand.as<float>(), cx->w_qoffs.as<int64_t>(), 0, nq,
-                    limit, cx->w_sel_slots.as<int32_t>(),
-                    cx->w_sel_dists.as<float>(), s);
+        select_ragged(limit, cx->w_sel_slots.as<int32_t>(),
+                      cx->w_sel_dists.as<float>());
         KCHECK("cand-topk");
     }
     HIP_CHECK(hipEventRecord(cx->ev[5], s));
@@ -547,19 +594,19 @@
     const SearchCtx::Call& c = cx->call;
     const size_t n = (size_t)c.nq * c.limit;
     const hipStream_t s = cx->stream;
-    const int do_sqrt = ix->metric == DistanceType_L2SqrtExpanded;
-    const double inv_mul2 =
-        (ix->quant_mul != 0.0 && ix->quant_mul != 1.0)
-            ? 1.0 / (ix->quant_mul * ix->quant_mul) : 1.0;
-    cx->w_out_ids.ensure(n * 8);
-    cx->w_out_dists.ensure(n * 4);
-    launch_gather(cx->w_sel_slots.as<int32_t>(), cx->w_sel_dists.as<float>(),
-                  cx->w_probe_lists.as<int32_t>(),
-                  cx->w_probe_offs.as<int64_t>(), ix->d_list_slot_base,
-                  ix->d_id_by_slot, (int)c.probe, (int)c.nq, (int)c.limit,
-                  do_sqrt, inv_mul2, cx->w_out_ids.as<int64_t>(),
-                  cx->w_out_dists.as<float>(), s);
-    KCHECK("gather");
+    if (!c.outputs_written) {
+        cx->w_out_ids.ensure(n * 8);
+        cx->w_out_dists.ensure(n * 4);
+        launch_gather(cx->w_sel_slots.as<int32_t>(),
+                      cx->w_sel_dists.as<float>(),
+                      cx->w_probe_lists.as<int32_t>(),
+                      cx->w_probe_offs.as<int64_t>(), ix->d_list_slot_base,
+                      ix->d_id_by_slot, (int)c.probe, (int)c.nq, (int)c.limit,
+                      score_sqrt(ix), score_inv_mul2(ix),
+                      cx->w_out_ids.as<int64_t>(),
+                      cx->w_out_dists.as<float>(), s);
+        KCHECK("gather");
+    }
     cx->ensure_hout(n * 12);
     int64_t* ho_ids = (int64_t*)cx->h_out;
     float* ho_dists = (float*)(ho_ids + n);
@@ -1745,6 +1792,121 @@
     }
 }
 
+void moann_ivf_flat_select_stats(gpu_ivf_flat_c h, uint64_t* filtered,
+                                 uint64_t* fallback, void* errmsg) {
+    try {
+        auto ix = IX(h);
+        if (!ix) throw std::runtime_error("null index");
+        std::lock_guard<std::mutex> lk(ix->mu);
+        unsigned long long sum[2] = {0, 0};
+        for (IvfIndex* part : {ix, ix->tail.get()}) {
+            if (!part || !part->d_select_stats) continue;
+            unsigned long long st[2];
+            HIP_CHECK(hipSetDevice(part->device));
+            HIP_CHECK(hipDeviceSynchronize());
+            HIP_CHECK(hipMemcpy(st, part->d_select_stats, sizeof st,
+                                hipMemcpyDeviceToHost));
+            sum[0] += st[0];
+            sum[1] += st[1];
+        }
+        if (filtered) *filtered = sum[0];
+        if (fallback) *fallback = sum[1];
+    } catch (const std::exception& e) {
+        set_errmsg(errmsg, "moann_ivf_flat_select_stats", e.what());
+    }
+}
+
+void moann_ivf_flat_set_refine_tail(gpu_ivf_flat_c h, int legacy,
+                                    void* errmsg) {
+    try {
+        auto ix = IX(h);
+        if (!ix) throw std::runtime_error("null index");
+        std::lock_guard<std::mutex> lk(ix->mu);
+        ix->refine_tail_legacy = legacy != 0;
+        if (ix->tail) ix->tail->refine_tail_legacy = legacy != 0;
+    } catch (const std::exception& e) {
+        set_errmsg(errmsg, "moann_ivf_flat_set_refine_tail", e.what());
+    }
+}
+
+void moann_select_plan(int64_t count, int32_t k, int32_t* filter,
+                       int32_t* sample, int32_t* rank, int32_t* capacity,
+                       int64_t* min_count, int32_t* kmax) {
+    const SelectPlan p = select_plan(count, k);
+    if (filter) *filter = p.filter;
+    if (sample) *sample = p.m;
+    if (rank) *rank = p.t;
+    if (capacity) *capacity = SELECT_CAPACITY;
+    if (min_count) *min_count = SELECT_MIN_COUNT;
+    if (kmax) *kmax = SELECT_KMAX;
+}
+
+void moann_select_sample_positions(int64_t count, int32_t k, int64_t* out) {
+    const SelectPlan p = select_plan(count, k);
+    for (int i = 0; p.filter && i < p.m; ++i)
+        out[i] = select_sample_pos(count, p.m, i);
+}
+
+void moann_select_topk(const float* dists, const int64_t* qoffs, int64_t nq,
+                       int32_t k, int32_t mode, int32_t* out_slots,
+                       float* out_dists, uint64_t* fallbacks, double* kernel_ms,
+                       void* errmsg) {
+    try {
+        if (nq < 0 || nq > INT32_MAX || k < 1 || k > 4096 ||
+            (mode != 0 && mode != 1))
+            throw std::runtime_error("bad nq, k or mode");
+        if (fallbacks) *fallbacks = 0;
+        if (kernel_ms) *kernel_ms = 0.0;
+        if (nq == 0) return;
+        for (int64_t q = 0; q < nq; ++q)
+            if (qoffs[q] < 0 || qoffs[q + 1] < qoffs[q] ||
+                qoffs[q + 1] - qoffs[q] > UINT32_MAX)
+                throw std::runtime_error("qoffs must ascend from >= 0");
+        const size_t total = (size_t)qoffs[nq], no = (size_t)nq * k;
+        DevBuf d_d, d_o, d_s, d_od, d_st;
+        d_d.ensure(std::max<size_t>(1, total) * 4);
+        d_o.ensure((size_t)(nq + 1) * 8);
+        d_s.ensure(no * 4);
+        d_od.ensure(no * 4);
+        d_st.ensure(16);
+        HIP_CHECK(hipMemcpy(d_d.ptr, dists, total * 4, hipMemcpyHostToDevice));
+        HIP_CHECK(hipMemcpy(d_o.ptr, qoffs, (size_t)(nq + 1) * 8,
+                            hipMemcpyHostToDevice));
+        HIP_CHECK(hipMemset(d_st.ptr, 0, 16));
+        struct Events {
+            hipEvent_t e[2] = {nullptr, nullptr};
+            ~Events() {
+                for (hipEvent_t x : e)
+                    if (x) (void)hipEventDestroy(x);
+            }
+        } ev;
+        HIP_CHECK(hipEventCreate(&ev.e[0]));
+        HIP_CHECK(hipEventCreate(&ev.e[1]));
+        HIP_CHECK(hipEventRecord(ev.e[0], nullptr));
+        if (mode == 1)
+            launch_select(d_d.as<float>(), d_o.as<int64_t>(), (int)nq, k,
+                          d_s.as<int32_t>(), d_od.as<float>(),
+                          d_st.as<unsigned long long>(), nullptr);
+        else
+            launch_topk(d_d.as<float>(), d_o.as<int64_t>(), 0, (int)nq, k,
+                        d_s.as<int32_t>(), d_od.as<float>(), nullptr);
+        HIP_CHECK(hipEventRecord(ev.e[1], nullptr));
+        HIP_CHECK(hipDeviceSynchronize());
+        KCHECK("select-topk");
+        float ms = 0.f;
+        HIP_CHECK(hipEventElapsedTime(&ms, ev.e[0], ev.e[1]));
+        unsigned long long st[2];
+        HIP_CHECK(hipMemcpy(out_slots, d_s.ptr, no * 4, hipMemcpyDeviceToHost));
+        HIP_CHECK(hipMemcpy(out_dists, d_od.ptr, no * 4,
+                            hipMemcpyDeviceToHost));
+        HIP_CHECK(hipMemcpy(st, d_st.ptr, 16, hipMemcpyDeviceToHost));
+        if (fallbacks) *fallbacks = st[1];
+        if (kernel_ms) *kernel_ms = ms;
+    } catch (const std::exception& e) {
+        set_errmsg(errmsg, "moann_select_topk", e.what());
+    }
+}
+
 void moann_brute_force_search(const float* dataset, uint64_t count,
                               uint32_t dimension, distance_type_t metric,
                               const int64_t* ids, const float* queries,
@@ -1908,6 +2070,7 @@
     chk("tail set_assignments");
     gpu_ivf_flat_build(th, &inner);
     chk("tail build");
+    tix->refine_tail_legacy = ix->refine_tail_legacy;
     ix->tail = std::move(tix);
     for (int64_t id : ix->tail_deleted) {
         IvfIndex* t = ix->tail.get();
diff --git a/matrixone_amd/csrc/moann_scan_plan.h b/matrixone_amd/csrc/moann_scan_plan.h
--- a/matrixone_amd/csrc/moann_scan_plan.h
+++ b/matrixone_amd/csrc/moann_scan_plan.h
@@ -55,6 +55,7 @@
     bool byte_qt8 = false;
     int chunk_g = 0;
     bool byte_mfma_off = false;
+    bool refine_tail_legacy = false;
 };
 
 struct ScanChoice {
diff --git a/matrixone_amd/csrc/moann_select_plan.h b/matrixone_amd/csrc/moann_select_plan.h
--- /dev/null
+++ b/matrixone_amd/csrc/moann_select_plan.h
@@ -0,0 +1,50 @@
+
+#ifndef MOANN_SELECT_PLAN_H
+#define MOANN_SELECT_PLAN_H
+
+#include <cstdint>
+
+#if defined(__HIPCC__)
+#define MOANN_SELECT_HD __host__ __device__
+#else
+#define MOANN_SELECT_HD
+#endif
+
+namespace moann {
+
+constexpr int SELECT_THREADS = 256;
+constexpr int SELECT_SAMPLE = 4096;
+constexpr int SELECT_CLUSTER = 16;
+constexpr int SELECT_CAPACITY = 2048;
+constexpr int SELECT_OVERSAMPLE = 8;
+constexpr int SELECT_T_MIN = 8;
+constexpr int SELECT_KMAX = 128;
+constexpr int64_t SELECT_MIN_COUNT = 4 * (int64_t)SELECT_SAMPLE;
+
+struct SelectPlan {
+    bool filter;
+    int m;
+    int t;
+};
+
+MOANN_SELECT_HD inline int64_t select_sample_pos(int64_t count, int m, int i) {
+    const int runs = m / SELECT_CLUSTER;
+    return (int64_t)(i / SELECT_CLUSTER) * count / runs + i % SELECT_CLUSTER;
+}
+
+MOANN_SELECT_HD inline SelectPlan select_plan(int64_t count, int k) {
+    SelectPlan p;
+    p.m = SELECT_SAMPLE;
+    p.t = 0;
+    p.filter = k >= 1 && k <= SELECT_KMAX && count >= SELECT_MIN_COUNT;
+    if (!p.filter) return p;
+    const int64_t want = (int64_t)SELECT_OVERSAMPLE * k * p.m;
+    int64_t t = (want + count - 1) / count;
+    if (t < SELECT_T_MIN) t = SELECT_T_MIN;
+    p.t = (int)t;
+    return p;
+}
+
+}
+
+#endif
diff --git a/matrixone_amd/csrc/select_plan_check.cpp b/matrixone_amd/csrc/select_plan_check.cpp
--- /dev/null
+++ b/matrixone_amd/csrc/select_plan_check.cpp
@@ -0,0 +1,79 @@
+
+#include "moann_select_plan.h"
+
+#include <cstdio>
+#include <cstdlib>
+
+using namespace moann;
+
+namespace {
+
+char g_case[128] = "";
+int g_checks = 0;
+
+#define CHECK(cond)                                                        \
+    do {                                                                   \
+        ++g_checks;                                                        \
+        if (!(cond)) {                                                     \
+            fprintf(stderr, "select_plan_check: %s:%d: %s\n  case: %s\n",  \
+                    __FILE__, __LINE__, #cond, g_case);                    \
+            exit(1);                                                       \
+        }                                                                  \
+    } while (0)
+
+void check_plan(int64_t count, int k) {
+    snprintf(g_case, sizeof g_case, "count=%lld k=%d", (long long)count, k);
+    const SelectPlan p = select_plan(count, k);
+    CHECK(p.filter ==
+          (k >= 1 && k <= SELECT_KMAX && count >= SELECT_MIN_COUNT));
+    if (!p.filter) return;
+    CHECK(p.m == SELECT_SAMPLE && p.m % SELECT_THREADS == 0);
+    CHECK(p.m % SELECT_CLUSTER == 0);
+    CHECK(p.t >= SELECT_T_MIN && p.t <= p.m);
+    const double expect = (double)p.t * (double)count / p.m;
+    CHECK(expect >= (double)SELECT_OVERSAMPLE * k);
+    CHECK(expect < (double)SELECT_OVERSAMPLE * k + (double)count / p.m ||
+          p.t == SELECT_T_MIN);
+    if (p.t > SELECT_T_MIN) CHECK(2 * expect <= SELECT_CAPACITY + 2.0 * count / p.m);
+    const int runs = p.m / SELECT_CLUSTER;
+    int64_t prev = -1;
+    for (int i = 0; i < p.m; ++i) {
+        const int64_t pos = select_sample_pos(count, p.m, i);
+        CHECK(pos > prev && pos < count);
+        if (i % SELECT_CLUSTER) CHECK(pos == prev + 1);
+        prev = pos;
+    }
+    CHECK(select_sample_pos(count, p.m, 0) == 0);
+    CHECK(count - prev <= count / runs + 1);
+}
+
+}
+
+int main() {
+    const int64_t M = SELECT_MIN_COUNT;
+    const int64_t counts[] = {0, 1, 63, 64, 4095, 4096, M - 1, M, M + 1,
+                              M + 2, M + 3, M + 17, 3 * M + 5, 20000, 78000,
+                              78125, 1000000, 10000000,
+                              ((int64_t)1 << 31) - 1, (int64_t)1 << 32,
+                              (int64_t)1 << 40};
+    const int ks[] = {-1, 0, 1, 10, 63, 64, 65, SELECT_KMAX, SELECT_KMAX + 1,
+                      1024, 4096};
+    for (int64_t c : counts)
+        for (int k : ks) check_plan(c, k);
+
+    snprintf(g_case, sizeof g_case, "constants");
+    CHECK(SELECT_OVERSAMPLE * SELECT_KMAX * 2 <= SELECT_CAPACITY);
+    CHECK(SELECT_MIN_COUNT >= SELECT_SAMPLE && SELECT_MIN_COUNT > SELECT_KMAX);
+    CHECK(SELECT_SAMPLE % SELECT_THREADS == 0);
+    CHECK(select_plan(SELECT_MIN_COUNT, SELECT_KMAX).t ==
+          SELECT_OVERSAMPLE * SELECT_KMAX * SELECT_SAMPLE / SELECT_MIN_COUNT);
+
+    {
+        const SelectPlan p = select_plan(78000, 64);
+        CHECK(p.filter && p.t == 27);
+        CHECK(!select_plan(78000, SELECT_KMAX + 1).filter);
+        CHECK(select_plan(78000, 10).t == SELECT_T_MIN);
+    }
+    printf("select_plan_check OK: %d checks\n", g_checks);
+    return 0;
+}
diff --git a/matrixone_amd/engine.py b/matrixone_amd/engine.py
--- a/matrixone_amd/engine.py
+++ b/matrixone_amd/engine.py
@@ -166,6 +166,20 @@
     L.moann_ivf_flat_result_wait.argtypes = [ct.c_void_p, ct.c_void_p]
     L.moann_ivf_flat_enable_refine.argtypes = [ct.c_void_p, ct.c_uint32,
                                                ct.c_void_p]
+    L.moann_ivf_flat_set_refine_tail.argtypes = [ct.c_void_p, ct.c_int,
+                                                 ct.c_void_p]
+    L.moann_ivf_flat_select_stats.argtypes = [
+        ct.c_void_p, ct.POINTER(ct.c_uint64), ct.POINTER(ct.c_uint64),
+        ct.c_void_p]
+    L.moann_select_topk.argtypes = [
+        ct.c_void_p, ct.c_void_p, ct.c_int64, ct.c_int32, ct.c_int32,
+        ct.c_void_p, ct.c_void_p, ct.POINTER(ct.c_uint64),
+        ct.POINTER(ct.c_double), ct.c_void_p]
+    L.moann_select_plan.argtypes = [
+        ct.c_int64, ct.c_int32] + [ct.POINTER(ct.c_int32)] * 4 + [
+        ct.POINTER(ct.c_int64), ct.POINTER(ct.c_int32)]
+    L.moann_select_sample_positions.argtypes = [ct.c_int64, ct.c_int32,
+                                                ct.c_void_p]
     L.moann_docfilter_eval.restype = ct.c_int
     L.moann_docfilter_eval.argtypes = [
         ct.c_int, ct.c_void_p, ct.c_uint64, ct.c_void_p, ct.c_uint64,
@@ -616,6 +630,20 @@
         lib().moann_ivf_flat_enable_refine(self._h, depth, err.ref)
         err.check("enable_refine")
 
+    def set_refine_tail(self, legacy: bool):
+        err = _Err()
+        lib().moann_ivf_flat_set_refine_tail(self._h, int(bool(legacy)),
+                                             err.ref)
+        err.check("set_refine_tail")
+
+    def select_stats(self) -> dict:
+        f, b = ct.c_uint64(0), ct.c_uint64(0)
+        err = _Err()
+        lib().moann_ivf_flat_select_stats(self._h, ct.byref(f), ct.byref(b),
+                                          err.ref)
+        err.check("select_stats")
+        return {"filtered": f.value, "fallback": b.value}
+
     def preds_bitset(self, cols_meta, columns, preds_json: str,
                      nulls=None) -> np.ndarray:
         cols_json, data_arr, null_arr, keep = _col_arrays(cols_meta, columns,
@@ -768,6 +796,41 @@
     return out_ids, out_dists
 
 
+SELECT_MODES = {"radix": 0, "filter": 1}
+
+
+def select_plan(count: int, k: int) -> dict:
+    f, m, t, cap, kmax = (ct.c_int32(0) for _ in range(5))
+    mn = ct.c_int64(0)
+    lib().moann_select_plan(count, k, ct.byref(f), ct.byref(m), ct.byref(t),
+                            ct.byref(cap), ct.byref(mn), ct.byref(kmax))
+    return {"filter": bool(f.value), "sample": m.value, "rank": t.value,
+            "capacity": cap.value, "min_count": mn.value, "kmax": kmax.value}
+
+
+def select_sample_positions(count: int, k: int) -> np.ndarray:
+    p = select_plan(count, k)
+    out = np.zeros(p["sample"] if p["filter"] else 0, dtype=np.int64)
+    lib().moann_select_sample_positions(count, k, out.ctypes.data)
+    return out
+
+
+def select_topk(dists, qoffs, k: int, mode: str = "filter"):
+    dists = np.ascontiguousarray(dists, dtype=np.float32)
+    qoffs = np.ascontiguousarray(qoffs, dtype=np.int64)
+    nq = qoffs.shape[0] - 1
+    out_s = np.empty((nq, k), dtype=np.int32)
+    out_d = np.empty((nq, k), dtype=np.float32)
+    fb, ms = ct.c_uint64(0), ct.c_double(0)
+    err = _Err()
+    lib().moann_select_topk(dists.ctypes.data, qoffs.ctypes.data, nq, k,
+                            SELECT_MODES[mode], out_s.ctypes.data,
+                            out_d.ctypes.data, ct.byref(fb), ct.byref(ms),
+                            err.ref)
+    err.check("select_topk")
+    return out_s, out_d, int(fb.value), float(ms.value)
+
+
 BF_MODES = {"auto": 0, "fused": 1, "gemm": 2}
 BF_STORAGES = {"f32": 0, "f16": 1}
 
```

Result: faster. 446,700 queries/s, median of 6 (+20.7%).
